# dpmerrell/PathMatFac.jl

Measured on AMD Instinct MI355X. Metric: fit_iters_per_sec, higher is better.
Workload: dtype f32; 1 GPU; fit! epoch on synthetic 200000x50000 matrix (D stored as f32), K=64, Gaussian loss, group-reg X (32 groups) + featureset-ARD Y, adam; rows sharded over 1 GPU(s); full_model=False, M=200000, N=50000, K=64, rows_per_gpu=200000, optimizer=adam, parallelism=single GPU, rccl_ranks=0, collectives_issued=0, column_chunks=1

## Files before the change

include/pmf_hip.h:

```cpp
#ifndef PMF_HIP_H
#define PMF_HIP_H

#include <stdint.h>

#ifdef __cplusplus
extern "C" {
#endif

typedef struct pmf_ctx pmf_ctx;

#define PMF_NOISE_NORMAL 0
#define PMF_NOISE_BERNOULLI 1
#define PMF_NOISE_POISSON 2
#define PMF_NOISE_SQ_HINGE 3

#define PMF_OPT_ADAGRAD 0
#define PMF_OPT_ADAM 1

#define PMF_STORE_F32 0
#define PMF_STORE_BF16 1

#define PMF_TERM_MAX_EPOCHS 0
#define PMF_TERM_LOSS_INCREASE 1
#define PMF_TERM_ABS_TOL 2
#define PMF_TERM_REL_TOL 3
#define PMF_TERM_NONFINITE 4

#define PMF_PARAM_X 0
#define PMF_PARAM_Y 1
#define PMF_PARAM_LOGSIGMA 2
#define PMF_PARAM_MU 3
#define PMF_PARAM_LOGDELTA 4
#define PMF_PARAM_THETA 5

typedef struct pmf_fit_opts {
  int32_t update_X;
  int32_t update_Y;
  int32_t update_col_layers;
  int32_t frozen_layers;
  int32_t frozen_regs;
  int32_t max_epochs;
  int32_t epoch;
  int32_t tol_max_iters;
  int32_t keep_trace;
  int32_t verbosity;
  int32_t print_iter;
  int32_t reserved;
  double abs_tol;
  double rel_tol;
  int64_t capacity;
} pmf_fit_opts;

typedef struct pmf_fit_result {
  int32_t term_code;
  int32_t epochs;
  int32_t n_trace;
  int32_t trace_cap;
  double final_loss;
  double *loss_trace;
  double seconds;
} pmf_fit_result;

const char *pmf_last_error(void);
int pmf_version(void);

int pmf_device_count(int *n);
int pmf_create(int device, pmf_ctx **out);
int pmf_destroy(pmf_ctx *ctx);
int pmf_set_stream(pmf_ctx *ctx, void *hip_stream);
int pmf_synchronize(pmf_ctx *ctx);

int pmf_set_data(pmf_ctx *ctx, const float *D_colmajor, int64_t M, int64_t N, int store);
int pmf_set_data_device(pmf_ctx *ctx, const void *D_device, int64_t M, int64_t N, int store);

int pmf_set_factors(pmf_ctx *ctx, const float *X, const float *Y, int K);
int pmf_set_X(pmf_ctx *ctx, const float *X, int K);
int pmf_set_Y(pmf_ctx *ctx, const float *Y, int K);
int pmf_get_factors(pmf_ctx *ctx, float *X, float *Y);

int pmf_set_col_params(pmf_ctx *ctx, const float *logsigma, const float *mu);
int pmf_get_col_params(pmf_ctx *ctx, float *logsigma, float *mu);

int pmf_set_n_batch_views(pmf_ctx *ctx, int n);
int pmf_set_batch_view(pmf_ctx *ctx, int v, int64_t col_start1, int64_t col_stop1, int nb,
                       const int32_t *batch_of_row, const float *logdelta, const float *theta);
int pmf_get_batch_view(pmf_ctx *ctx, int v, float *logdelta, float *theta);

int pmf_set_noise(pmf_ctx *ctx, int n_ranges, const int64_t *starts1, const int64_t *stops1, const int32_t *kinds,
                  const float *weights);

int pmf_set_noise_thresholds(pmf_ctx *ctx, int n_ranges, const int64_t *starts1, const int64_t *stops1, const float *thr);
int pmf_get_noise_thresholds(pmf_ctx *ctx, float *thr);

int pmf_clear_xreg(pmf_ctx *ctx);
int pmf_add_xreg_l2(pmf_ctx *ctx, const float *w, float p);
int pmf_add_xreg_group(pmf_ctx *ctx, int n_groups, const int64_t *starts1, const int64_t *stops1, const float *w,
                       float p);

int pmf_clear_yreg(pmf_ctx *ctx);
int pmf_add_yreg_l2(pmf_ctx *ctx, const float *w, float p);
int pmf_add_yreg_group(pmf_ctx *ctx, int n_groups, const int64_t *starts1, const int64_t *stops1, const float *w,
                       float p);
int pmf_add_yreg_ard(pmf_ctx *ctx, int n_ranges, const int64_t *starts1, const int64_t *stops1, const float *alpha,
                     const float *beta, float p);
int pmf_add_yreg_fsard(pmf_ctx *ctx, const float *alpha, const float *beta, float p);

typedef struct pmf_csr { int64_t n_rows, n_cols; const int64_t *rowptr; const int32_t *col; const float *val; } pmf_csr;
int pmf_add_xreg_network(pmf_ctx *ctx, int K, const pmf_csr *AA, const pmf_csr *AB, const pmf_csr *BB,
                         const float *const *u0, float p);
int pmf_add_yreg_network(pmf_ctx *ctx, int K, const pmf_csr *AA, const pmf_csr *AB, const pmf_csr *BB,
                         const float *const *u0, float p);
int pmf_get_reg_network_state(pmf_ctx *ctx, int which, int k, float *u, int *cg_iters);
int pmf_add_xreg_l1(pmf_ctx *ctx, const float *w, const uint8_t *mask, float p);
int pmf_add_yreg_l1(pmf_ctx *ctx, const float *w, const uint8_t *mask, float p);

int pmf_set_layer_regs(pmf_ctx *ctx, int n_ranges, const int64_t *starts1, const int64_t *stops1,
                       const float *w_logsigma, const float *c_logsigma, const float *w_mu, const float *c_mu,
                       const float *w_logdelta, const float *c_logdelta, const float *w_theta,
                       const float *c_theta);

int pmf_set_optimizer(pmf_ctx *ctx, int kind, float lr, float eps, float beta1, float beta2);
int pmf_set_lr(pmf_ctx *ctx, float lr);
int pmf_get_lr(pmf_ctx *ctx, float *lr);
int pmf_reset_optimizer_state(pmf_ctx *ctx);
int pmf_get_opt_state(pmf_ctx *ctx, int which, int view, float *acc, float *mom);

int pmf_fit(pmf_ctx *ctx, const pmf_fit_opts *opts, pmf_fit_result *result);

int pmf_loss(pmf_ctx *ctx, double *total, double *data, double *xreg, double *yreg);

typedef struct pmf_lbfgs_opts {
  int32_t m;
  int32_t max_iter;
  int32_t backtrack_max_iter;
  int32_t keep_trace;
  int32_t verbosity;
  int32_t print_iter;
  double rel_tol;
  double abs_tol;
  double backtrack_shrinkage;
  double c1;
  double sy_min;
} pmf_lbfgs_opts;
typedef struct pmf_lbfgs_result {
  int32_t term_code;
  int32_t iters;
  int32_t loss_evals;
  int32_t grad_evals;
  int32_t resets;
  int32_t n_trace;
  int32_t trace_cap;
  int32_t reserved;
  double final_loss;
  double seconds;
  double *loss_trace;
  int32_t *trial_trace;
  int32_t *flag_trace;
} pmf_lbfgs_result;
int pmf_fit_lbfgs(pmf_ctx *ctx, const pmf_lbfgs_opts *opts, pmf_lbfgs_result *result);
int pmf_debug_lbfgs_direction(pmf_ctx *ctx, int n_pairs, const float *sX, const float *sY, const float *yX,
                              const float *yY, const float *gX, const float *gY, float *pX, float *pY);

int pmf_epoch_begin(pmf_ctx *ctx, const pmf_fit_opts *opts);
int pmf_epoch_step_local(pmf_ctx *ctx, const pmf_fit_opts *opts);
int pmf_epoch_step_shared(pmf_ctx *ctx, const pmf_fit_opts *opts);
int pmf_epoch_loss(pmf_ctx *ctx, double *local_loss, double *shared_terms);

#define PMF_COMM_ID_BYTES 128
#define PMF_COMM_NONE 0
#define PMF_COMM_RCCL 1
#define PMF_COMM_HOST 2
typedef int (*pmf_host_allreduce_fn)(void *user, void *host_buf, int64_t count, int dtype);
int pmf_comm_get_unique_id(void *id_out);
int pmf_comm_init(pmf_ctx *ctx, int rank, int nranks, const void *unique_id);
int pmf_comm_init_host(pmf_ctx *ctx, int rank, int nranks, pmf_host_allreduce_fn fn, void *user);
int pmf_comm_destroy(pmf_ctx *ctx);
int pmf_comm_set_chunks(pmf_ctx *ctx, int n_chunks);
int pmf_comm_allreduce(pmf_ctx *ctx, void *host_buf, int64_t count, int dtype, int op);
int pmf_comm_info(pmf_ctx *ctx, int *rank, int *nranks, int *transport, int *n_chunks, int *reserved_cus,
                  int64_t *n_collectives);

int pmf_debug_last_path(pmf_ctx *ctx, int *bmode, int *layer_path, int *slots, int *xreg);
int pmf_debug_last_kernel(pmf_ctx *ctx, int *kernel);

#define PMF_PASS_EXTENTS_MAX 16
int pmf_debug_pass_extents(pmf_ctx *ctx, int update_X, int update_Y, const int64_t *cap_override, int n_max,
                           const char **names, int64_t *need, int64_t *capacity, int *n);

int pmf_debug_live_bytes(int64_t *device_bytes, int64_t *pinned_bytes);

int pmf_grad_device_ptr(pmf_ctx *ctx, int which, void **ptr, int64_t *n_elements);
int pmf_get_grad(pmf_ctx *ctx, int which, int view, float *out);

int pmf_forward(pmf_ctx *ctx, float *Z_host);

#define PMF_IMPUTE_BATCH 1
#define PMF_IMPUTE_LINK 2
#define PMF_IMPUTE_KEEP_OBSERVED 4
int pmf_impute(pmf_ctx *ctx, int flags, int64_t row_start1, int64_t row_stop1, float *out_host, int64_t ld);
int pmf_impute_device(pmf_ctx *ctx, int flags, int64_t row_start1, int64_t row_stop1, float *out_device, int64_t ld);
int pmf_impute_entries(pmf_ctx *ctx, int flags, int64_t n, const int64_t *rows1, const int64_t *cols1, float *out_host);
int pmf_debug_impute_offset(int64_t row, int64_t col, int64_t ld, int64_t *offset);

typedef struct pmf_sim_opts {
  uint64_t seed;
  int64_t row_offset;
  float noise;
  float frac_missing;
} pmf_sim_opts;
int pmf_simulate_data(pmf_ctx *ctx, const pmf_sim_opts *opts, int64_t row_start1, int64_t row_stop1, float *out_host, int64_t ld);
int pmf_simulate_data_device(pmf_ctx *ctx, const pmf_sim_opts *opts, int64_t row_start1, int64_t row_stop1, float *out_device,
                             int64_t ld);
int pmf_simulate_data_resident(pmf_ctx *ctx, const pmf_sim_opts *opts);

#define PMF_DEBATCH_LINK 1
#define PMF_DEBATCH_FILL_MISSING 2
int pmf_remove_batch_effect(pmf_ctx *ctx, int flags, int64_t row_start1, int64_t row_stop1, const float *Z_host, int64_t ldz,
                            float *out_host, int64_t ld);
int pmf_remove_batch_effect_device(pmf_ctx *ctx, int flags, int64_t row_start1, int64_t row_stop1, const float *Z_device,
                                   int64_t ldz, float *out_device, int64_t ld);
int pmf_remove_batch_effect_entries(pmf_ctx *ctx, int flags, int64_t n, const int64_t *rows1, const int64_t *cols1,
                                    const float *values, float *out_host);

int pmf_stats(pmf_ctx *ctx, int use_factors, float *col_n, float *col_sum, float *col_sumsq, float *col_sqerr,
              float *col_ssq_grad, float *batch_count, float *batch_sqerr);

typedef struct pmf_em_opts {
  int32_t update_priors;
  int32_t max_iter;
  int32_t verbosity;
  int32_t reserved;
  double rtol;
} pmf_em_opts;
typedef struct pmf_em_result {
  int32_t iters;
  int32_t n_diffs;
  int32_t diffs_cap;
  int32_t reserved;
  double *diffs;
  double seconds;
} pmf_em_result;
int pmf_stage_init_logsigma(pmf_ctx *ctx);
int pmf_stage_reweight_col_losses(pmf_ctx *ctx, int64_t M_total);
int pmf_get_noise_weights(pmf_ctx *ctx, float *w);
int pmf_stage_minimal_group_weights(pmf_ctx *ctx, int64_t M_total, float *w_out);
int pmf_stage_theta_delta_em(pmf_ctx *ctx, const pmf_em_opts *opts, const float *sigma2, double *delta2,
                             pmf_em_result *result);

int pmf_gram(pmf_ctx *ctx, int which, int n_groups, const int64_t *starts1, const int64_t *stops1, int diag_only, double *out);
int pmf_stage_lambda_max(pmf_ctx *ctx, int which, int n_groups, const int64_t *starts1, const int64_t *stops1, double *lam_out);
int pmf_stage_whiten(pmf_ctx *ctx, int64_t M_total, int n_views, const int64_t *starts1, const int64_t *stops1,
                     double *x_rms_out, double *y_rms_max_out);
int pmf_stage_rotate_by_svd(pmf_ctx *ctx, double *sing_out, double *U_out);
int pmf_stage_reorder_by_importance(pmf_ctx *ctx, int32_t *perm_out);
int pmf_debug_postprocess_times(pmf_ctx *ctx, double *gram_s, double *eig_s, double *apply_s);

int pmf_fsard_update_A(pmf_ctx *ctx, int64_t col_start1, int64_t col_stop1, int L, const float *S, const float *alpha,
                       const float *lambda, float alpha0, float v0, float lr, float *ssq_grad, float *A, int max_epochs,
                       int term_iter, double atol, double *best_loss, int *epochs_run, float *beta_out);
int pmf_fsard_update_A_csr(pmf_ctx *ctx, int64_t col_start1, int64_t col_stop1, int L, const int64_t *rowptr,
                           const int32_t *col, const float *val, const float *alpha, const float *lambda, float alpha0,
                           float v0, float lr, float *ssq_grad, float *A, int max_epochs, int term_iter, double atol,
                           double *best_loss, int *epochs_run, float *beta_out);

#define PMF_PREC_F32 0
#define PMF_PREC_BF16X3 1
int pmf_set_precision(pmf_ctx *ctx, int mode);
int pmf_get_precision(pmf_ctx *ctx, int *mode, int64_t *split_launches);

int pmf_kernel_time(pmf_ctx *ctx, double *mean_ms, int64_t *launches, int reset);
int pmf_synth_data(pmf_ctx *ctx, uint64_t seed, float noise, float frac_nan);

#ifdef __cplusplus
}
#endif
#endif
```

pathmatfac.jl_amd/_lib.py:

```python
import ctypes as C
import os
from pathlib import Path

import numpy as np

_HERE = Path(__file__).resolve().parent
LIB_PATH = _HERE / "libpmf_hip.so"

NOISE = {"normal": 0, "bernoulli": 1, "poisson": 2, "bernoulli_sq_hinge": 3, "ordinal_sq_hinge3": 3}
HINGE_THRESHOLDS = {"bernoulli_sq_hinge": (0.0, np.inf, np.inf), "ordinal_sq_hinge3": (-np.inf, -0.5, 0.5)}
OPT = {"adagrad": 0, "adam": 1}
STORE = {"f32": 0, "bf16": 1}
TERM = {0: "max_epochs", 1: "loss_increase", 2: "abs_tol", 3: "rel_tol", 4: "nonfinite"}
IMPUTE_BATCH, IMPUTE_LINK, IMPUTE_KEEP_OBSERVED = 1, 2, 4
DEBATCH_LINK, DEBATCH_FILL_MISSING = 1, 2
PARAM = {"X": 0, "Y": 1, "logsigma": 2, "mu": 3, "logdelta": 4, "theta": 5}


class PMFError(RuntimeError):
    pass


class FitOpts(C.Structure):
    _fields_ = [("update_X", C.c_int32), ("update_Y", C.c_int32), ("update_col_layers", C.c_int32),
                ("frozen_layers", C.c_int32), ("frozen_regs", C.c_int32), ("max_epochs", C.c_int32),
                ("epoch", C.c_int32), ("tol_max_iters", C.c_int32), ("keep_trace", C.c_int32),
                ("verbosity", C.c_int32), ("print_iter", C.c_int32), ("reserved", C.c_int32),
                ("abs_tol", C.c_double), ("rel_tol", C.c_double), ("capacity", C.c_int64)]


class FitResult(C.Structure):
    _fields_ = [("term_code", C.c_int32), ("epochs", C.c_int32), ("n_trace", C.c_int32),
                ("trace_cap", C.c_int32), ("final_loss", C.c_double), ("loss_trace", C.POINTER(C.c_double)),
                ("seconds", C.c_double)]


class LbfgsOpts(C.Structure):
    _fields_ = [("m", C.c_int32), ("max_iter", C.c_int32), ("backtrack_max_iter", C.c_int32), ("keep_trace", C.c_int32),
                ("verbosity", C.c_int32), ("print_iter", C.c_int32), ("rel_tol", C.c_double), ("abs_tol", C.c_double),
                ("backtrack_shrinkage", C.c_double), ("c1", C.c_double), ("sy_min", C.c_double)]


class LbfgsResult(C.Structure):
    _fields_ = [("term_code", C.c_int32), ("iters", C.c_int32), ("loss_evals", C.c_int32), ("grad_evals", C.c_int32),
                ("resets", C.c_int32), ("n_trace", C.c_int32), ("trace_cap", C.c_int32), ("reserved", C.c_int32),
                ("final_loss", C.c_double), ("seconds", C.c_double), ("loss_trace", C.POINTER(C.c_double)),
                ("trial_trace", C.POINTER(C.c_int32)), ("flag_trace", C.POINTER(C.c_int32))]


class EmOpts(C.Structure):
    _fields_ = [("update_priors", C.c_int32), ("max_iter", C.c_int32), ("verbosity", C.c_int32), ("reserved", C.c_int32),
                ("rtol", C.c_double)]


class EmResult(C.Structure):
    _fields_ = [("iters", C.c_int32), ("n_diffs", C.c_int32), ("diffs_cap", C.c_int32), ("reserved", C.c_int32),
                ("diffs", C.POINTER(C.c_double)), ("seconds", C.c_double)]


class SimOpts(C.Structure):
    _fields_ = [("seed", C.c_uint64), ("row_offset", C.c_int64), ("noise", C.c_float), ("frac_missing", C.c_float)]


class Csr(C.Structure):
    _fields_ = [("n_rows", C.c_int64), ("n_cols", C.c_int64), ("rowptr", C.POINTER(C.c_int64)),
                ("col", C.POINTER(C.c_int32)), ("val", C.POINTER(C.c_float))]


def csr_arrays(A):
    import scipy.sparse as sp
    A = sp.csr_matrix(A)
    A.sum_duplicates()
    A.sort_indices()
    return (A.shape, np.ascontiguousarray(A.indptr, dtype=np.int64), np.ascontiguousarray(A.indices, dtype=np.int32),
            np.ascontiguousarray(A.data, dtype=np.float32))


def dense_to_csr(S):
    S = np.ascontiguousarray(S, dtype=np.float32)
    if S.ndim != 2:
        raise ValueError("dense_to_csr: S must be a matrix")
    L, Nv = S.shape
    flat = np.flatnonzero(S.ravel())
    rowptr = np.zeros(L + 1, np.int64)
    if Nv:
        np.cumsum(np.bincount(flat // Nv, minlength=L), out=rowptr[1:])
        col = (flat % Nv).astype(np.int32)
    else:
        col = np.zeros(0, np.int32)
    return rowptr, col, S.ravel()[flat].astype(np.float32)


EXPORTS = [
    "pmf_last_error", "pmf_version", "pmf_device_count", "pmf_create", "pmf_destroy", "pmf_set_stream", "pmf_synchronize",
    "pmf_set_data", "pmf_set_data_device", "pmf_set_factors", "pmf_set_X", "pmf_set_Y", "pmf_get_factors",
    "pmf_set_col_params", "pmf_get_col_params", "pmf_set_n_batch_views", "pmf_set_batch_view",
    "pmf_get_batch_view", "pmf_set_noise", "pmf_clear_xreg", "pmf_add_xreg_l2", "pmf_add_xreg_group",
    "pmf_clear_yreg", "pmf_add_yreg_l2", "pmf_add_yreg_group", "pmf_add_yreg_ard", "pmf_add_yreg_fsard",
    "pmf_set_layer_regs", "pmf_set_optimizer", "pmf_set_lr", "pmf_get_lr", "pmf_reset_optimizer_state",
    "pmf_fit", "pmf_epoch_begin", "pmf_epoch_step_local", "pmf_epoch_step_shared", "pmf_epoch_loss",
    "pmf_grad_device_ptr", "pmf_get_grad", "pmf_forward", "pmf_stats", "pmf_kernel_time", "pmf_synth_data",
    "pmf_set_precision", "pmf_get_precision",
    "pmf_comm_get_unique_id", "pmf_comm_init", "pmf_comm_init_host", "pmf_comm_destroy", "pmf_comm_set_chunks",
    "pmf_comm_info", "pmf_comm_allreduce", "pmf_get_opt_state", "pmf_fsard_update_A", "pmf_debug_last_path", "pmf_debug_last_kernel",
    "pmf_debug_pass_extents", "pmf_debug_live_bytes",
    "pmf_add_xreg_network", "pmf_add_yreg_network", "pmf_get_reg_network_state", "pmf_add_xreg_l1", "pmf_add_yreg_l1",
    "pmf_impute", "pmf_impute_device", "pmf_impute_entries", "pmf_debug_impute_offset",
    "pmf_loss", "pmf_fit_lbfgs", "pmf_debug_lbfgs_direction",
    "pmf_stage_init_logsigma", "pmf_stage_reweight_col_losses", "pmf_get_noise_weights", "pmf_stage_minimal_group_weights",
    "pmf_stage_theta_delta_em",
    "pmf_gram", "pmf_stage_lambda_max", "pmf_stage_whiten", "pmf_stage_rotate_by_svd", "pmf_stage_reorder_by_importance",
    "pmf_debug_postprocess_times",
    "pmf_fsard_update_A_csr",
    "pmf_set_noise_thresholds", "pmf_get_noise_thresholds",
    "pmf_remove_batch_effect", "pmf_remove_batch_effect_device", "pmf_remove_batch_effect_entries",
    "pmf_simulate_data", "pmf_simulate_data_device", "pmf_simulate_data_resident",
]

COMM_ID_BYTES = 128
HOST_ALLREDUCE_FN = C.CFUNCTYPE(C.c_int, C.c_void_p, C.c_void_p, C.c_int64, C.c_int)


def comm_unique_id(lib_path=None):
    lib = load_library(lib_path)
    buf = C.create_string_buffer(COMM_ID_BYTES)
    if lib.pmf_comm_get_unique_id(buf) != 0:
        raise PMFError(lib.pmf_last_error().decode())
    return buf.raw



def live_bytes(lib_path=None):
    lib = load_library(lib_path)
    d, h = C.c_int64(0), C.c_int64(0)
    if lib.pmf_debug_live_bytes(C.byref(d), C.byref(h)) != 0:
        raise PMFError(lib.pmf_last_error().decode())
    return d.value, h.value


def device_count(lib_path=None):
    lib = load_library(lib_path)
    n = C.c_int(0)
    if lib.pmf_device_count(C.byref(n)) != 0:
        raise PMFError(lib.pmf_last_error().decode())
    return n.value


_lib = None


def load_library(path=None):
    global _lib
    if _lib is not None and path is None:
        return _lib
    p = Path(path) if path else LIB_PATH
    if not p.exists():
        raise PMFError(f"{p} not found: build it with pathmatfac.jl_amd/csrc/build.sh "
                       "(python -c 'import __graft_entry__ as g; g.build()'). There is no CPU fallback.")
    if os.environ.get("PMF_NO_TORCH", "0") != "1":
        try:
            import torch
        except ImportError:
            pass
    lib = C.CDLL(str(p))
    lib.pmf_last_error.restype = C.c_char_p
    for name in EXPORTS:
        getattr(lib, name)
    _lib = lib
    return lib


def _f32(a, order="F"):
    return np.require(np.asarray(a, dtype=np.float32), requirements=["F" if order == "F" else "C", "A"])


def _fp(a):
    return a.ctypes.data_as(C.POINTER(C.c_float)) if a is not None else C.POINTER(C.c_float)()


def _i64p(a):
    return a.ctypes.data_as(C.POINTER(C.c_int64))


def _flat(a):
    if a is None:
        return None
    if isinstance(a, (list, tuple)) and len(a) and np.ndim(a[0]) > 0:
        a = np.concatenate([np.asarray(x, dtype=np.float32).ravel() for x in a])
    return _f32(np.asarray(a, dtype=np.float32).ravel())


def _ranges(ranges):
    s = np.ascontiguousarray([r[0] for r in ranges], dtype=np.int64)
    e = np.ascontiguousarray([r[1] for r in ranges], dtype=np.int64)
    return s, e


class Context:

    def __init__(self, device=0, lib_path=None):
        self.lib = load_library(lib_path)
        self._h = C.c_void_p()
        self._chk(self.lib.pmf_create(int(device), C.byref(self._h)))
        self.M = self.N = self.K = 0
        self.view_shapes = []
        self.n_noise_ranges = 0

    def _chk(self, rc):
        if rc != 0:
            raise PMFError(self.lib.pmf_last_error().decode())

    def close(self):
        if getattr(self, "_h", None) is not None and self._h:
            self.lib.pmf_destroy(self._h)
            self._h = None

    def __del__(self):
        try:
            self.close()
        except Exception:
            pass

    def set_stream(self, stream_ptr):
        HIP_STREAM_LEGACY = 1
        self._chk(self.lib.pmf_set_stream(self._h, C.c_void_p(stream_ptr if stream_ptr else HIP_STREAM_LEGACY)))
        self._stream_adopted = True

    def use_own_stream(self):
        self._chk(self.lib.pmf_set_stream(self._h, C.c_void_p(0)))
        self._stream_adopted = False

    def synchronize(self):
        self._chk(self.lib.pmf_synchronize(self._h))

    def set_data(self, D, store="f32"):
        D = _f32(D)
        if D.shape != (self.M, self.N):
            self.n_noise_ranges = 0
        self.M, self.N = D.shape
        self._chk(self.lib.pmf_set_data(self._h, _fp(D), C.c_int64(self.M), C.c_int64(self.N), STORE[store]))

    def set_data_device(self, ptr, M, N, store="f32"):
        if (int(M), int(N)) != (self.M, self.N):
            self.n_noise_ranges = 0
        self.M, self.N = int(M), int(N)
        self._chk(self.lib.pmf_set_data_device(self._h, C.c_void_p(ptr), C.c_int64(M), C.c_int64(N), STORE[store]))

    def set_factors(self, X, Y):
        X, Y = _f32(X), _f32(Y)
        K = X.shape[0]
        if X.shape != (K, self.M) or Y.shape != (K, self.N):
            raise PMFError(f"factor shapes {X.shape}, {Y.shape} do not match data {self.M} x {self.N}")
        self.K = K
        self._chk(self.lib.pmf_set_factors(self._h, _fp(X), _fp(Y), K))

    def set_X(self, X):
        X = _f32(X)
        self._chk(self.lib.pmf_set_X(self._h, _fp(X), X.shape[0]))

    def set_Y(self, Y):
        Y = _f32(Y)
        self._chk(self.lib.pmf_set_Y(self._h, _fp(Y), Y.shape[0]))

    def get_factors(self):
        X = np.zeros((self.K, self.M), np.float32, order="F")
        Y = np.zeros((self.K, self.N), np.float32, order="F")
        self._chk(self.lib.pmf_get_factors(self._h, _fp(X), _fp(Y)))
        return X, Y

    def set_col_params(self, logsigma=None, mu=None):
        ls = None if logsigma is None else _f32(logsigma)
        m = None if mu is None else _f32(mu)
        self._chk(self.lib.pmf_set_col_params(self._h, _fp(ls), _fp(m)))

    def get_col_params(self):
        ls = np.zeros(self.N, np.float32)
        mu = np.zeros(self.N, np.float32)
        self._chk(self.lib.pmf_get_col_params(self._h, _fp(ls), _fp(mu)))
        return ls, mu

    def set_batch_views(self, views):
        self._chk(self.lib.pmf_set_n_batch_views(self._h, len(views)))
        self.view_shapes = []
        for v, b in enumerate(views):
            ld, th = _f32(b["logdelta"]), _f32(b["theta"])
            nb, Nv = ld.shape
            bor = np.ascontiguousarray(b["batch_of_row"], dtype=np.int32)
            if bor.shape != (self.M,):
                raise PMFError("batch_of_row must have one entry per row")
            self._chk(self.lib.pmf_set_batch_view(self._h, v, C.c_int64(b["start1"]), C.c_int64(b["stop1"]), nb,
                                                  bor.ctypes.data_as(C.POINTER(C.c_int32)), _fp(ld), _fp(th)))
            self.view_shapes.append((nb, Nv))

    def update_batch_values(self, v, start1, stop1, batch_of_row, logdelta, theta):
        ld, th = _f32(logdelta), _f32(theta)
        bor = np.ascontiguousarray(batch_of_row, dtype=np.int32)
        self._chk(self.lib.pmf_set_batch_view(self._h, v, C.c_int64(start1), C.c_int64(stop1), ld.shape[0],
                                              bor.ctypes.data_as(C.POINTER(C.c_int32)), _fp(ld), _fp(th)))

    def get_batch_view(self, v):
        nb, Nv = self.view_shapes[v]
        ld = np.zeros((nb, Nv), np.float32, order="F")
        th = np.zeros((nb, Nv), np.float32, order="F")
        self._chk(self.lib.pmf_get_batch_view(self._h, v, _fp(ld), _fp(th)))
        return ld, th

    def set_noise(self, ranges, kinds, weights=None):
        s, e = _ranges(ranges)
        k = np.ascontiguousarray([NOISE[x] if isinstance(x, str) else int(x) for x in kinds], dtype=np.int32)
        w = None if weights is None else _f32(weights)
        self._chk(self.lib.pmf_set_noise(self._h, len(k), _i64p(s), _i64p(e), k.ctypes.data_as(C.POINTER(C.c_int32)),
                                         _fp(w)))
        self.n_noise_ranges = len(k)
        named = [(r, HINGE_THRESHOLDS[x]) for r, x in zip(ranges, kinds) if x == "ordinal_sq_hinge3"]
        if named:
            self.set_noise_thresholds([r for r, _ in named], [t for _, t in named])

    def set_noise_thresholds(self, ranges, thresholds):
        s, e = _ranges(ranges)
        t = np.ascontiguousarray(np.asarray(thresholds, dtype=np.float32).reshape(len(s), 3))
        self._chk(self.lib.pmf_set_noise_thresholds(self._h, len(s), _i64p(s), _i64p(e), _fp(t)))

    def get_noise_thresholds(self):
        t = np.zeros((self.N, 3), np.float32)
        self._chk(self.lib.pmf_get_noise_thresholds(self._h, _fp(t)))
        return t

    def clear_xreg(self):
        self._chk(self.lib.pmf_clear_xreg(self._h))

    def clear_yreg(self):
        self._chk(self.lib.pmf_clear_yreg(self._h))

    def add_reg_l2(self, which, w, p=1.0):
        w = _f32(np.asarray(w).ravel())
        f = self.lib.pmf_add_xreg_l2 if which == "X" else self.lib.pmf_add_yreg_l2
        self._chk(f(self._h, _fp(w), C.c_float(p)))

    def add_reg_group(self, which, ranges, w, p=1.0):
        s, e = _ranges(ranges)
        w = np.ascontiguousarray(np.asarray(w, dtype=np.float32))
        if w.shape != (len(s), self.K):
            raise PMFError(f"group weights must be (n_groups, K) = ({len(s)}, {self.K}); got {w.shape}")
        f = self.lib.pmf_add_xreg_group if which == "X" else self.lib.pmf_add_yreg_group
        self._chk(f(self._h, len(s), _i64p(s), _i64p(e), _fp(w), C.c_float(p)))

    def add_yreg_ard(self, ranges, alpha, beta, p=1.0):
        s, e = _ranges(ranges)
        a, b = _f32(np.asarray(alpha).ravel()), _f32(np.asarray(beta).ravel())
        self._chk(self.lib.pmf_add_yreg_ard(self._h, len(s), _i64p(s), _i64p(e), _fp(a), _fp(b), C.c_float(p)))

    def add_yreg_fsard(self, alpha, beta, p=1.0):
        a, b = _f32(np.asarray(alpha).ravel()), _f32(beta)
        if a.shape != (self.N,) or b.shape != (self.K, self.N):
            raise PMFError("FeatureSetARD: alpha must be N, beta K x N")
        self._chk(self.lib.pmf_add_yreg_fsard(self._h, _fp(a), _fp(b), C.c_float(p)))

    def add_reg_network(self, which, AA, AB, BB, u0=None, p=1.0):
        K = len(AA)
        keep, blocks = [], []
        for mats in (AA, AB, BB):
            arr = (Csr * K)()
            for k, A in enumerate(mats):
                shape, rp, col, val = csr_arrays(A)
                keep.append((rp, col, val))
                arr[k] = Csr(shape[0], shape[1], rp.ctypes.data_as(C.POINTER(C.c_int64)),
                             col.ctypes.data_as(C.POINTER(C.c_int32)), _fp(val))
            blocks.append(arr)
        up = None
        if u0 is not None:
            us = [_f32(np.asarray(u).ravel()) for u in u0]
            for k, (u, B) in enumerate(zip(us, BB)):
                if u.shape != (B.shape[0],):
                    raise PMFError(f"network regularizer: u0[{k}] has {u.shape[0]} entries, BB[{k}] {B.shape[0]} rows")
            keep.append(us)
            up = (C.POINTER(C.c_float) * K)(*[_fp(u) for u in us])
        f = self.lib.pmf_add_xreg_network if which == "X" else self.lib.pmf_add_yreg_network
        self._chk(f(self._h, K, blocks[0], blocks[1], blocks[2], up, C.c_float(p)))
        if not hasattr(self, "_net_v"):
            self._net_v = {}
        self._net_v[which] = [int(B.shape[0]) for B in BB]

    def get_reg_network_state(self, which, k):
        v = getattr(self, "_net_v", {}).get(which)
        n = v[k] if v is not None and 0 <= k < len(v) else 0
        u = np.zeros(n, np.float32)
        it = C.c_int(0)
        self._chk(self.lib.pmf_get_reg_network_state(self._h, PARAM[which], int(k), _fp(u) if n else None, C.byref(it)))
        return u, it.value

    def add_reg_l1(self, which, w, mask=None, p=1.0):
        w = _f32(np.asarray(w).ravel())
        n = self.M if which == "X" else self.N
        if w.shape != (self.K,):
            raise PMFError(f"L1 weights must have K = {self.K} entries; got {w.shape}")
        mp = None
        if mask is not None:
            m = np.require(np.asarray(mask, dtype=np.uint8), requirements=["F", "A"])
            if m.shape != (self.K, n):
                raise PMFError(f"L1 mask must be K x n = ({self.K}, {n}); got {m.shape}")
            mp = m.ctypes.data_as(C.POINTER(C.c_uint8))
        f = self.lib.pmf_add_xreg_l1 if which == "X" else self.lib.pmf_add_yreg_l1
        self._chk(f(self._h, _fp(w), mp, C.c_float(p)))

    def set_layer_regs(self, ranges=None, w_logsigma=None, c_logsigma=None, w_mu=None, c_mu=None,
                       w_logdelta=None, c_logdelta=None, w_theta=None, c_theta=None):
        ranges = ranges or []
        s, e = _ranges(ranges) if ranges else (np.zeros(1, np.int64), np.zeros(1, np.int64))
        arrs = [_flat(a) for a in (w_logsigma, c_logsigma, w_mu, c_mu, w_logdelta, c_logdelta, w_theta, c_theta)]
        self._keep = arrs
        self._chk(self.lib.pmf_set_layer_regs(self._h, len(ranges), _i64p(s), _i64p(e), *[_fp(a) for a in arrs]))

    def set_optimizer(self, kind="adagrad", lr=1.0, eps=1e-8, beta1=0.9, beta2=0.999):
        self._chk(self.lib.pmf_set_optimizer(self._h, OPT[kind], C.c_float(lr), C.c_float(eps), C.c_float(beta1),
                                             C.c_float(beta2)))

    def set_lr(self, lr):
        self._chk(self.lib.pmf_set_lr(self._h, C.c_float(lr)))

    def get_lr(self):
        v = C.c_float(0)
        self._chk(self.lib.pmf_get_lr(self._h, C.byref(v)))
        return v.value

    def reset_optimizer_state(self):
        self._chk(self.lib.pmf_reset_optimizer_state(self._h))

    @staticmethod
    def make_opts(update_X=False, update_Y=False, update_col_layers=False, frozen_layers=0, frozen_regs=0,
                  max_epochs=1000, epoch=1, tol_max_iters=3, keep_trace=True, verbosity=0, print_iter=10,
                  abs_tol=1e-9, rel_tol=1e-6, capacity=10 ** 8):
        o = FitOpts()
        o.update_X, o.update_Y, o.update_col_layers = int(update_X), int(update_Y), int(update_col_layers)
        o.frozen_layers, o.frozen_regs = int(frozen_layers), int(frozen_regs)
        o.max_epochs, o.epoch, o.tol_max_iters = int(max_epochs), int(epoch), int(tol_max_iters)
        o.keep_trace, o.verbosity, o.print_iter = int(keep_trace), int(verbosity), int(print_iter)
        o.abs_tol, o.rel_tol, o.capacity = float(abs_tol), float(rel_tol), int(capacity)
        return o

    def fit(self, **kw):
        o = self.make_opts(**kw)
        cap = max(o.max_epochs - o.epoch + 1, 1)
        trace = np.zeros(cap, np.float64)
        r = FitResult()
        r.trace_cap = cap
        r.loss_trace = trace.ctypes.data_as(C.POINTER(C.c_double))
        self._chk(self.lib.pmf_fit(self._h, C.byref(o), C.byref(r)))
        return {"term_code": TERM[r.term_code], "epochs": r.epochs, "loss": trace[:r.n_trace].copy(),
                "final_loss": r.final_loss, "seconds": r.seconds}

    def loss(self):
        v = [C.c_double(0) for _ in range(4)]
        self._chk(self.lib.pmf_loss(self._h, *[C.byref(x) for x in v]))
        return dict(zip(("total", "data", "xreg", "yreg"), (x.value for x in v)))

    def fit_lbfgs(self, m=10, max_iter=1000, backtrack_max_iter=100, rel_tol=1e-9, abs_tol=1e-6, backtrack_shrinkage=0.8,
                  c1=1e-4, sy_min=1e-4, keep_trace=True, verbosity=0, print_iter=10):
        o = LbfgsOpts(int(m), int(max_iter), int(backtrack_max_iter), int(keep_trace), int(verbosity), int(print_iter),
                      float(rel_tol), float(abs_tol), float(backtrack_shrinkage), float(c1), float(sy_min))
        cap = max(int(max_iter), 1)
        loss, trials, flags = np.zeros(cap, np.float64), np.zeros(cap, np.int32), np.zeros(cap, np.int32)
        r = LbfgsResult()
        r.trace_cap = cap
        r.loss_trace = loss.ctypes.data_as(C.POINTER(C.c_double))
        r.trial_trace = trials.ctypes.data_as(C.POINTER(C.c_int32))
        r.flag_trace = flags.ctypes.data_as(C.POINTER(C.c_int32))
        self._chk(self.lib.pmf_fit_lbfgs(self._h, C.byref(o), C.byref(r)))
        n = r.n_trace
        return {"term_code": TERM[r.term_code], "iters": r.iters, "loss": loss[:n].copy(), "trials": trials[:n].copy(),
                "flags": flags[:n].copy(), "final_loss": r.final_loss, "loss_evals": r.loss_evals,
                "grad_evals": r.grad_evals, "resets": r.resets, "seconds": r.seconds}

    def debug_lbfgs_direction(self, s_pairs, y_pairs, g):
        n = len(s_pairs)
        def stack(pairs, i, cols):
            if not pairs:
                return None
            return np.ascontiguousarray(np.stack([np.asfortranarray(q[i], dtype=np.float32).ravel(order="F") for q in pairs]))
        sX, sY, yX, yY = stack(s_pairs, 0, self.M), stack(s_pairs, 1, self.N), stack(y_pairs, 0, self.M), stack(y_pairs, 1, self.N)
        gX, gY = _f32(g[0]), _f32(g[1])
        pX = np.zeros((self.K, self.M), np.float32, order="F")
        pY = np.zeros((self.K, self.N), np.float32, order="F")
        self._chk(self.lib.pmf_debug_lbfgs_direction(self._h, n, _fp(sX), _fp(sY), _fp(yX), _fp(yY), _fp(gX), _fp(gY),
                                                     _fp(pX), _fp(pY)))
        return pX, pY

    def epoch_begin(self, o):
        self._chk(self.lib.pmf_epoch_begin(self._h, C.byref(o)))

    def epoch_step_local(self, o):
        self._chk(self.lib.pmf_epoch_step_local(self._h, C.byref(o)))

    def epoch_step_shared(self, o):
        self._chk(self.lib.pmf_epoch_step_shared(self._h, C.byref(o)))

    def epoch_loss(self):
        a, b = C.c_double(0), C.c_double(0)
        self._chk(self.lib.pmf_epoch_loss(self._h, C.byref(a), C.byref(b)))
        return a.value, b.value

    def grad_device_ptr(self, which):
        p, n = C.c_void_p(), C.c_int64(0)
        self._chk(self.lib.pmf_grad_device_ptr(self._h, PARAM[which], C.byref(p), C.byref(n)))
        return p.value, n.value

    def get_grad(self, which, view=0):
        if which == "X":
            out = np.zeros((self.K, self.M), np.float32, order="F")
        elif which == "Y":
            out = np.zeros((self.K, self.N), np.float32, order="F")
        elif which in ("logsigma", "mu"):
            out = np.zeros(self.N, np.float32)
        else:
            out = np.zeros(self.view_shapes[view], np.float32, order="F")
        self._chk(self.lib.pmf_get_grad(self._h, PARAM[which], int(view), _fp(out)))
        return out

    def get_opt_state(self, which, view=0):
        if which == "X":
            shape = (self.K, self.M)
        elif which == "Y":
            shape = (self.K, self.N)
        elif which in ("logsigma", "mu"):
            shape = (self.N,)
        else:
            shape = self.view_shapes[view]
        acc, mom = np.zeros(shape, np.float32, order="F"), np.zeros(shape, np.float32, order="F")
        self._chk(self.lib.pmf_get_opt_state(self._h, PARAM[which], int(view), _fp(acc), _fp(mom)))
        return acc, mom

    def _fsard_call(self, entry, start1, stop1, L, Nv, s_args, alpha, lam, alpha0, v0, lr, ssq_grad, max_epochs, term_iter,
                    atol):
        al = np.ascontiguousarray(alpha, dtype=np.float32)
        lm = np.ascontiguousarray(lam, dtype=np.float32)
        if ssq_grad.dtype != np.float32 or not ssq_grad.flags.c_contiguous or ssq_grad.shape != (L, self.K):
            raise PMFError("ssq_grad must be a C-contiguous float32 L x K array")
        A = np.zeros((L, self.K), np.float32)
        beta = np.zeros((self.K, max(Nv, 0)), np.float32, order="F")
        best, ep = C.c_double(0), C.c_int(0)
        self._chk(entry(self._h, C.c_int64(start1), C.c_int64(stop1), int(L), *s_args, _fp(al), _fp(lm), C.c_float(alpha0),
                        C.c_float(v0), C.c_float(lr), _fp(ssq_grad), _fp(A), int(max_epochs), int(term_iter),
                        C.c_double(atol), C.byref(best), C.byref(ep), _fp(beta)))
        return A, beta, best.value, ep.value

    def fsard_update_A(self, start1, stop1, S, alpha, lam, alpha0, v0, lr, ssq_grad, max_epochs=1000, term_iter=20,
                       atol=1e-5):
        S = np.ascontiguousarray(S, dtype=np.float32)
        L, Nv = S.shape
        if Nv != stop1 - start1 + 1:
            raise PMFError("S must have one column per column of the view")
        return self._fsard_call(self.lib.pmf_fsard_update_A, start1, stop1, L, Nv, (_fp(S),), alpha, lam, alpha0, v0, lr,
                                ssq_grad, max_epochs, term_iter, atol)

    def fsard_update_A_csr(self, start1, stop1, S, alpha, lam, alpha0, v0, lr, ssq_grad, max_epochs=1000, term_iter=20,
                           atol=1e-5):
        Nv = stop1 - start1 + 1
        if isinstance(S, (tuple, list)):
            if len(S) != 3:
                raise PMFError("S must be a dense L x Nv array or a (rowptr, col, val) triple")
            rowptr, col, val = S
        else:
            S = np.asarray(S)
            if S.ndim != 2 or S.shape[1] != Nv:
                raise PMFError("S must have one column per column of the view")
            rowptr, col, val = dense_to_csr(S)
        rowptr = np.ascontiguousarray(rowptr, dtype=np.int64)
        col = np.ascontiguousarray(col, dtype=np.int32)
        val = np.ascontiguousarray(val, dtype=np.float32)
        L = rowptr.size - 1
        if L < 1 or col.shape != val.shape or col.ndim != 1 or rowptr[-1] != col.size:
            raise PMFError("S: rowptr must have L + 1 >= 2 entries and end at the length of col and val")
        if col.size == 0:
            col, val = np.zeros(1, np.int32), np.zeros(1, np.float32)
        al = np.ascontiguousarray(alpha, dtype=np.float32)
        lm = np.ascontiguousarray(lam, dtype=np.float32)
        if al.size != Nv or lm.size != self.K:
            raise PMFError("alpha must have one entry per column of the view and lambda one per factor")
        s_args = (_i64p(rowptr), col.ctypes.data_as(C.POINTER(C.c_int32)), _fp(val))
        return self._fsard_call(self.lib.pmf_fsard_update_A_csr, start1, stop1, L, Nv, s_args, al, lm, alpha0, v0, lr,
                                ssq_grad, max_epochs, term_iter, atol)

    def forward(self):
        Z = np.zeros((self.M, self.N), np.float32, order="F")
        self._chk(self.lib.pmf_forward(self._h, _fp(Z)))
        return Z

    @staticmethod
    def impute_flags(include_batch_effects=False, link=False, keep_observed=False):
        return ((IMPUTE_BATCH if include_batch_effects else 0) | (IMPUTE_LINK if link else 0)
                | (IMPUTE_KEEP_OBSERVED if keep_observed else 0))

    def impute(self, flags=0, row_start1=1, row_stop1=None, out=None, out_row=0):
        row_stop1 = self.M if row_stop1 is None else int(row_stop1)
        rows = max(row_stop1 - int(row_start1) + 1, 0)
        if out is None:
            out, out_row = np.zeros((rows, self.N), np.float32, order="F"), 0
        elif out.dtype != np.float32 or out.ndim != 2 or not out.flags.f_contiguous or out.shape[1] != self.N:
            raise PMFError("impute: out must be a Fortran-ordered float32 array with N columns")
        if out_row < 0 or out_row + rows > out.shape[0]:
            raise PMFError("impute: the block does not fit in out")
        ptr = C.c_void_p(out.ctypes.data + 4 * int(out_row)) if out.size else None
        self._chk(self.lib.pmf_impute(self._h, int(flags), C.c_int64(row_start1), C.c_int64(row_stop1), ptr,
                                      C.c_int64(out.shape[0])))
        return out[out_row:out_row + rows]

    def impute_device(self, ptr, flags=0, row_start1=1, row_stop1=None, ld=None):
        row_stop1 = self.M if row_stop1 is None else int(row_stop1)
        ld = row_stop1 - int(row_start1) + 1 if ld is None else int(ld)
        self._chk(self.lib.pmf_impute_device(self._h, int(flags), C.c_int64(row_start1), C.c_int64(row_stop1),
                                             C.c_void_p(ptr), C.c_int64(ld)))

    def impute_entries(self, rows1, cols1, flags=0):
        r = np.ascontiguousarray(rows1, dtype=np.int64).ravel()
        c = np.ascontiguousarray(cols1, dtype=np.int64).ravel()
        if r.shape != c.shape:
            raise PMFError("impute_entries: rows and columns must have the same length")
        out = np.zeros(max(r.size, 1), np.float32)
        self._chk(self.lib.pmf_impute_entries(self._h, int(flags), C.c_int64(r.size), _i64p(r), _i64p(c), _fp(out)))
        return out[:r.size]

    @staticmethod
    def sim_opts(seed=0, noise=0.1, frac_missing=0.0, row_offset=0):
        return SimOpts(int(seed) & 0xFFFFFFFFFFFFFFFF, int(row_offset), float(noise), float(frac_missing))

    def simulate_data(self, seed=0, noise=0.1, frac_missing=0.0, row_offset=0, row_start1=1, row_stop1=None, out=None,
                      out_row=0):
        row_stop1 = self.M if row_stop1 is None else int(row_stop1)
        rows = max(row_stop1 - int(row_start1) + 1, 0)
        if out is None:
            out, out_row = np.zeros((rows, self.N), np.float32, order="F"), 0
        elif out.dtype != np.float32 or out.ndim != 2 or not out.flags.f_contiguous or out.shape[1] != self.N:
            raise PMFError("simulate_data: out must be a Fortran-ordered float32 array with N columns")
        if out_row < 0 or out_row + rows > out.shape[0]:
            raise PMFError("simulate_data: the block does not fit in out")
        ptr = C.c_void_p(out.ctypes.data + 4 * int(out_row)) if out.size else None
        o = self.sim_opts(seed, noise, frac_missing, row_offset)
        self._chk(self.lib.pmf_simulate_data(self._h, C.byref(o), C.c_int64(row_start1), C.c_int64(row_stop1), ptr,
                                             C.c_int64(out.shape[0])))
        return out[out_row:out_row + rows]

    def simulate_data_device(self, ptr, seed=0, noise=0.1, frac_missing=0.0, row_offset=0, row_start1=1, row_stop1=None,
                             ld=None):
        row_stop1 = self.M if row_stop1 is None else int(row_stop1)
        ld = row_stop1 - int(row_start1) + 1 if ld is None else int(ld)
        o = self.sim_opts(seed, noise, frac_missing, row_offset)
        self._chk(self.lib.pmf_simulate_data_device(self._h, C.byref(o), C.c_int64(row_start1), C.c_int64(row_stop1),
                                                    C.c_void_p(ptr), C.c_int64(ld)))

    def simulate_data_resident(self, seed=0, noise=0.1, frac_missing=0.0, row_offset=0):
        o = self.sim_opts(seed, noise, frac_missing, row_offset)
        self._chk(self.lib.pmf_simulate_data_resident(self._h, C.byref(o)))

    @staticmethod
    def debatch_flags(link=False, fill_missing=False):
        return (DEBATCH_LINK if link else 0) | (DEBATCH_FILL_MISSING if fill_missing else 0)

    def remove_batch_effect(self, flags=0, row_start1=1, row_stop1=None, Z=None, out=None, out_row=0):
        row_stop1 = self.M if row_stop1 is None else int(row_stop1)
        rows = max(row_stop1 - int(row_start1) + 1, 0)
        zp, ldz = None, 0
        if Z is not None:
            Zf = _f32(Z)
            if Zf.shape != (rows, self.N):
                raise PMFError(f"remove_batch_effect: Z must be rows x N = {rows} x {self.N}")
            zp, ldz = C.c_void_p(Zf.ctypes.data), max(rows, 1)
        if out is None:
            out, out_row = np.zeros((rows, self.N), np.float32, order="F"), 0
        elif out.dtype != np.float32 or out.ndim != 2 or not out.flags.f_contiguous or out.shape[1] != self.N:
            raise PMFError("remove_batch_effect: out must be a Fortran-ordered float32 array with N columns")
        if out_row < 0 or out_row + rows > out.shape[0]:
            raise PMFError("remove_batch_effect: the block does not fit in out")
        ptr = C.c_void_p(out.ctypes.data + 4 * int(out_row)) if out.size else None
        self._chk(self.lib.pmf_remove_batch_effect(self._h, int(flags), C.c_int64(row_start1), C.c_int64(row_stop1), zp,
                                                   C.c_int64(ldz), ptr, C.c_int64(out.shape[0])))
        return out[out_row:out_row + rows]

    def remove_batch_effect_device(self, out_ptr, flags=0, row_start1=1, row_stop1=None, z_ptr=None, ldz=None, ld=None):
        row_stop1 = self.M if row_stop1 is None else int(row_stop1)
        rows = row_stop1 - int(row_start1) + 1
        ld = rows if ld is None else int(ld)
        ldz = rows if ldz is None else int(ldz)
        self._chk(self.lib.pmf_remove_batch_effect_device(self._h, int(flags), C.c_int64(row_start1), C.c_int64(row_stop1),
                                                          C.c_void_p(z_ptr) if z_ptr else None, C.c_int64(ldz),
                                                          C.c_void_p(out_ptr), C.c_int64(ld)))

    def remove_batch_effect_entries(self, rows1, cols1, values=None, flags=0):
        r = np.ascontiguousarray(rows1, dtype=np.int64).ravel()
        c = np.ascontiguousarray(cols1, dtype=np.int64).ravel()
        if r.shape != c.shape:
            raise PMFError("remove_batch_effect_entries: rows and columns must have the same length")
        v = None
        if values is not None:
            v = np.ascontiguousarray(values, dtype=np.float32).ravel()
            if v.shape != r.shape:
                raise PMFError("remove_batch_effect_entries: one value per entry")
            if v.size == 0:
                v = np.zeros(1, np.float32)
        out = np.zeros(max(r.size, 1), np.float32)
        self._chk(self.lib.pmf_remove_batch_effect_entries(self._h, int(flags), C.c_int64(r.size), _i64p(r), _i64p(c), _fp(v),
                                                           _fp(out)))
        return out[:r.size]

    def stats(self, use_factors=False):
        N = self.N
        out = {k: np.zeros(N, np.float32) for k in ("n", "sum", "sumsq", "sqerr", "ssq_grad")}
        nbt = sum(nb * nv for nb, nv in self.view_shapes)
        bc, bs = np.zeros(max(nbt, 1), np.float32), np.zeros(max(nbt, 1), np.float32)
        self._chk(self.lib.pmf_stats(self._h, int(use_factors), _fp(out["n"]), _fp(out["sum"]), _fp(out["sumsq"]),
                                     _fp(out["sqerr"]), _fp(out["ssq_grad"]), _fp(bc), _fp(bs)))
        off, cnt, sq = 0, [], []
        for nb, nv in self.view_shapes:
            cnt.append(bc[off:off + nb * nv].reshape((nb, nv), order="F").copy())
            sq.append(bs[off:off + nb * nv].reshape((nb, nv), order="F").copy())
            off += nb * nv
        out["batch_count"], out["batch_sqerr"] = cnt, sq
        return out

    def stage_init_logsigma(self):
        self._chk(self.lib.pmf_stage_init_logsigma(self._h))

    def stage_reweight_col_losses(self, M_total):
        self._chk(self.lib.pmf_stage_reweight_col_losses(self._h, C.c_int64(int(M_total))))

    def get_noise_weights(self):
        w = np.zeros(self.N, np.float32)
        self._chk(self.lib.pmf_get_noise_weights(self._h, _fp(w)))
        return w

    def stage_minimal_group_weights(self, M_total):
        w = np.zeros(max(self.n_noise_ranges, 1), np.float32)
        self._chk(self.lib.pmf_stage_minimal_group_weights(self._h, C.c_int64(int(M_total)), _fp(w)))
        return w[:self.n_noise_ranges]

    def stage_theta_delta_em(self, delta2, sigma2, update_priors=True, max_iter=100, rtol=1e-8, verbosity=0):
        if len(delta2) != len(self.view_shapes) or any(np.shape(d) != s for d, s in zip(delta2, self.view_shapes)):
            raise PMFError(f"delta2 must hold one array per batch view, shaped {self.view_shapes}")
        s2 = _f32(np.asarray(sigma2).ravel())
        if s2.shape != (self.N,):
            raise PMFError("sigma2 must have N entries")
        flat = np.ascontiguousarray(np.concatenate([np.asarray(d, np.float64).ravel(order="F") for d in delta2] or
                                                   [np.zeros(1)]))
        cap = max(int(max_iter), 1)
        diffs = np.zeros(cap, np.float64)
        o = EmOpts(int(bool(update_priors)), int(max_iter), int(verbosity), 0, float(rtol))
        r = EmResult()
        r.diffs_cap = cap
        r.diffs = diffs.ctypes.data_as(C.POINTER(C.c_double))
        self._chk(self.lib.pmf_stage_theta_delta_em(self._h, C.byref(o), _fp(s2), flat.ctypes.data_as(C.POINTER(C.c_double)),
                                                    C.byref(r)))
        out, off = [], 0
        for nb, nv in self.view_shapes:
            out.append(flat[off:off + nb * nv].reshape((nb, nv), order="F").copy())
            off += nb * nv
        theta = [self.get_batch_view(v)[1] for v in range(len(self.view_shapes))]
        return dict(theta=theta, delta2=out, diffs=diffs[:r.n_diffs].copy(), iters=r.iters, seconds=r.seconds)

    @staticmethod
    def _dp(a):
        return a.ctypes.data_as(C.POINTER(C.c_double))

    def gram(self, which, ranges, diag_only=False):
        s, e = _ranges(ranges)
        out = np.zeros((len(s), self.K) if diag_only else (len(s), self.K, self.K), np.float64)
        self._chk(self.lib.pmf_gram(self._h, int(which), len(s), _i64p(s), _i64p(e), int(bool(diag_only)), self._dp(out)))
        return out

    def stage_lambda_max(self, which, ranges):
        s, e = _ranges(ranges)
        lam = np.zeros(max(len(s), 1), np.float64)
        self._chk(self.lib.pmf_stage_lambda_max(self._h, int(which), len(s), _i64p(s), _i64p(e), self._dp(lam)))
        return lam[:len(s)]

    def stage_whiten(self, M_total, view_ranges):
        s, e = _ranges(view_ranges)
        xr, c = np.zeros(max(self.K, 1), np.float64), np.zeros(max(len(s), 1), np.float64)
        self._chk(self.lib.pmf_stage_whiten(self._h, C.c_int64(int(M_total)), len(s), _i64p(s), _i64p(e), self._dp(xr), self._dp(c)))
        return xr[:self.K], c[:len(s)]

    def stage_rotate_by_svd(self):
        sing, U = np.zeros(max(self.K, 1), np.float64), np.zeros((max(self.K, 1),) * 2, np.float64)
        self._chk(self.lib.pmf_stage_rotate_by_svd(self._h, self._dp(sing), self._dp(U)))
        return sing[:self.K], U[:self.K, :self.K]

    def stage_reorder_by_importance(self):
        p = np.zeros(max(self.K, 1), np.int32)
        self._chk(self.lib.pmf_stage_reorder_by_importance(self._h, p.ctypes.data_as(C.POINTER(C.c_int32))))
        return p[:self.K].astype(np.int64)

    def postprocess_times(self):
        g, e, a = C.c_double(0), C.c_double(0), C.c_double(0)
        self._chk(self.lib.pmf_debug_postprocess_times(self._h, C.byref(g), C.byref(e), C.byref(a)))
        return dict(gram=g.value, eig=e.value, apply=a.value)

    def comm_init(self, rank, nranks, unique_id):
        if len(unique_id) != COMM_ID_BYTES:
            raise PMFError("unique id must be 128 bytes (comm_unique_id())")
        self._chk(self.lib.pmf_comm_init(self._h, int(rank), int(nranks), C.c_char_p(bytes(unique_id))))

    def comm_init_host(self, rank, nranks, allreduce):
        def _cb(_user, buf, count, dtype):
            try:
                ct = C.c_double if dtype == 1 else C.c_float
                arr = np.ctypeslib.as_array(C.cast(buf, C.POINTER(ct)), shape=(int(count),))
                allreduce(arr)
                return 0
            except Exception:
                import traceback
                traceback.print_exc()
                return -1
        self._host_cb = HOST_ALLREDUCE_FN(_cb)
        self._chk(self.lib.pmf_comm_init_host(self._h, int(rank), int(nranks), self._host_cb, None))

    def comm_destroy(self):
        self._chk(self.lib.pmf_comm_destroy(self._h))
        self._host_cb = None

    def comm_set_chunks(self, n):
        self._chk(self.lib.pmf_comm_set_chunks(self._h, int(n)))

    def comm_allreduce(self, arr, op="sum"):
        if arr.dtype not in (np.float32, np.float64) or not arr.flags.c_contiguous:
            raise PMFError("comm_allreduce needs a contiguous float32 / float64 array")
        self._chk(self.lib.pmf_comm_allreduce(self._h, arr.ctypes.data_as(C.c_void_p), C.c_int64(arr.size),
                                              1 if arr.dtype == np.float64 else 0, {"sum": 0, "max": 1}[op]))
        return arr

    def comm_info(self):
        r, n, t, ch, cu = C.c_int(0), C.c_int(0), C.c_int(0), C.c_int(0), C.c_int(0)
        nc = C.c_int64(0)
        self._chk(self.lib.pmf_comm_info(self._h, C.byref(r), C.byref(n), C.byref(t), C.byref(ch), C.byref(cu), C.byref(nc)))
        return dict(rank=r.value, nranks=n.value, transport=("none", "rccl", "host")[t.value], n_chunks=ch.value,
                    reserved_cus=cu.value, n_collectives=nc.value)

    def last_path(self):
        b, l, s, x = C.c_int(0), C.c_int(0), C.c_int(0), C.c_int(0)
        self._chk(self.lib.pmf_debug_last_path(self._h, C.byref(b), C.byref(l), C.byref(s), C.byref(x)))
        return dict(bmode=b.value, layer_path=l.value, slots=s.value, xreg=x.value)

    def last_kernel(self):
        k = C.c_int(0)
        self._chk(self.lib.pmf_debug_last_kernel(self._h, C.byref(k)))
        return k.value

    def pass_extents(self, update_X=False, update_Y=False, capacity_override=None):
        n_max = 16
        names, n = (C.c_char_p * n_max)(), C.c_int(0)
        need, cap = (C.c_int64 * n_max)(), (C.c_int64 * n_max)()
        ov = None
        if capacity_override is not None:
            plain = self.pass_extents(update_X, update_Y)
            unknown = set(capacity_override) - set(plain)
            if unknown:
                raise PMFError(f"pass_extents: unknown buffers {sorted(unknown)}")
            ov = (C.c_int64 * n_max)(*([-1] * n_max))
            for i, k in enumerate(plain):
                ov[i] = int(capacity_override.get(k, -1))
        self._chk(self.lib.pmf_debug_pass_extents(self._h, int(update_X), int(update_Y), ov, n_max, names, need, cap,
                                                  C.byref(n)))
        return {names[i].decode(): dict(need=need[i], capacity=cap[i]) for i in range(n.value)}

    def set_precision(self, mode):
        self._chk(self.lib.pmf_set_precision(self._h, {"f32": 0, "bf16x3": 1}[mode]))

    def get_precision(self):
        mode, n = C.c_int(0), C.c_int64(0)
        self._chk(self.lib.pmf_get_precision(self._h, C.byref(mode), C.byref(n)))
        return ("f32", "bf16x3")[mode.value], n.value

    def kernel_time(self, reset=False):
        ms, n = C.c_double(0), C.c_int64(0)
        self._chk(self.lib.pmf_kernel_time(self._h, C.byref(ms), C.byref(n), int(reset)))
        return ms.value, n.value

    def synth_data(self, seed=20260104, noise=0.1, frac_nan=0.0):
        self._chk(self.lib.pmf_synth_data(self._h, C.c_uint64(seed), C.c_float(noise), C.c_float(frac_nan)))
```

pathmatfac.jl_amd/csrc/pmf_common.h:

```cpp
#ifndef PMF_COMMON_H
#define PMF_COMMON_H
#include <hip/hip_runtime.h>

#include <cstdint>
#include <type_traits>
#include <unordered_map>

#include "../../include/pmf_hip.h"

int pmf_fail(const char *fmt, ...);
#define HIPCHK(x)                                                                                    \
  do {                                                                                               \
    hipError_t e_ = (x);                                                                             \
    if (e_ != hipSuccess) return pmf_fail("%s failed: %s (%s:%d)", #x, hipGetErrorString(e_), __FILE__, __LINE__); \
  } while (0)
#define PMFCHK(x)          \
  do {                     \
    int r_ = (x);          \
    if (r_ < 0) return r_; \
  } while (0)

typedef std::unordered_map<const void *, size_t> PmfDynLds;
int pmf_ensure_dyn_lds(PmfDynLds *cache, const void *kern, size_t lds);

typedef float f32x16 __attribute__((ext_vector_type(16)));

#define PMF_MAXV 16
#define PMF_PM_BYTES 256
#define PMF_BN 32
#define PMF_DPAD 64

__host__ __device__ __forceinline__ int64_t pmf_d_off(int64_t i, int64_t j, int64_t nRB) {
  const int il = (int)(i & 31), jl = (int)(j & 31);
  const int h = (jl >> 2) & 1;
  const int r = (jl & 3) + 4 * (jl >> 3);
  return (((j >> 5) * nRB) + (i >> 5)) * 1024 + (r >> 2) * 256 + (h * 32 + il) * 4 + (r & 3);
}

struct ViewDesc {
  int64_t c0;
  int64_t c1;
  int64_t tab_off;
  int32_t nb;
  int32_t pad;
};

struct FusedArgs {
  const void *D;
  const uint32_t *tflags;
  int64_t nRB;
  const float *X;
  const float *Y;
  float *gX;
  float *gY;
  float *gy_slabs;
  int64_t slab_stride;
  int64_t n_rp;
  int64_t n_tiles;
  const int64_t *wg_begin;
  int32_t tps;
  int32_t n_ct;
  const float4 *colp;
  const int32_t *bor;
  const float2 *btab;
  const float2 *btd;
  const uint8_t *pm, *row_slot, *colview;
  int32_t nbs_shift;
  int32_t n_bv;
  double *loss_partial;
  int64_t M, N;
  int32_t n_cseg;
  int32_t want_gx, want_gy;
  unsigned long long *stamps;
  int32_t dbg;
  const ViewDesc *views;
  const char *Xsb, *Ysb;
  int32_t ct0;
  float *gx_part;
  const int32_t *piece_base;
  int64_t gx_slot_stride;
  const float *sb_scale_x, *sb_scale_y;
  const float *htab;
};

__device__ __forceinline__ int pmf_rowmap(int r, int h) { return (r & 3) + 8 * (r >> 2) + 4 * h; }
__device__ __forceinline__ bool pmf_finite(float y) { return fabsf(y) <= 3.402823466e38f; }

__host__ __device__ __forceinline__ int pmf_meta_kind(int meta) { return meta & 3; }
__host__ __device__ __forceinline__ int pmf_meta_view(int meta) { return (meta >> 2) - 1; }
__host__ __device__ __forceinline__ int64_t pmf_view_index(const ViewDesc &vd, int64_t j, int b) { return (j - vd.c0) * vd.nb + b; }
__host__ __device__ __forceinline__ int64_t pmf_btab_index(const ViewDesc &vd, int64_t j, int b) { return vd.tab_off + pmf_view_index(vd, j, b); }
__device__ __forceinline__ int pmf_row_batch(const int32_t *bor, int64_t M, int v, int64_t i) { return v >= 0 ? bor[(int64_t)v * M + i] : -1; }
__device__ __forceinline__ float2 pmf_batch_dt(const ViewDesc &vd, const float2 *btab, int64_t j, int b) {
  return b >= 0 ? btab[pmf_btab_index(vd, j, b)] : make_float2(1.f, 0.f);
}

#define PMF_HT 8
__device__ __forceinline__ void pmf_hinge_terms(float z, float y, const float *T, float &a, float &b) {
  const int c = (int)fminf(fmaxf(y + 0.5f, 0.f), 3.f);
  const float lo = T[c], hi = T[4 + c];
  a = fmaxf(0.f, 1.f - (z - lo));
  b = fmaxf(0.f, 1.f - (hi - z));
}
__device__ __forceinline__ float pmf_hinge_class(float z, const float4 t) { return (float)((t.x < z) + (t.y < z) + (t.z < z)); }

template <bool HINGE = true>
__device__ __forceinline__ void pmf_noise(int kind, float z, float y, float w, const float *tp, float &l, float &g) {
  if (HINGE && kind == PMF_NOISE_SQ_HINGE) {
    float a, b;
    pmf_hinge_terms(z, y, tp, a, b);
    l = 0.5f * w * fmaf(a, a, b * b);
    g = w * (b - a);
  } else if (kind == PMF_NOISE_NORMAL) {
    const float d = z - y;
    g = w * d;
    l = 0.5f * g * d;
  } else if (kind == PMF_NOISE_BERNOULLI) {
    const float e = __expf(-fabsf(z));
    const float sp = fmaxf(z, 0.f) + __logf(1.f + e);
    const float r = __frcp_rn(1.f + e);
    const float sg = z >= 0.f ? r : e * r;
    l = w * (sp - y * z);
    g = w * (sg - y);
  } else {
    const float e = __expf(z);
    l = w * (e - y * z);
    g = w * (e - y);
  }
}

#define PMF_SCHED_FENCE() asm volatile("" ::: "memory")

typedef float pmf_f32x4 __attribute__((ext_vector_type(4)));
__device__ __forceinline__ float4 pmf_load_stream(const float4 *p) {
  const pmf_f32x4 v = __builtin_nontemporal_load(reinterpret_cast<const pmf_f32x4 *>(p));
  return make_float4(v.x, v.y, v.z, v.w);
}
__device__ __forceinline__ void pmf_store_stream(float4 *p, const float4 &v) {
  const pmf_f32x4 vv = {v.x, v.y, v.z, v.w};
  __builtin_nontemporal_store(vv, reinterpret_cast<pmf_f32x4 *>(p));
}

#if defined(PMF_STAMPS) && defined(PMF_STAMP_FROM)
#define PMF_STAMP(slot)                                                                      \
  do {                                                                                       \
    if ((slot) == PMF_STAMP_FROM || (slot) == PMF_STAMP_TO) {                                \
      unsigned long long t_;                                                                 \
      __builtin_amdgcn_sched_barrier(0);                                                     \
      asm volatile("s_memtime %0\n\ts_waitcnt lgkmcnt(0)" : "=s"(t_)::"memory");             \
      __builtin_amdgcn_sched_barrier(0);                                                     \
      if ((slot) == PMF_STAMP_TO) st_acc[1] += t_ - st_prev;                                 \
      if ((slot) == PMF_STAMP_FROM) st_prev = t_;                                            \
    }                                                                                        \
  } while (0)
#elif defined(PMF_STAMPS)
#define PMF_STAMP(slot)                                                                      \
  do {                                                                                       \
    unsigned long long t_;                                                                   \
    __builtin_amdgcn_sched_barrier(0);                                                       \
    asm volatile("s_memtime %0\n\ts_waitcnt lgkmcnt(0)" : "=s"(t_)::"memory");               \
    __builtin_amdgcn_sched_barrier(0);                                                       \
    st_acc[slot] += t_ - st_prev;                                                            \
    st_prev = t_;                                                                            \
  } while (0)
#else
#define PMF_STAMP(slot) do { } while (0)
#endif


typedef __bf16 bf16x8 __attribute__((ext_vector_type(8)));
typedef __bf16 bf16x4 __attribute__((ext_vector_type(4)));
typedef short s16x4 __attribute__((ext_vector_type(4)));

template <int KB>
__host__ __device__ __forceinline__ int pmf_sb_f(int row) {
  if (KB == 1) return (row >> 2) & 3;
  const int x = (row >> 1) & 7;
  return x ^ ((x & 1) << 2);
}
template <int KB>
__host__ __device__ __forceinline__ int pmf_sb_off(int row, int ch) { return 64 * KB * row + 16 * (ch ^ pmf_sb_f<KB>(row)); }

template <int KB>
struct SbCfg {
  static constexpr int NW = 8, Kp = 32 * KB, SLAB = 32 * Kp;
  static constexpr int IMG = 2048 * KB;
  static constexpr int BLK = 3 * IMG;
  static constexpr int LDSP = 2 * IMG;
  static constexpr size_t lds_bytes = 2 * LDSP + IMG + NW * LDSP + NW * SLAB * 4 + 8 * PMF_BN * 4 + 16 + 8 * NW;
  static constexpr size_t lds_batch(int n_bv) { return PMF_BN * 16 * sizeof(float2) + PMF_PM_BYTES + (size_t)NW * n_bv * 32; }
  static constexpr int max_bv = KB == 1 ? PMF_MAXV : (int)((160 * 1024 - lds_bytes - PMF_BN * 16 * sizeof(float2) - PMF_PM_BYTES) / (NW * 32));
};

struct SbSplitArgs {
  const float *src;
  const float4 *colp;
  int64_t n, nblk;
  char *out;
};

struct Sb2Cfg {
  static constexpr size_t lds_bytes = (2 * 2 * 4096 + 4096 + 8 * 2 * 4096 + 4 * 8192 + 4 * 4096 + 8 * PMF_BN * 4 + 16 + 8 * 4 + 15) / 16 * 16;
  static constexpr size_t lds_batch(int n_bv) { return PMF_BN * 16 * sizeof(float2) + PMF_PM_BYTES + (size_t)4 * 2 * n_bv * 32; }
  static constexpr int max_bv = PMF_MAXV;
};

__device__ __forceinline__ bf16x8 pmf_sb_tr8(const char *p0, const char *p1) {
  typedef s16x4 __attribute__((address_space(3))) * lds_p;
  const s16x4 t0 = __builtin_amdgcn_ds_read_tr16_b64_v4i16((lds_p)(p0));
  const s16x4 t1 = __builtin_amdgcn_ds_read_tr16_b64_v4i16((lds_p)(p1));
  typedef short s16x8 __attribute__((ext_vector_type(8)));
  const s16x8 t = __builtin_shufflevector(t0, t1, 0, 1, 2, 3, 4, 5, 6, 7);
  return __builtin_bit_cast(bf16x8, t);
}


__host__ __device__ __forceinline__ int pmf_sb4_off(int row, int ch) { return 256 * row + 16 * (ch ^ (((row & 3) << 2) | ((row >> 2) & 3))); }
template <int KB>
struct Sb4Cfg {
  static constexpr int NW = 4, Kp = 32 * KB, SLAB = 32 * Kp;
  static constexpr int IMG = 32 * 256;
  static constexpr int XBLK = 5 * IMG;
  static constexpr int YBLK = 3 * IMG;
  static constexpr size_t lds_bytes = (2 * 2 * IMG + IMG + NW * SLAB * 4 + 8 * PMF_BN * 4 + 16 + 8 * NW + 15) / 16 * 16;
  static constexpr size_t lds_batch(int n_bv) { return PMF_BN * 16 * sizeof(float2) + PMF_PM_BYTES + (size_t)NW * n_bv * 32; }
  static constexpr int max_bv = PMF_MAXV;
};
struct Sb4SplitArgs {
  const float *src;
  const float4 *colp;
  int64_t n, nblk;
  int32_t Ksrc, transposed;
  char *out;
};
typedef _Float16 f16x8 __attribute__((ext_vector_type(8)));
template <int KB>
__host__ __device__ __forceinline__ int pmf_sb8_f_off(int row, int ch) { return 1024 * (ch % (2 * KB)) + 512 * (ch / (2 * KB)) + 16 * row; }
__host__ __device__ __forceinline__ int pmf_sb8_xt_off(int k, int c) { return 64 * k + 16 * (c ^ ((k >> 2) & 3)); }
template <int KB>
struct Sb8Cfg {
  static_assert(KB == 4 || KB == 2, "pmf_fused_sb8_kernel: KB = 4 or 2");
  static constexpr int NW = 4, RB = 8 / KB, Kp = 32 * KB, BM = 32 * NW * RB, NBLK = NW * RB;
  static constexpr int IMG = 64 * Kp;
  static constexpr int XBLK = 4 * IMG, YBLK = 4 * IMG;
  static constexpr size_t lds_bytes = (2 * 2 * IMG + 2 * IMG + NBLK * 4096 + NBLK * IMG + 8 * PMF_BN * 4 + 16 + 8 * NW + 15) / 16 * 16;
  static constexpr size_t lds_batch(int n_bv) { return PMF_BN * 16 * sizeof(float2) + PMF_PM_BYTES + (size_t)NW * RB * n_bv * 32; }
  static constexpr int max_bv = (int)((160 * 1024 - lds_bytes - PMF_BN * 16 * sizeof(float2) - PMF_PM_BYTES) / (NW * RB * 32)) < PMF_MAXV
                                    ? (int)((160 * 1024 - lds_bytes - PMF_BN * 16 * sizeof(float2) - PMF_PM_BYTES) / (NW * RB * 32)) : PMF_MAXV;
};
template <int KB>
__host__ __device__ __forceinline__ int pmf_sb8_y_off(int row, int ch) { return KB == 4 ? pmf_sb4_off(row, ch) : pmf_sb_off<2>(row, ch); }
struct Sb8SplitArgs {
  const float *src;
  const float4 *colp;
  const float *scale;
  int64_t n, nblk;
  int32_t transposed;
  char *out;
};
struct Sb8ScaleArgs {
  const float *src;
  const float4 *colp;
  int64_t n;
  int32_t Kp;
  uint32_t *max_bits;
  float *scale_out;
};

__device__ __forceinline__ uint32_t pmf_bt_index(const FusedArgs &a, const unsigned char *Pm, int64_t j, int s, int vw) {
  const int ident = (1 << a.nbs_shift) - 1;
  int b = ident;
  if (vw != 255) { const int q = Pm[vw * 16 + s]; if (q != 255) b = q; }
  return ((uint32_t)j << a.nbs_shift) + (uint32_t)b;
}

__device__ __forceinline__ int pmf_bt_view(const FusedArgs &a, int64_t j, int e) { return a.colview[j + (e >> 4)]; }
__device__ __forceinline__ float2 pmf_bt_entry(const FusedArgs &a, const unsigned char *Pm, int64_t j, int e, int vw) {
  return a.btd[pmf_bt_index(a, Pm, j + (e >> 4), e & 15, vw)];
}

__device__ __forceinline__ int pmf_xcd_wg(unsigned b, unsigned g) {
  const unsigned x = b & 7, q = g >> 3, r = g & 7;
  return (int)(x * q + (x < r ? x : r) + (b >> 3));
}

__host__ __device__ __forceinline__ int64_t pmf_d_off16(int64_t i, int64_t j, int64_t nRB) {
  const int il = (int)(i & 31), jl = (int)(j & 31);
  const int h = (jl >> 2) & 1;
  const int r = (jl & 3) + 4 * (jl >> 3);
  return (((j >> 5) * nRB) + (i >> 5)) * 1024 + ((r >> 3) * 256 + (h * 32 + il) * 4 + ((r & 7) >> 1)) * 2 + (r & 1);
}
template <bool DB>
struct PmfDTile;
template <>
struct PmfDTile<false> {
  f32x16 v;
  static constexpr int NCH = 4;
  __device__ __forceinline__ float get(int r) const { return v[r]; }
  __device__ __forceinline__ void load(const void *D, int64_t tile, int lane, int q) {
    const float4 x = pmf_load_stream(reinterpret_cast<const float4 *>(reinterpret_cast<const float *>(D) + tile * 1024) + lane + 64 * q);
    v[4 * q + 0] = x.x; v[4 * q + 1] = x.y; v[4 * q + 2] = x.z; v[4 * q + 3] = x.w;
  }
  __device__ __forceinline__ void touch() const { const f32x16 k = v; asm volatile("" ::"v"(k)); }
};
template <>
struct PmfDTile<true> {
  uint32_t w[8];
  static constexpr int NCH = 2;
  __device__ __forceinline__ float get(int r) const {
    const uint32_t x = w[r >> 1];
    return __uint_as_float((r & 1) ? (x & 0xffff0000u) : (x << 16));
  }
  __device__ __forceinline__ void load(const void *D, int64_t tile, int lane, int q) {
    typedef uint32_t u32x4 __attribute__((ext_vector_type(4)));
    const u32x4 x = __builtin_nontemporal_load(reinterpret_cast<const u32x4 *>(reinterpret_cast<const uint16_t *>(D) + tile * 1024) + lane + 64 * q);
    w[4 * q + 0] = x.x; w[4 * q + 1] = x.y; w[4 * q + 2] = x.z; w[4 * q + 3] = x.w;
  }
  __device__ __forceinline__ void touch() const {
    const uint32_t a0 = w[0], a1 = w[1], a2 = w[2], a3 = w[3], a4 = w[4], a5 = w[5], a6 = w[6], a7 = w[7];
    asm volatile("" ::"v"(a0), "v"(a1), "v"(a2), "v"(a3), "v"(a4), "v"(a5), "v"(a6), "v"(a7));
  }
};


#define PMF_LS 2

struct LayerPassArgs {
  const void *D;
  int32_t d_bf16;
  int64_t nRB;
  const float *X, *Y;
  const float4 *colp;
  const int32_t *bor;
  const float2 *btd;
  float2 *LG;
  int64_t lg_stride;
  int32_t nbs_shift;
  double *loss_partial;
  int64_t M, N;
  int32_t n_bv, n_ct, n_rp, n_seg, R;
  const float *htab;
};

struct LayerMapArgs {
  const float2 *LG;
  int64_t lg_stride;
  int32_t n_parts;
  const float2 *btd;
  const float4 *colp;
  float *g_logsigma, *g_mu, *g_logdelta, *g_theta;
  int64_t N;
  int32_t n_bv, nbs_shift;
  ViewDesc views[PMF_MAXV];
  int64_t val_off[PMF_MAXV];
};

__host__ __device__ __forceinline__ int64_t pmf_impute_off(int64_t r, int64_t j, int64_t ld) { return j * ld + r; }

__device__ __forceinline__ float pmf_impute_invlink(int kind, float z, const float4 *tp) {
  if (kind == PMF_NOISE_SQ_HINGE) return pmf_hinge_class(z, *tp);
  if (kind == PMF_NOISE_BERNOULLI) {
    const float e = __expf(-fabsf(z));
    const float r = __frcp_rn(1.f + e);
    return z >= 0.f ? r : e * r;
  }
  if (kind == PMF_NOISE_POISSON) return __expf(z);
  return z;
}

struct ImputeArgs {
  const float *X, *Y;
  const float4 *colp;
  const int32_t *bor;
  const float2 *btab;
  const ViewDesc *views;
  const void *D;
  int64_t nRB;
  float *out;
  int64_t ld;
  int64_t M, N;
  int64_t row0, row1;
  int64_t rp0, n_rp;
  int32_t n_bv, n_ct, n_seg, R, flags;
  const float4 *thr;
};

__host__ __device__ __forceinline__ void pmf_philox4x32(const uint32_t c[4], uint32_t k0, uint32_t k1, uint32_t r[4]) {
  uint32_t c0 = c[0], c1 = c[1], c2 = c[2], c3 = c[3];
#pragma unroll
  for (int i = 0; i < 10; ++i) {
    const uint64_t p0 = (uint64_t)0xD2511F53u * c0, p1 = (uint64_t)0xCD9E8D57u * c2;
    const uint32_t n0 = (uint32_t)(p1 >> 32) ^ c1 ^ k0, n2 = (uint32_t)(p0 >> 32) ^ c3 ^ k1;
    c1 = (uint32_t)p1; c3 = (uint32_t)p0; c0 = n0; c2 = n2;
    k0 += 0x9E3779B9u; k1 += 0xBB67AE85u;
  }
  r[0] = c0; r[1] = c1; r[2] = c2; r[3] = c3;
}
struct PmfSimDraws { float n, u3, u4; };
__host__ __device__ __forceinline__ PmfSimDraws pmf_sim_draws(uint64_t seed, uint64_t i, uint64_t j, bool want_n) {
  const uint32_t c[4] = {(uint32_t)i, (uint32_t)(i >> 32), (uint32_t)j, (uint32_t)(j >> 32)};
  uint32_t r[4];
  pmf_philox4x32(c, (uint32_t)seed, (uint32_t)(seed >> 32), r);
  PmfSimDraws d;
  d.n = 0.f;
  if (want_n) {
    const float u1 = (float)((r[0] >> 8) + 1u) * 5.9604644775390625e-8f, u2 = (float)(r[1] >> 8) * 5.9604644775390625e-8f;
    d.n = sqrtf(-2.f * logf(u1)) * cosf(6.28318530718f * u2);
  }
  d.u3 = (float)(r[2] >> 8) * 5.9604644775390625e-8f;
  d.u4 = (float)(r[3] >> 8) * 5.9604644775390625e-8f;
  return d;
}

struct SimArgs {
  uint64_t seed;
  int64_t row_offset;
  float noise, frac_missing;
};
#define PMF_SIM_COLMAJOR 0
#define PMF_SIM_TILE_F32 1
#define PMF_SIM_TILE_BF16 2

struct ImputeEntriesArgs {
  const float *X, *Y;
  const float4 *colp;
  const int32_t *bor;
  const float2 *btab;
  const ViewDesc *views;
  const int64_t *rows1, *cols1;
  float *out;
  int64_t n, M;
  int32_t Kp, K, flags;
  const float4 *thr;
};

struct DebatchArgs {
  const void *Z;
  int64_t ldz, nRB;
  const float4 *colp;
  const int32_t *bor;
  const float2 *btab;
  const ViewDesc *views;
  float *out;
  int64_t ld;
  int64_t M, N;
  int64_t row0, row1;
  int64_t rb0, n_rb;
  int64_t n_ct;
  int32_t n_bv, flags;
};

struct DebatchEntriesArgs {
  const float *values;
  const void *D;
  int64_t nRB;
  int32_t d_bf16, n_bv;
  const float4 *colp;
  const int32_t *bor;
  const float2 *btab;
  const ViewDesc *views;
  const int64_t *rows1, *cols1;
  float *out;
  int64_t n, M;
  int32_t flags;
};

typedef int PmfFusedLaunch(PmfDynLds *cache, hipStream_t stream, const FusedArgs &a, int grid, bool batch, bool mixed);
PmfFusedLaunch pmf_launch_fused_exact_11, pmf_launch_fused_exact_12, pmf_launch_fused_exact_21, pmf_launch_fused_exact_31,
    pmf_launch_fused_exact_41, pmf_launch_fused_exact_11_bf16, pmf_launch_fused_exact_12_bf16, pmf_launch_fused_exact_21_bf16,
    pmf_launch_fused_exact_31_bf16, pmf_launch_fused_exact_41_bf16;
extern thread_local int pmf_last_xreg;
PmfFusedLaunch pmf_launch_fused_sb_1, pmf_launch_fused_sb_2, pmf_launch_fused_sb_1_bf16, pmf_launch_fused_sb_2_bf16;
PmfFusedLaunch pmf_launch_fused_sb2, pmf_launch_fused_sb2_bf16;
PmfFusedLaunch pmf_launch_fused_sb4_3, pmf_launch_fused_sb4_4, pmf_launch_fused_sb4_3_bf16, pmf_launch_fused_sb4_4_bf16;
PmfFusedLaunch pmf_launch_fused_sb8_2, pmf_launch_fused_sb8_4, pmf_launch_fused_sb8_2_bf16, pmf_launch_fused_sb8_4_bf16;
int pmf_launch_sb4_split(hipStream_t stream, const Sb4SplitArgs &a);
int pmf_launch_sb8_split(hipStream_t stream, const Sb8SplitArgs &a, int KB);
int pmf_launch_sb8_scale(hipStream_t stream, const Sb8ScaleArgs &a);
int pmf_launch_sb_split_1(hipStream_t stream, const SbSplitArgs &a);
int pmf_launch_sb_split_2(hipStream_t stream, const SbSplitArgs &a);
size_t pmf_layer_pass_lds(int KB, int lnw, int nbs);
int pmf_launch_layer_pass(PmfDynLds *cache, hipStream_t stream, int KB, int lnw, bool mixed, int grid, const LayerPassArgs &a);
int pmf_launch_layer_map(hipStream_t stream, const LayerMapArgs &m);
int pmf_impute_waves(int KB);
int pmf_launch_impute(PmfDynLds *cache, hipStream_t stream, int KB, bool d_bf16, int grid, const ImputeArgs &a);
int pmf_launch_impute_entries(hipStream_t stream, const ImputeEntriesArgs &a);
int pmf_launch_simulate(PmfDynLds *cache, hipStream_t stream, int KB, int form, int grid, const ImputeArgs &a, const SimArgs &s);
int pmf_launch_debatch(hipStream_t stream, int src, int n_cu, const DebatchArgs &a);
int pmf_launch_debatch_entries(hipStream_t stream, const DebatchEntriesArgs &a);
#endif
```

pathmatfac.jl_amd/csrc/pmf_ctx.h:

```cpp
#ifndef PMF_CTX_H
#define PMF_CTX_H
#include <hip/hip_runtime.h>

#include <algorithm>
#include <atomic>
#include <chrono>
#include <cmath>
#include <cstdarg>
#include <cstdio>
#include <cstdlib>
#include <cstring>
#include <memory>
#include <string>
#include <unordered_map>
#include <vector>

#include "pmf_common.h"

int memset_now(void *p, int v, size_t bytes);
inline std::atomic<int64_t> pmf_live_bytes[2];
template <typename T, bool PINNED = false>
struct DevBuf {
  T *p = nullptr;
  size_t n = 0;
  DevBuf() = default;
  DevBuf(const DevBuf &) = delete;
  DevBuf &operator=(const DevBuf &) = delete;
  DevBuf(DevBuf &&o) noexcept : p(o.p), n(o.n) { o.p = nullptr; o.n = 0; }
  DevBuf &operator=(DevBuf &&o) noexcept {
    if (this != &o) { free(); p = o.p; n = o.n; o.p = nullptr; o.n = 0; }
    return *this;
  }
  ~DevBuf() { free(); }
  operator T *() const { return p; }
  size_t size() const { return n; }
  size_t bytes() const { return n * sizeof(T); }
  void free() {
    if (p) {
      (void)(PINNED ? hipHostFree(p) : hipFree(p));
      pmf_live_bytes[PINNED] -= (int64_t)bytes();
    }
    p = nullptr; n = 0;
  }
  int alloc(size_t count, bool zero, const char *what = nullptr) {
    free();
    count = std::max<size_t>(count, 1);
    const hipError_t e = PINNED ? hipHostMalloc((void **)&p, count * sizeof(T)) : hipMalloc((void **)&p, count * sizeof(T));
    if (e != hipSuccess) {
      p = nullptr;
      (void)hipGetLastError();
      return pmf_fail("cannot allocate %zu bytes of %s memory for %s: %s", count * sizeof(T), PINNED ? "pinned host" : "device",
                      what ? what : "a library buffer", hipGetErrorString(e));
    }
    n = count;
    pmf_live_bytes[PINNED] += (int64_t)bytes();
    if (zero) {
      if (PINNED) memset(p, 0, bytes());
      else PMFCHK(memset_now(p, 0, bytes()));
    }
    return 0;
  }
  int ensure(size_t count, bool zero, const char *what = nullptr) { return count <= n ? 0 : alloc(count, zero, what); }
  int upload(const T *src, size_t count) {
    if (count) HIPCHK(hipMemcpy(p, src, count * sizeof(T), hipMemcpyHostToDevice));
    return 0;
  }
};
template <typename T>
using PinnedBuf = DevBuf<T, true>;

struct ParamBuf {
  DevBuf<float> p, g, acc, mom;
  DevBuf<float> wq, cq;
  DevBuf<float> wl1;
  int64_t n = 0;
  float bp1 = 0.f, bp2 = 0.f;
};

struct PanelSlots {
  int64_t serial = -1;
  int BM = 0;
  bool ok = false;
  DevBuf<uint8_t> pm, row_slot;
};

struct WorkSplit {
  int64_t key[11] = {-1, -1, -1, -1, -1, -1, -1, -1, -1, -1, -1};
  int grid = 0;
  int64_t serial = 0;
  DevBuf<int64_t> wg_begin;
  DevBuf<int32_t> c_off, c_idx;
  DevBuf<int32_t> piece_base;
  std::vector<int32_t> h_piece_base;
  std::vector<int32_t> piece_rp;
  int32_t slot_base = 0;
  DevBuf<int32_t> d_piece_base_abs;
};

struct Comm {
  int rank = 0, nranks = 1;
  void *nccl = nullptr;
  pmf_host_allreduce_fn host_fn = nullptr;
  void *host_user = nullptr;
  hipStream_t stream = nullptr;
  PinnedBuf<char> stage;
  int reserve_cus = 0;
  int cta_cap = 0;
  DevBuf<char> dstage;
  bool broken = false;
  int64_t m_mean = 0;
  std::vector<hipEvent_t> ev_ready, ev_done;
  hipEvent_t ev_loss_ready = nullptr, ev_loss_done = nullptr, ev_layer_ready = nullptr, ev_layer_done = nullptr;
  int64_t n_allreduce = 0;
};

struct NetReg {
  int K = 0;
  int64_t n = 0, V = 0;
  float p = 1.f;
  std::vector<int64_t> h_voff;
  DevBuf<int64_t> voff;
  DevBuf<int64_t> aa_rp, ab_rp, abt_rp, bb_rp;
  DevBuf<int32_t> aa_col, ab_col, abt_col, bb_col;
  DevBuf<float> aa_val, ab_val, abt_val, bb_val;
  DevBuf<float> u;
  DevBuf<float> work;
  DevBuf<float> PT;
  DevBuf<float> grad;
  DevBuf<int32_t> iters;
  DevBuf<double> uloss;
  int rb = 1;
  int64_t vmax = 0;
};

struct pmf_ctx {
  int device = 0;
  hipStream_t stream = nullptr;
  bool own_stream = true;
  int n_cu = 256;
  int64_t M = 0, N = 0;
  int K = 0, Kp = 0, KB = 0;
  DevBuf<char> D;
  bool own_D = false;
  int64_t D_M = 0, D_Npad = 0, nRB = 0;
  DevBuf<uint32_t> tflags;
  bool tflags_valid = false;
  int store = PMF_STORE_F32;
  ParamBuf P[6];
  int n_bv = 0;
  std::vector<ViewDesc> views;
  std::vector<int64_t> val_off;
  std::vector<int64_t> bvb_off;
  DevBuf<int32_t> bor;
  DevBuf<float2> btab;
  bool views_dirty = true;
  DevBuf<ViewDesc> d_views;
  DevBuf<float2> LG;
  DevBuf<float> lgrad_part;
  DevBuf<float2> btd;
  bool btd_ok = false;
  int nbs = 16;
  DevBuf<uint8_t> colview;
  std::vector<std::vector<int32_t>> h_bor;
  PanelSlots pslots[3];
  int64_t views_serial = 0;
  int last_kernel = 0;
  int last_bmode = 0, last_layer_path = 0, last_xreg = 0;
  DevBuf<int32_t> d_val_view;
  DevBuf<int32_t> colmeta;
  DevBuf<float> colw;
  DevBuf<float4> colp;
  DevBuf<float4> thr;
  DevBuf<float> htab;
  std::vector<float> h_thr;
  bool mixed = false;
  bool prepared = false;
  DevBuf<float> ard_alpha, ard_beta;
  float ard_scale = 0.f;
  bool has_ard = false;
  bool ard_is_fsard = false;
  int opt_kind = PMF_OPT_ADAGRAD;
  float lr = 1.f, eps = 1e-8f, b1 = 0.9f, b2 = 0.999f;
  bool state_init = false;
  DevBuf<double> loss_partial;
  std::vector<uint8_t> h_kind;
  std::vector<int64_t> noise_s1, noise_e1;
  std::vector<WorkSplit> splits;
  int n_chunks_req = 0;
  DevBuf<float> gx_part;
  DevBuf<int32_t> gx_off, gx_idx;
  int64_t gx_serial = -1;
  int64_t split_serial = 0;
  Comm comm;
  int last_chunks = 1;
  hipEvent_t ev_host = nullptr;
  int64_t kind_version = 0;
  DevBuf<float> gy_slabs;
  int precision = PMF_PREC_F32;
  DevBuf<char> xsb, ysb;
  DevBuf<float> sb8_scale;
  DevBuf<uint32_t> sb8_max;
  int64_t sb_launches = 0;
  int64_t n_macro = 0;
  DevBuf<double> reg_partial;
  DevBuf<double> d_loss;
  PinnedBuf<double> h_loss;
  std::vector<std::pair<hipEvent_t, hipEvent_t>> ev_pool;
  size_t ev_used = 0;
  double kernel_ms_sum = 0.0;
  int64_t kernel_launches = 0;
  NetReg *net[2] = {nullptr, nullptr};
  int reg_counts[4] = {0, 0, 0, 0};
  DevBuf<char> scratch;
  DevBuf<char> impute_stage;
  PmfDynLds dyn_lds;
  double pp_seconds[3] = {0.0, 0.0, 0.0};
  struct LbfgsState *lbfgs = nullptr;
};

#define REG_SLOTS 1024
#define PMF_MAX_CHUNKS 16

struct FusedFamily;
struct FusedGeom {
  const FusedFamily *fam = nullptr;
  int grid_max = 256, S = 1;
  int bmode = 0;
  PanelSlots *ps = nullptr;
  int64_t n_rp = 0, n_ct_all = 0;
  int64_t ct0[PMF_MAX_CHUNKS], nct[PMF_MAX_CHUNKS];
};

struct RegCounts { int c[4]; };

__device__ __forceinline__ double block_reduce_sum(double v, double *sh) {
#pragma unroll
  for (int off = 32; off > 0; off >>= 1) v += __shfl_xor(v, off, 64);
  const int w = threadIdx.x >> 6;
  if ((threadIdx.x & 63) == 0) sh[w] = v;
  __syncthreads();
  double s = 0.0;
  if (threadIdx.x == 0)
    for (int q = 0; q < (int)(blockDim.x >> 6); ++q) s += sh[q];
  return s;
}
__device__ __forceinline__ double block_all_sum_256(double v, double *sh) {
#pragma unroll
  for (int off = 32; off > 0; off >>= 1) v += __shfl_xor(v, off, 64);
  if ((threadIdx.x & 63) == 0) sh[threadIdx.x >> 6] = v;
  __syncthreads();
  const double s = ((sh[0] + sh[1]) + sh[2]) + sh[3];
  __syncthreads();
  return s;
}

struct StepArgs {
  float *p, *g, *acc, *mom;
  const float *wq, *cq;
  const float *ard_alpha, *ard_beta;
  float ard_scale;
  int64_t n;
  int Kp, K;
  int opt_kind;
  float lr, eps, b1, b2, c1, c2;
  int do_step;
  int use_reg;
  double *reg_partial;
};
__device__ __forceinline__ void pmf_reg_quad(float p, float w, float cq, float &g, double &lacc) {
  const float d = p - cq;
  const float gr = w * d;
  lacc += 0.5 * (double)(gr * d);
  g += gr;
}
__device__ __forceinline__ void pmf_reg_ard(float p, float be, float al, float scale, float &g, double &lacc) {
  const float b = 1.f + (0.5f / be) * (p * p);
  lacc += (double)(scale * (0.5f + al) * logf(b));
  g += scale * ((al + 0.5f) * p / (b * be));
}

inline int nblocks(int64_t n, int bs) { return (int)((n + bs - 1) / bs); }
inline void fill_views(const pmf_ctx *c, ViewDesc *views, int64_t *val_off = nullptr) {
  for (int v = 0; v < c->n_bv; ++v) {
    views[v] = c->views[v];
    if (val_off) val_off[v] = c->val_off[v];
  }
}
inline int ensure_loss_partials(pmf_ctx *c, int64_t n) {
  PMFCHK(c->loss_partial.ensure((size_t)n, true));
  c->n_macro = n;
  return 0;
}
template <typename T>
int upload_new(DevBuf<T> &b, const T *src, size_t n) {
  PMFCHK(b.alloc(n, false));
  return b.upload(src, n);
}
template <typename T>
int upload_vec(pmf_ctx *c, std::common_type_t<T> *dst, const T *src, size_t n) {
  if (n == 0) return 0;
  HIPCHK(hipMemcpyAsync(dst, src, sizeof(T) * n, hipMemcpyHostToDevice, c->stream));
  HIPCHK(hipStreamSynchronize(c->stream));
  return 0;
}

int ctx_bind(pmf_ctx *c);
int ensure_dyn_lds(pmf_ctx *c, const void *kern, size_t lds);
int check_ready(pmf_ctx *c);
int prepare(pmf_ctx *c);
int upload_padded(pmf_ctx *c, float *dst, const float *src, int64_t n, float padval);
int download_padded(pmf_ctx *c, float *dst_host, const float *src_dev, int64_t n);
int epoch_open(pmf_ctx *c, const pmf_fit_opts *o);
int epoch_layer_pass(pmf_ctx *c, const pmf_fit_opts *o, bool with_loss);
int step_param_range(pmf_ctx *c, int which, int64_t e0, int64_t n, bool do_step, bool use_reg, int reg_slot, int *reg_count,
                     int max_blocks, bool advance);
int step_param(pmf_ctx *c, int which, bool do_step, bool use_reg, int reg_slot, int *reg_count);
int step_layers(pmf_ctx *c, const pmf_fit_opts *o, int *reg_count);
int launch_loss_reduce(pmf_ctx *c, const RegCounts &rc, int mask);
void step_args_xy(pmf_ctx *c, int which, StepArgs *s);
int eval_full_loss(pmf_ctx *c, double out[4]);
int eval_data_grads(pmf_ctx *c);
int stats_pass_check(pmf_ctx *c);
int stats_pass(pmf_ctx *c, int use_factors, bool want_cols, bool want_batch, const float **cols, const float **batch);
int harvest_events(pmf_ctx *c);
int launch_fused(pmf_ctx *c, bool want_gx, bool want_gy);
FusedGeom fused_geometry(pmf_ctx *c, bool want_gx, bool want_gy, bool allow_chunks);
int prepare_fused_pass(pmf_ctx *c, const FusedGeom &g, bool want_gx, bool want_gy);
int launch_fused_chunk(pmf_ctx *c, const FusedGeom &g, int s, bool want_gx, bool want_gy);
struct PassExtent { const char *name; int64_t need, cap; };
constexpr int PMF_PASS_EXTENTS = 10;
int fused_pass_extents(pmf_ctx *c, const FusedGeom &g, bool want_gx, bool want_gy, PassExtent *out);
int check_pass_extents(const PassExtent *e, int n);
int guard_fused_pass(pmf_ctx *c, const FusedGeom &g, bool want_gx, bool want_gy);
void lbfgs_free(pmf_ctx *c);
void netreg_free(pmf_ctx *c, int which);
int netreg_eval(pmf_ctx *c, int which, int *reg_count);
int comm_release(pmf_ctx *c);
bool comm_active(const pmf_ctx *c);
int comm_allreduce(pmf_ctx *c, void *p, int64_t count, bool f64);
int comm_error_exit(pmf_ctx *c, int rc);
#endif
```

pathmatfac.jl_amd/csrc/pmf_fused.hip.inc:

```

template <int KB, int NW, int RBW = 1>
struct FusedCfg {
  static constexpr int Kp = 32 * KB;
  static constexpr int KpS = Kp + 4;
  static constexpr int SLAB = 32 * Kp;
  static constexpr int YT = PMF_BN * KpS;
  static constexpr int XP = 32 * KpS;
  static constexpr int TT = (RBW - 1) * 1024;
  static constexpr int FIXED = NW * SLAB + NW * RBW * XP + NW * TT + 8 * PMF_BN + 4;
  static constexpr int LDS_BUDGET = 160 * 1024;
  static constexpr int NYB = (2 * YT + FIXED) * 4 + 8 * NW <= LDS_BUDGET ? 2 : 1;
  static constexpr size_t lds_bytes = (sizeof(float) * (NYB * YT + FIXED) + sizeof(double) * NW + 15) / 16 * 16;
  static constexpr size_t lds_batch_extra = PMF_BN * 16 * sizeof(float2) + PMF_PM_BYTES + NW * RBW * 16 * 32;
};

#ifndef PMF_NW4_WAVES
#define PMF_NW4_WAVES 1
#endif
template <int KB, int NW, int RBW, int BMODE, bool MIXED, int GM, bool DB, bool XW = false, bool XR = false>
__global__ __launch_bounds__(64 * NW, (NW == 8 ? 2 : PMF_NW4_WAVES)) void pmf_fused_kernel(const FusedArgs a) {
  using Cfg = FusedCfg<KB, NW, RBW>;
  constexpr bool FULL = GM != 3;
  constexpr bool TIGHT = XW && DB && MIXED && BMODE != 0;
  constexpr bool BATCH = BMODE != 0;
  constexpr bool bt_lds = BMODE == 1;
  constexpr int Kp = Cfg::Kp;
  constexpr int KS = Kp / 2;
  constexpr int KpS = Cfg::KpS;
  constexpr int BM = 32 * NW * RBW;
  constexpr int BN = PMF_BN;
  constexpr int NT = 64 * NW;
  constexpr int SLAB = Cfg::SLAB;
  constexpr int NYB = Cfg::NYB;
  constexpr int YV = (BN * Kp / 4 + NT - 1) / NT;
  constexpr int RV4 = (BN * Kp / 4 + NT - 1) / NT;
  constexpr int NBT = (BN * 16 + NT - 1) / NT;
  static_assert(!XW || (KB == 2 && NW == 8 && RBW == 1 && GM == 0 && NYB == 2 && RV4 == 1 && 2 * NW * 1024 <= NW * SLAB),
                "cross-wave GEMM3: 8 waves x one row block, Kp = 64, both gradients");
  static_assert(!XR || XW, "register-resident X fragments: the cross-wave GEMM3 instances only");

  extern __shared__ __attribute__((aligned(16))) char smem[];
  float *Ys = reinterpret_cast<float *>(smem);
  float *Xs = Ys + NYB * Cfg::YT;
  float *Sl = Xs + NW * RBW * Cfg::XP;
  float *Tt = Sl + NW * SLAB;
  float *Cmu = Tt + NW * Cfg::TT;
  float *Cw = Cmu + 2 * BN;
  float *Csg = Cw + 2 * BN;
  int *Cmt = reinterpret_cast<int *>(Csg + 2 * BN);
  int *Ck = Cmt + 2 * BN;
  double *red = reinterpret_cast<double *>(Ck + 4);
  float *Btd = reinterpret_cast<float *>(smem + Cfg::lds_bytes), *Btt = Btd + BN * 16;
  unsigned char *Pm = reinterpret_cast<unsigned char *>(Btd + 2 * BN * 16);
  unsigned char *Bw0 = Pm + PMF_PM_BYTES + (threadIdx.x >> 6) * RBW * 16 * 32;

  const int tid = threadIdx.x;
  const int lane = tid & 63;
  const int w = tid >> 6;
  const int l31 = lane & 31;
  const int h = lane >> 5;
  const int64_t M = a.M, N = a.N;
  const bool want_gx = GM == 3 ? a.want_gx != 0 : GM != 2, want_gy = GM == 3 ? a.want_gy != 0 : GM != 1;
  const int dbg = FULL ? 0 : a.dbg;
  float *Sw = Sl + w * SLAB;
  float *Xw[RBW], *T[RBW];
#pragma unroll
  for (int rb = 0; rb < RBW; ++rb) {
    Xw[rb] = Xs + (w * RBW + rb) * Cfg::XP;
    T[rb] = rb == 0 ? Sw + (KB - 1) * 1024 : Tt + (w * (RBW - 1) + rb - 1) * 1024;
  }
  const int xw_j = 16 * (w & 1) + (lane & 15), xw_k = 16 * (w >> 1) + 4 * (lane >> 4);
  const int xw_e = xw_j * Kp + xw_k;
  const int xw_x = 4 * (lane >> 4) * KpS + 16 * (w >> 1) + (lane & 15);
  int xw_g[4];
  typedef const __attribute__((address_space(3))) float *lds_cptr;
  unsigned xw_xa[4];
#pragma unroll
  for (int u = 0; u < 4; ++u) {
    const int i = 4 * (lane >> 4) + u;
    xw_g[u] = i * 32 + 4 * ((xw_j >> 2) ^ (i & 7)) + (xw_j & 3);
    xw_xa[u] = (unsigned)(uintptr_t)(lds_cptr)(Xs + xw_x + u * KpS);
    if (XW && !TIGHT) asm volatile("" : "+v"(xw_xa[u]));
  }

  constexpr bool HOIST = KB == 2 && NW == 8 && RBW == 1 && GM != 3 && !TIGHT && (XW || GM != 0 || BMODE == 0);
  unsigned ho_y[2][YV], ho_s[2][YV], ho_c[2], ho_g[2][RV4];
  if (HOIST) {
#pragma unroll
    for (int z = 0; z < 2; ++z) {
      const int ncol = z == 0 || N % BN == 0 ? BN : (int)(N % BN);
#pragma unroll
      for (int q = 0; q < YV; ++q) {
        int e4 = tid + NT * q;
        if (e4 > BN * Kp / 4 - 1) e4 = BN * Kp / 4 - 1;
        int jl = (e4 * 4) / Kp;
        if (jl >= ncol) { jl = ncol - 1; e4 = jl * (Kp / 4); }
        ho_y[z][q] = 16u * e4;
        ho_s[z][q] = 16u * jl;
        asm volatile("" : "+v"(ho_y[z][q]), "+v"(ho_s[z][q]));
      }
      ho_c[z] = 16u * (tid < ncol ? tid : ncol - 1);
      asm volatile("" : "+v"(ho_c[z]));
#pragma unroll
      for (int q = 0; q < RV4; ++q) {
        int e = xw_e;
        if (!XW) {
          const int f = tid + NT * q, ff = f < BN * Kp / 4 ? f : 0;
          e = ((ff % (BN * 8)) / 8) * Kp + 32 * (ff / (BN * 8)) + 4 * (ff % 8);
        }
        ho_g[z][q] = 4u * (e < ncol * Kp ? e : e % Kp);
        asm volatile("" : "+v"(ho_g[z][q]));
      }
    }
  }
  auto ho_at = [](const void *base, unsigned off) { return reinterpret_cast<const char *>(base) + off; };
#ifdef PMF_STAMPS
  unsigned long long st_acc[16] = {0, 0, 0, 0, 0, 0, 0, 0, 0, 0, 0, 0, 0, 0, 0, 0};
  unsigned long long st_prev = __builtin_amdgcn_s_memtime();
  const unsigned long long st_t0 = st_prev, st_r0 = __builtin_amdgcn_s_memrealtime();
#endif
  const int wg = pmf_xcd_wg(blockIdx.x, gridDim.x);
  const int64_t w_begin = a.wg_begin[wg];
  const int64_t w_end = a.wg_begin[wg + 1];
  float *myslab = a.gy_slabs + (int64_t)wg * a.slab_stride;
  const int64_t seg_block = a.n_rp * a.tps;
  double lossacc = 0.0;
  int seg_cur = -1, pidx = 0, t0_first = 0;
  int gx_slot = (GM == 2) ? 0 : a.piece_base[wg];
  for (int64_t widx = w_begin; widx < w_end;) {
    int cs = (int)(widx / seg_block);
    if (cs > a.n_cseg - 1) cs = a.n_cseg - 1;
    const int tps_cs = cs == a.n_cseg - 1 ? a.n_ct - (a.n_cseg - 1) * a.tps : a.tps;
    const int64_t rem = widx - (int64_t)cs * seg_block;
    const int64_t rp = rem / tps_cs;
    const int ti0 = (int)(rem - rp * tps_cs);
    const int ntiles = (int)(tps_cs - ti0 < w_end - widx ? tps_cs - ti0 : w_end - widx);
    widx += ntiles;
    if (cs != seg_cur) { seg_cur = cs; pidx = 0; t0_first = ti0; } else { ++pidx; }
    bool slab_first = true;
    const int64_t col_begin = ((int64_t)a.ct0 + (int64_t)cs * a.tps + ti0) * BN;
    int64_t row0[RBW], irow_c[RBW];
    bool row_ok[RBW];
#pragma unroll
    for (int rb = 0; rb < RBW; ++rb) {
      row0[rb] = rp * BM + (int64_t)(w * RBW + rb) * 32;
      const int64_t irow = row0[rb] + l31;
      row_ok[rb] = irow < M;
      irow_c[rb] = row_ok[rb] ? irow : (M - 1);
    }

    constexpr int XV = (32 * Kp / 4) / 64;
    float4 xv0[RBW][XV];
#pragma unroll
    for (int rb = 0; rb < RBW; ++rb) {
#pragma unroll
      for (int q = 0; q < XV; ++q) {
        const int e4 = lane + 64 * q;
        const int il = (e4 * 4) / Kp;
        const int64_t ir = row0[rb] + il < M ? row0[rb] + il : M - 1;
        xv0[rb][q] = *reinterpret_cast<const float4 *>(a.X + ir * Kp + (e4 * 4) % Kp);
      }
    }
    f32x16 gx[RBW][KB];
#pragma unroll
    for (int rb = 0; rb < RBW; ++rb)
#pragma unroll
      for (int kb = 0; kb < KB; ++kb)
#pragma unroll
        for (int r = 0; r < 16; ++r) gx[rb][kb][r] = 0.f;
    float4 xf[XR ? KS / 4 : 1];
    float xg[XR ? 8 * NW : 1];

    auto stage_load_y = [&](int64_t jt, int q, float4 (&yv)[YV], float (&sgv)[YV]) {
      const float *yb = a.Y + jt * Kp;
      const float4 *cb = a.colp + jt;
      const int64_t rem = N - jt;
      if (HOIST) {
        const bool rag = rem < BN;
        yv[q] = *reinterpret_cast<const float4 *>(ho_at(yb, rag ? ho_y[1][q] : ho_y[0][q]));
        sgv[q] = *reinterpret_cast<const float *>(ho_at(cb, rag ? ho_s[1][q] : ho_s[0][q]));
        return;
      }
      const int ncol = rem > BN ? BN : (int)rem;
      int e4 = tid + NT * q;
      if (e4 > BN * Kp / 4 - 1) e4 = BN * Kp / 4 - 1;
      int jl = (e4 * 4) / Kp;
      if (jl >= ncol) { jl = ncol - 1; e4 = jl * (Kp / 4); }
      yv[q] = *reinterpret_cast<const float4 *>(yb + e4 * 4);
      sgv[q] = cb[jl].x;
    };
    auto stage_load_c = [&](int64_t jt, float4 &cv) {
      const float4 *cb = a.colp + jt;
      const int64_t rem = N - jt;
      if (HOIST) {
        cv = *reinterpret_cast<const float4 *>(ho_at(cb, rem < BN ? ho_c[1] : ho_c[0]));
        return;
      }
      const int ncol = rem > BN ? BN : (int)rem;
      cv = cb[tid < ncol ? tid : ncol - 1];
    };
    auto stage_load = [&](int64_t jt, float4 (&yv)[YV], float (&sgv)[YV], float4 &cv) {
#pragma unroll
      for (int q = 0; q < YV; ++q) stage_load_y(jt, q, yv, sgv);
      stage_load_c(jt, cv);
    };
    auto stage_store = [&](int ybuf, int cbuf, int64_t jt, const float4 (&yv)[YV], const float (&sgv)[YV], const float4 &cv) {
      float *Yn = Ys + ybuf * Cfg::YT;
      const int64_t rem = N - jt;
      const int ncol = rem > BN ? BN : (int)rem;
#pragma unroll
      for (int q = 0; q < YV; ++q) {
        const int e4 = tid + NT * q;
        if (e4 < BN * Kp / 4) {
          const int jl = (e4 * 4) / Kp, kf = (e4 * 4) % Kp;
          const float sg = jl < ncol ? sgv[q] : 0.f;
          *reinterpret_cast<float4 *>(Yn + jl * KpS + kf) = make_float4(yv[q].x * sg, yv[q].y * sg, yv[q].z * sg, yv[q].w * sg);
        }
      }
      asm volatile("" ::"v"(cv.x), "v"(cv.y), "v"(cv.z), "v"(cv.w));
      if (tid < BN) {
        const bool livec = tid < ncol;
        Csg[cbuf * BN + tid] = livec ? cv.x : 0.f;
        Cmu[cbuf * BN + tid] = livec ? cv.y : 0.f;
        Cw[cbuf * BN + tid] = livec ? cv.z : 0.f;
        Cmt[cbuf * BN + tid] = livec ? __float_as_int(cv.w) : 3;
        if (MIXED) {
          const int kd = __float_as_int(cv.w) & 3;
          const unsigned m0 = (unsigned)__ballot(!livec || kd == 0), m1 = (unsigned)__ballot(!livec || kd == 1),
                         m2 = (unsigned)__ballot(!livec || kd == 2);
          if (tid == 0) Ck[cbuf] = m0 == 0xffffffffu ? 0 : (m1 == 0xffffffffu ? 1 : (m2 == 0xffffffffu ? 2 : 3));
        }
        if (bt_lds) {
          const int vw = (__float_as_int(cv.w) >> 2) - 1;
          const int vw0 = __builtin_amdgcn_readfirstlane(vw);
          const unsigned mv = (unsigned)__ballot(!livec || vw == vw0);
          if (tid == 0) Ck[2 + cbuf] = mv == 0xffffffffu ? vw0 : -2;
        }
      }
    };
    auto bt_e = [&](int q) { return (tid & 31) * 16 + (tid >> 5) + (NT / 32) * q; };
    auto bt_mu = [&](int64_t jt, int e) -> float { const int64_t j = jt + (e >> 4); return j < N ? a.colp[j].y : 0.f; };
    auto bt_store = [&](int e, const float2 &dt, float mu) __attribute__((always_inline)) {
      const int o = (e & 15) * 32 + (e >> 4);
      Btd[o] = dt.x;
      Btt[o] = dt.y + mu;
    };
    float4 gold[RV4];
    PmfDTile<DB> dcur[RBW];
    constexpr int DCH = PmfDTile<DB>::NCH;
    auto slab_map = [&](int q, int &so, int &e) -> bool {
      const int f = tid + NT * q;
      const bool in = f < BN * Kp / 4;
      const int ff = in ? f : 0;
      so = 4 * ff;
      e = ((ff % (BN * 8)) / 8) * Kp + 32 * (ff / (BN * 8)) + 4 * (ff % 8);
      return in;
    };
    auto slab_prefetch_one = [&](int64_t jt, int q) {
      const float *sb = myslab + jt * Kp;
      const int64_t rem = N - jt;
      if (HOIST) {
        gold[q] = pmf_load_stream(reinterpret_cast<const float4 *>(ho_at(sb, rem < BN ? ho_g[1][q] : ho_g[0][q])));
        return;
      }
      const int nel = (rem > BN ? BN : (int)rem) * Kp;
      int so, e;
      if (XW) e = xw_e;
      else slab_map(q, so, e);
      gold[q] = pmf_load_stream(reinterpret_cast<const float4 *>(sb + (e < nel ? e : (e % Kp))));
    };
    auto forward_reduce = [&](f32x16 (&acc)[RBW], int ybuf, int cbuf, bool do_red, int64_t jt_red) {
      const int cb0 = cbuf * BN + 4 * h;
#pragma unroll
      for (int r = 0; r < 16; ++r) {
        const float m0 = BATCH ? 0.f : Cmu[cb0 + (r & 3) + 8 * (r >> 2)];
#pragma unroll
        for (int rb = 0; rb < RBW; ++rb) acc[rb][r] = m0;
      }
      const float4 *yr = reinterpret_cast<const float4 *>(Ys + ybuf * Cfg::YT + l31 * KpS + h * (Kp / 2));
      const float4 *xr[RBW];
      float4 yv = yr[0], xv[RBW];
#pragma unroll
      for (int rb = 0; rb < RBW; ++rb) {
        xr[rb] = reinterpret_cast<const float4 *>(Xw[rb] + l31 * KpS + h * (Kp / 2));
        xv[rb] = XR ? xf[0] : xr[rb][0];
      }
      constexpr int NIT = KS / 4, RTOT = NW * RV4, RPI = (RTOT + NIT - 1) / NIT;
      float4 racc[RV4];
      int so[RV4], eo[RV4];
      bool in[RV4];
#pragma unroll
      for (int q = 0; q < RV4; ++q) {
        racc[q] = make_float4(0.f, 0.f, 0.f, 0.f);
        in[q] = slab_map(q, so[q], eo[q]);
      }
#pragma unroll
      for (int q = 0; q < NIT; ++q) {
        float4 yn = yv, xn[RBW];
#pragma unroll
        for (int rb = 0; rb < RBW; ++rb) xn[rb] = xv[rb];
        if (q + 1 < NIT) {
          yn = yr[q + 1];
#pragma unroll
          for (int rb = 0; rb < RBW; ++rb) xn[rb] = XR ? xf[XR ? q + 1 : 0] : xr[rb][q + 1];
        }
        if (do_red) {
#pragma unroll
          for (int z = 0; z < RPI; ++z) {
            const int idx = q * RPI + z;
            if (idx < RTOT) {
              const float4 v = *reinterpret_cast<const float4 *>(Sl + (idx / RV4) * SLAB + so[idx % RV4]);
              float4 &ra = racc[idx % RV4];
              ra.x += v.x; ra.y += v.y; ra.z += v.z; ra.w += v.w;
            }
          }
        }
#pragma unroll
        for (int rb = 0; rb < RBW; ++rb) acc[rb] = __builtin_amdgcn_mfma_f32_32x32x2f32(yv.x, xv[rb].x, acc[rb], 0, 0, 0);
#pragma unroll
        for (int rb = 0; rb < RBW; ++rb) acc[rb] = __builtin_amdgcn_mfma_f32_32x32x2f32(yv.y, xv[rb].y, acc[rb], 0, 0, 0);
#pragma unroll
        for (int rb = 0; rb < RBW; ++rb) acc[rb] = __builtin_amdgcn_mfma_f32_32x32x2f32(yv.z, xv[rb].z, acc[rb], 0, 0, 0);
#pragma unroll
        for (int rb = 0; rb < RBW; ++rb) acc[rb] = __builtin_amdgcn_mfma_f32_32x32x2f32(yv.w, xv[rb].w, acc[rb], 0, 0, 0);
        yv = yn;
#pragma unroll
        for (int rb = 0; rb < RBW; ++rb) xv[rb] = xn[rb];
        __builtin_amdgcn_sched_barrier(0);
      }
      if (do_red && (FULL || !(dbg & 8))) {
#pragma unroll
        for (int rb = 0; rb < RBW; ++rb) {
          dcur[rb].touch();
        }
        const int64_t rem = N - jt_red;
        const int nel = (rem > BN ? BN : (int)rem) * Kp;
        float *sb = myslab + jt_red * Kp;
#pragma unroll
        for (int q = 0; q < RV4; ++q) {
          float4 v = racc[q];
          const float sgj = Csg[(cbuf ^ 1) * BN + eo[q] / Kp];
          v.x *= sgj; v.y *= sgj; v.z *= sgj; v.w *= sgj;
          if (!slab_first) { v.x += gold[q].x; v.y += gold[q].y; v.z += gold[q].z; v.w += gold[q].w; }
          if (in[q] && eo[q] < nel) pmf_store_stream(reinterpret_cast<float4 *>(sb + eo[q]), v);
        }
      }
    };

    bool rows_in[RBW];
    int rb_u[RBW];
    uint32_t tflag[RBW];
#pragma unroll
    for (int rb = 0; rb < RBW; ++rb) {
      const int rb_raw = __builtin_amdgcn_readfirstlane((int)(row0[rb] >> 5));
      rows_in[rb] = rb_raw < a.nRB;
      rb_u[rb] = rows_in[rb] ? rb_raw : (int)a.nRB - 1;
      tflag[rb] = a.tflags[(col_begin >> 5) * a.nRB + rb_u[rb]];
#pragma unroll
      for (int q = 0; q < DCH; ++q) dcur[rb].load(a.D, (col_begin >> 5) * a.nRB + rb_u[rb], lane, q);
    }
    {
      float4 yv[YV], cv;
      float sgv[YV];
      stage_load(col_begin, yv, sgv, cv);
#pragma unroll
      for (int rb = 0; rb < RBW; ++rb)
#pragma unroll
        for (int q = 0; q < XV; ++q) {
          const int e4 = lane + 64 * q;
          const int il = (e4 * 4) / Kp, kf = (e4 * 4) % Kp;
          *reinterpret_cast<float4 *>(Xw[rb] + il * KpS + kf) = row0[rb] + il < M ? xv0[rb][q] : make_float4(0.f, 0.f, 0.f, 0.f);
        }
      stage_store(0, 0, col_begin, yv, sgv, cv);
      if (bt_lds) {
#pragma unroll
        for (int q = 0; q < NBT; ++q) {
          const int e = bt_e(q);
          bt_store(e, pmf_bt_entry(a, a.pm + rp * a.n_bv * 16, col_begin, e, pmf_bt_view(a, col_begin, e)), bt_mu(col_begin, e));
        }
        if (tid < a.n_bv * 16) Pm[tid] = a.pm[rp * a.n_bv * 16 + tid];
        if (h == 0)
#pragma unroll
          for (int rb = 0; rb < RBW; ++rb)
            for (int v = 0; v < a.n_bv; ++v) Bw0[rb * 512 + v * 32 + l31] = a.row_slot[(int64_t)v * M + irow_c[rb]];
      }
    }
    __syncthreads();
    if (XR) {
      const float4 *xr0 = reinterpret_cast<const float4 *>(Xw[0] + l31 * KpS + h * (Kp / 2));
#pragma unroll
      for (int q = 0; q < KS / 4; ++q) xf[XR ? q : 0] = xr0[q];
#pragma unroll
      for (int q = 0; q < 8 * NW; ++q) {
        const int p = q >> 3, u = (q >> 1) & 3, hi = q & 1;
        xg[XR ? q : 0] = *(lds_cptr)(uintptr_t)(xw_xa[u] + 4 * (p * Cfg::XP + 16 * hi * KpS));
      }
    }

    f32x16 acc[RBW];
    forward_reduce(acc, 0, 0, false, 0);

    for (int t = 0; t < ntiles; ++t) {
      const int par = t & 1;
      const int cur = NYB == 2 ? par : 0, nxt = NYB == 2 ? (par ^ 1) : 0;
      const int64_t j0 = col_begin + (int64_t)t * BN;
      const float *Yc = Ys + cur * Cfg::YT;
      const bool have_next = (t + 1 < ntiles);
      const int cb0 = par * BN + 4 * h;
      float4 ynext[YV], cnext;
      float2 btn[NBT];
      float btm[NBT];
      int btv[NBT];
      float sgnext[YV];
      PMF_STAMP(0);
      const float xw_sg = XW ? Csg[par * BN + xw_j] : 0.f;

      float lsum = 0.f;
      const int tkind = MIXED ? __builtin_amdgcn_readfirstlane(Ck[par]) : 0;
      const int tview = bt_lds ? __builtin_amdgcn_readfirstlane(Ck[2 + par]) : -1;
      float lnorm = 0.f;
      auto epi_reg = [&](int rb, int r, float dl, float th, float wj, int kmode, bool fast) __attribute__((always_inline)) {
        if (dbg & 4) return;
        float z = acc[rb][r];
        if (BATCH) z = fmaf(z, dl, th);
        float y = dcur[rb].get(r);
        if (kmode == PMF_NOISE_NORMAL) {
          if (!fast) y = (pmf_finite(y) && row_ok[rb]) ? y : z;
          const float d = z - y, g = wj * d;
          lnorm = fmaf(g, d, lnorm);
          acc[rb][r] = BATCH ? g * dl : g;
        } else {
          const bool ok = pmf_finite(y) && row_ok[rb];
          float l, g;
          if (kmode == 3) pmf_noise<MIXED>(Cmt[cb0 + (r & 3) + 8 * (r >> 2)] & 3, z, y, wj, a.htab + (j0 + 4 * h) * PMF_HT + PMF_HT * ((r & 3) + 8 * (r >> 2)), l, g);
          else pmf_noise(kmode, z, y, wj, nullptr, l, g);
          lsum += ok ? l : 0.f;
          acc[rb][r] = ok ? (BATCH ? g * dl : g) : 0.f;
        }
      };
      auto grp_load = [&](int rb, int c4, bool uni, const float *bdl, const float *btl, float4 &dl4, float4 &th4) __attribute__((always_inline)) {
        if (!BATCH) {
          th4 = make_float4(0.f, 0.f, 0.f, 0.f);
        } else if (bt_lds && uni) {
          dl4 = *reinterpret_cast<const float4 *>(bdl + 8 * c4);
          th4 = *reinterpret_cast<const float4 *>(btl + 8 * c4);
        } else {
          float dv[4], tv[4];
#pragma unroll
          for (int u = 0; u < 4; ++u) {
            const int cl = 8 * c4 + 4 * h + u;
            const int v = (Cmt[par * BN + cl] >> 2) - 1;
            dv[u] = 1.f;
            if (bt_lds) {
              const int bsr = v < 0 ? 15 : Bw0[rb * 512 + v * 32 + l31];
              dv[u] = Btd[bsr * 32 + cl];
              tv[u] = Btt[bsr * 32 + cl];
            } else {
              tv[u] = Cmu[par * BN + cl];
              if (v >= 0) {
                const int64_t vc0 = a.views[v].c0, vto = a.views[v].tab_off;
                const int vnb = a.views[v].nb;
                const int b = a.bor[(int64_t)v * M + irow_c[rb]];
                if (b >= 0) {
                  const float2 dt = a.btab[vto + (j0 + cl - vc0) * vnb + b];
                  dv[u] = dt.x;
                  tv[u] += dt.y;
                }
              }
            }
          }
          dl4 = make_float4(dv[0], dv[1], dv[2], dv[3]);
          th4 = make_float4(tv[0], tv[1], tv[2], tv[3]);
        }
      };
      const float4 *cw4 = reinterpret_cast<const float4 *>(Cw + cb0);
      auto f4get = [](const float4 &v, int u) { return u == 0 ? v.x : (u == 1 ? v.y : (u == 2 ? v.z : v.w)); };

      const int64_t jn = have_next ? j0 + BN : j0;
      constexpr int NOTH = YV + 1 + RV4 + (BATCH ? NBT : 0);
      constexpr int NVM = NOTH + (DCH + 1) * RBW;
      bool tile_fast[RBW];
#pragma unroll
      for (int rb = 0; rb < RBW; ++rb) tile_fast[rb] = rows_in[rb] && tflag[rb] != 0;
      auto vmem_op = [&](int i) {
        if (i == 0 && bt_lds) {
#pragma unroll
          for (int q = 0; q < NBT; ++q) btv[q] = pmf_bt_view(a, jn, bt_e(q));
        }
        if (i < YV) stage_load_y(jn, i, ynext, sgnext);
        else if (i == YV) stage_load_c(jn, cnext);
        else if (i < YV + 1 + RV4) { if (want_gy) slab_prefetch_one(j0, i - YV - 1); }
        else if (i < NOTH) {
          const int q = i - YV - 1 - RV4;
          if (bt_lds) { btn[q] = pmf_bt_entry(a, Pm, jn, bt_e(q), btv[q]); btm[q] = bt_mu(jn, bt_e(q)); }
        }
        else if (i < NVM) {
          const int rb = (i - NOTH) / (DCH + 1), q = (i - NOTH) % (DCH + 1);
          if (q < DCH) {
            if (FULL || !(dbg & 2)) dcur[rb].load(a.D, (jn >> 5) * a.nRB + rb_u[rb], lane, q);
          } else {
            tflag[rb] = a.tflags[(jn >> 5) * a.nRB + rb_u[rb]];
          }
        }
      };
      typedef float f32x2 __attribute__((ext_vector_type(2)));
#pragma unroll
      for (int rb = 0; rb < RBW; ++rb) {
        if (!BATCH && tile_fast[rb] && (!MIXED || tkind == 0)) {
          f32x2 ls2 = {0.f, 0.f};
          if (!(dbg & 4)) {
#pragma unroll
            for (int c4 = 0; c4 < 4; ++c4) {
              const float4 w4 = cw4[2 * c4];
#pragma unroll
              for (int p2 = 0; p2 < 2; ++p2) {
                const int r = 4 * c4 + 2 * p2;
                const f32x2 zz = {acc[rb][r], acc[rb][r + 1]}, yy = {dcur[rb].get(r), dcur[rb].get(r + 1)};
                const f32x2 ww = p2 == 0 ? f32x2{w4.x, w4.y} : f32x2{w4.z, w4.w};
                f32x2 dd;
                asm("v_pk_add_f32 %0, %1, %2 neg_lo:[0,1] neg_hi:[0,1]" : "=v"(dd) : "v"(zz), "v"(yy));
                const f32x2 gg = ww * dd;
                ls2 = gg * dd + ls2;
                acc[rb][r] = gg.x; acc[rb][r + 1] = gg.y;
              }
            }
          }
          lsum += 0.5f * (ls2.x + ls2.y);
        } else {
          int bs = 15;
          if (bt_lds && tview >= 0) bs = Bw0[rb * 512 + tview * 32 + l31];
          const float *bdl = Btd + bs * 32 + 4 * h, *btl = Btt + bs * 32 + 4 * h;
          auto epi_all = [&](int kmode, bool uni, bool fast) __attribute__((always_inline)) {
#pragma unroll
            for (int c4 = 0; c4 < 4; ++c4) {
              const float4 w4 = cw4[2 * c4];
              float4 dl4 = make_float4(1.f, 1.f, 1.f, 1.f), th4;
              grp_load(rb, c4, uni, bdl, btl, dl4, th4);
#pragma unroll
              for (int u = 0; u < 4; ++u) epi_reg(rb, 4 * c4 + u, f4get(dl4, u), f4get(th4, u), f4get(w4, u), kmode, fast);
            }
          };
          const bool uni = !bt_lds || tview != -2;
          if (!uni) epi_all(3, false, false);
          else if (!MIXED || tkind == 0) { if (BATCH && tile_fast[rb]) epi_all(PMF_NOISE_NORMAL, true, true); else epi_all(PMF_NOISE_NORMAL, true, false); }
          else if (tkind == 1) epi_all(PMF_NOISE_BERNOULLI, true, false);
          else if (tkind == 2) epi_all(PMF_NOISE_POISSON, true, false);
          else epi_all(3, true, false);
        }
        if (want_gy) {
#pragma unroll
          for (int c4 = 0; c4 < 4; ++c4)
            *reinterpret_cast<float4 *>((XW ? Sl + (par * NW + w) * 1024 : T[rb]) + l31 * 32 + 4 * ((2 * c4 + h) ^ (l31 & 7))) =
                make_float4(acc[rb][4 * c4], acc[rb][4 * c4 + 1], acc[rb][4 * c4 + 2], acc[rb][4 * c4 + 3]);
        }
      }
      PMF_STAMP(1);
      if (want_gx) {
        float bq[3][KB];
#pragma unroll
        for (int s0 = 0; s0 < 2; ++s0) {
          const float *yp = Yc + pmf_rowmap(s0, h) * KpS + l31;
#pragma unroll
          for (int kb = 0; kb < KB; ++kb) bq[s0][kb] = yp[32 * kb];
        }
        __builtin_amdgcn_sched_barrier(0);
#pragma unroll
        for (int s = 0; s < 16; ++s) {
          if (s + 2 < 16) {
            const float *yp = Yc + pmf_rowmap(s + 2, h) * KpS + l31;
#pragma unroll
            for (int kb = 0; kb < KB; ++kb) bq[(s + 2) % 3][kb] = yp[32 * kb];
          }
          if (s < NVM) vmem_op(s);
#pragma unroll
          for (int rb = 0; rb < RBW; ++rb)
#pragma unroll
            for (int kb = 0; kb < KB; ++kb)
              gx[rb][kb] = __builtin_amdgcn_mfma_f32_32x32x2f32(acc[rb][s], bq[s % 3][kb], gx[rb][kb], 0, 0, 0);
          __builtin_amdgcn_sched_barrier(0);
        }
#pragma unroll
        for (int i = 16; i < NVM; ++i) vmem_op(i);
      } else if (GM != 2) {
#pragma unroll
        for (int i = 0; i < NVM; ++i) vmem_op(i);
      }
      lossacc += (double)fmaf(0.5f, lnorm, lsum);

      PMF_STAMP(3);
      if (want_gy && !XW) {
        __builtin_amdgcn_wave_barrier();
        f32x16 gy[KB];
#pragma unroll
        for (int kb = 0; kb < KB; ++kb)
#pragma unroll
          for (int r = 0; r < 16; ++r) gy[kb][r] = 0.f;
#pragma unroll
        for (int s = 0; s < 16; ++s) {
          const int i = 2 * s + h;
          if (GM == 2 && s < NVM) vmem_op(s);
#pragma unroll
          for (int rb = 0; rb < RBW; ++rb) {
            const float av = T[rb][i * 32 + 4 * ((l31 >> 2) ^ (i & 7)) + (l31 & 3)];
#pragma unroll
            for (int kb = 0; kb < KB; ++kb)
              gy[kb] = __builtin_amdgcn_mfma_f32_32x32x2f32(av, Xw[rb][i * KpS + 32 * kb + l31], gy[kb], 0, 0, 0);
          }
        }
        if (GM == 2) {
#pragma unroll
          for (int i = 16; i < NVM; ++i) vmem_op(i);
        }
        if (!(dbg & 32)) {
#pragma unroll
          for (int kb = 0; kb < KB; ++kb)
#pragma unroll
            for (int r = 0; r < 16; ++r) Sw[kb * 1024 + pmf_rowmap(r, h) * 32 + l31] = gy[kb][r];
        } else {
          f32x16 keep = gy[0];
#pragma unroll
          for (int kb = 1; kb < KB; ++kb) keep += gy[kb];
          asm volatile("" ::"v"(keep));
        }
      }

      PMF_STAMP(4);
      if (NYB == 1) __syncthreads();
      stage_store(nxt, par ^ 1, jn, ynext, sgnext, cnext);
      PMF_STAMP(5);
      __syncthreads();
      PMF_STAMP(6);

      if (bt_lds) {
#pragma unroll
        for (int q = 0; q < NBT; ++q) bt_store(bt_e(q), btn[q], btm[q]);
      }
      slab_first = pidx == 0 || (pidx == 1 && ti0 + t < t0_first);
      if (XW) {
        typedef float f32x4 __attribute__((ext_vector_type(4)));
        constexpr int XW_RING = 8, XW_AHEAD = 6;
        const float *Gp = Sl + par * (NW * 1024);
        int xt_g[4];
        unsigned xt_xa[4];
        if (TIGHT) {
          int lo = lane;
          asm volatile("" : "+v"(lo));
#pragma unroll
          for (int u = 0; u < 4; ++u) {
            const int i = 4 * (lo >> 4) + u, j = 16 * (w & 1) + (lo & 15);
            xt_g[u] = i * 32 + 4 * ((j >> 2) ^ (i & 7)) + (j & 3);
            xt_xa[u] = (unsigned)(uintptr_t)(lds_cptr)(Xs + 4 * (lo >> 4) * KpS + 16 * (w >> 1) + (lo & 15) + u * KpS);
          }
        }
        float xa[XW_RING], xb[XW_RING];
        auto xw_read = [&](int q) __attribute__((always_inline)) {
          const int p = q >> 3, u = (q >> 1) & 3;
#pragma unroll
          for (int hi = 0; hi < 2; ++hi) {
            if (!XR) xa[(q + hi) % XW_RING] = *(lds_cptr)(uintptr_t)((TIGHT ? xt_xa[u] : xw_xa[u]) + 4 * (p * Cfg::XP + 16 * hi * KpS));
            xb[(q + hi) % XW_RING] = Gp[p * 1024 + (TIGHT ? xt_g[u] : xw_g[u]) + 512 * hi];
          }
        };
#pragma unroll
        for (int q = 0; q < XW_AHEAD; q += 2) xw_read(q);
        f32x4 gy0 = {0.f, 0.f, 0.f, 0.f}, gy1 = {0.f, 0.f, 0.f, 0.f};
        __builtin_amdgcn_sched_barrier(0);
#pragma unroll
        for (int q = 0; q < 8 * NW; q += 2) {
          if (q + XW_AHEAD < 8 * NW) xw_read(q + XW_AHEAD);
          gy0 = __builtin_amdgcn_mfma_f32_16x16x4f32(XR ? xg[XR ? q : 0] : xa[q % XW_RING], xb[q % XW_RING], gy0, 0, 0, 0);
          gy1 = __builtin_amdgcn_mfma_f32_16x16x4f32(XR ? xg[XR ? q + 1 : 0] : xa[(q + 1) % XW_RING], xb[(q + 1) % XW_RING], gy1, 0, 0, 0);
          __builtin_amdgcn_sched_barrier(0);
        }
        dcur[0].touch();
        const int64_t rem = N - j0;
        const int nel = (rem > BN ? BN : (int)rem) * Kp;
        float4 v = make_float4((gy0[0] + gy1[0]) * xw_sg, (gy0[1] + gy1[1]) * xw_sg, (gy0[2] + gy1[2]) * xw_sg, (gy0[3] + gy1[3]) * xw_sg);
        if (!slab_first) { v.x += gold[0].x; v.y += gold[0].y; v.z += gold[0].z; v.w += gold[0].w; }
        if (xw_e < nel) pmf_store_stream(reinterpret_cast<float4 *>(myslab + j0 * Kp + xw_e), v);
        PMF_STAMP(4);
        forward_reduce(acc, nxt, par ^ 1, false, 0);
        PMF_STAMP(8);
        if (bt_lds) __syncthreads();
        PMF_STAMP(9);
      } else {
        if (FULL || have_next) forward_reduce(acc, nxt, par ^ 1, want_gy && !(dbg & 1), j0);
        else if (want_gy && !(dbg & 1)) { f32x16 dummy[RBW]; forward_reduce(dummy, nxt, par ^ 1, true, j0); }
        PMF_STAMP(8);
        if ((GM != 1 || bt_lds) && !(dbg & 16)) __syncthreads();
        PMF_STAMP(9);
      }
    }
    if (XW && !bt_lds) __syncthreads();

    PMF_STAMP(10);
    if (want_gx) {
      float *gp = a.gx_part + (int64_t)gx_slot * a.gx_slot_stride + (int64_t)(w * RBW) * 32 * Kp + l31;
#pragma unroll
      for (int rb = 0; rb < RBW; ++rb)
#pragma unroll
        for (int kb = 0; kb < KB; ++kb)
#pragma unroll
          for (int r = 0; r < 16; ++r) gp[(rb * 32 + pmf_rowmap(r, h)) * Kp + 32 * kb] = gx[rb][kb][r];
    }
    ++gx_slot;
    PMF_STAMP(11);
  }
#pragma unroll
  for (int off = 32; off > 0; off >>= 1) lossacc += __shfl_xor(lossacc, off, 64);
  if (lane == 0) red[w] = lossacc;
  __syncthreads();
  if (tid == 0) {
    double s = 0.0;
    for (int q = 0; q < NW; ++q) s += red[q];
    a.loss_partial[wg] = s;
  }
#ifdef PMF_STAMPS
  st_acc[14] = __builtin_amdgcn_s_memtime() - st_t0;
  st_acc[15] = __builtin_amdgcn_s_memrealtime() - st_r0;
  if (a.stamps && (threadIdx.x & 63) == 0) {
    for (int q = 0; q < 16; ++q) a.stamps[((int64_t)blockIdx.x * NW + (threadIdx.x >> 6)) * 16 + q] = st_acc[q];
  }
#endif
}
```

pathmatfac.jl_amd/csrc/pmf_pass.hip:

```cpp
#include "pmf_ctx.h"

__global__ void k_tile_flags(const void *__restrict__ D, int64_t ntiles, uint32_t *__restrict__ flags, int bf16) {
  const int64_t t = blockIdx.x;
  if (t >= ntiles) return;
  bool ok;
  if (bf16) {
    const uint2 v = reinterpret_cast<const uint2 *>(reinterpret_cast<const uint16_t *>(D) + t * 1024)[threadIdx.x];
    ok = (v.x & 0x7f80u) != 0x7f80u && (v.x & 0x7f800000u) != 0x7f800000u && (v.y & 0x7f80u) != 0x7f80u && (v.y & 0x7f800000u) != 0x7f800000u;
  } else {
    const float4 v = reinterpret_cast<const float4 *>(reinterpret_cast<const float *>(D) + t * 1024)[threadIdx.x];
    ok = fabsf(v.x) <= 3.402823466e38f && fabsf(v.y) <= 3.402823466e38f && fabsf(v.z) <= 3.402823466e38f && fabsf(v.w) <= 3.402823466e38f;
  }
  const int all_ok = __syncthreads_and(ok ? 1 : 0);
  if (threadIdx.x == 0) flags[t] = all_ok ? 1u : 0u;
}

static int ensure_tile_flags(pmf_ctx *c) {
  if (c->tflags_valid) return 0;
  const int64_t ntiles = c->nRB * (c->D_Npad / 32);
  PMFCHK(c->tflags.ensure((size_t)ntiles, false));
  if (ntiles > 0x7fffffff) return pmf_fail("too many tiles");
  k_tile_flags<<<(unsigned)ntiles, 256, 0, c->stream>>>(c->D, ntiles, c->tflags, c->store == PMF_STORE_BF16);
  HIPCHK(hipGetLastError());
  c->tflags_valid = true;
  return 0;
}

__global__ __launch_bounds__(64) void k_gy_reduce(const float *__restrict__ slabs, int64_t stride,
                                                  const int32_t *__restrict__ c_off, const int32_t *__restrict__ c_idx,
                                                  int Kp, int64_t N, float *__restrict__ gY, int ct0,
                                                  const float4 *__restrict__ colscale) {
  const int ct = blockIdx.x;
  const int64_t e0 = (int64_t)(ct0 + ct) * 32 * Kp;
  const int64_t rem = (int64_t)Kp * N - e0;
  const int nel = rem > 32 * Kp ? 32 * Kp : (int)rem;
  const int q = (blockIdx.y * 64 + threadIdx.x) * 4;
  if (q >= nel) return;
  const float *base = slabs + e0 + q;
  const int c0 = c_off[ct], n = c_off[ct + 1] - c0;
  const int32_t *ci = c_idx + c0;
  float4 a0 = make_float4(0.f, 0.f, 0.f, 0.f), a1 = a0, a2 = a0, a3 = a0;
  int c = 0;
  for (; c + 4 <= n; c += 4) {
    const float4 v0 = *reinterpret_cast<const float4 *>(base + (int64_t)ci[c] * stride);
    const float4 v1 = *reinterpret_cast<const float4 *>(base + (int64_t)ci[c + 1] * stride);
    const float4 v2 = *reinterpret_cast<const float4 *>(base + (int64_t)ci[c + 2] * stride);
    const float4 v3 = *reinterpret_cast<const float4 *>(base + (int64_t)ci[c + 3] * stride);
    a0.x += v0.x; a0.y += v0.y; a0.z += v0.z; a0.w += v0.w;
    a1.x += v1.x; a1.y += v1.y; a1.z += v1.z; a1.w += v1.w;
    a2.x += v2.x; a2.y += v2.y; a2.z += v2.z; a2.w += v2.w;
    a3.x += v3.x; a3.y += v3.y; a3.z += v3.z; a3.w += v3.w;
  }
  for (; c < n; ++c) {
    const float4 v = *reinterpret_cast<const float4 *>(base + (int64_t)ci[c] * stride);
    a0.x += v.x; a0.y += v.y; a0.z += v.z; a0.w += v.w;
  }
  const float sg = colscale ? colscale[(e0 + q) / Kp].x : 1.f;
  *reinterpret_cast<float4 *>(gY + e0 + q) =
      make_float4(((a0.x + a1.x) + (a2.x + a3.x)) * sg, ((a0.y + a1.y) + (a2.y + a3.y)) * sg, ((a0.z + a1.z) + (a2.z + a3.z)) * sg,
                  ((a0.w + a1.w) + (a2.w + a3.w)) * sg);
}

__global__ __launch_bounds__(256) void k_gx_reduce(const float *__restrict__ part, int64_t slot_stride,
                                                   const int32_t *__restrict__ gx_off, const int32_t *__restrict__ gx_idx,
                                                   int64_t panel_floats, int64_t total_floats, float *__restrict__ gX) {
  const int rp = blockIdx.x;
  const int64_t q = ((int64_t)blockIdx.y * 256 + threadIdx.x) * 4;
  if (q >= panel_floats) return;
  const int64_t e = (int64_t)rp * panel_floats + q;
  if (e >= total_floats) return;
  const int c0 = gx_off[rp], n = gx_off[rp + 1] - c0;
  const int32_t *ci = gx_idx + c0;
  const float *base = part + q;
  float4 a0 = make_float4(0.f, 0.f, 0.f, 0.f), a1 = a0;
  int c = 0;
  for (; c + 2 <= n; c += 2) {
    const float4 v0 = *reinterpret_cast<const float4 *>(base + (int64_t)ci[c] * slot_stride);
    const float4 v1 = *reinterpret_cast<const float4 *>(base + (int64_t)ci[c + 1] * slot_stride);
    a0.x += v0.x; a0.y += v0.y; a0.z += v0.z; a0.w += v0.w;
    a1.x += v1.x; a1.y += v1.y; a1.z += v1.z; a1.w += v1.w;
  }
  if (c < n) {
    const float4 v = *reinterpret_cast<const float4 *>(base + (int64_t)ci[c] * slot_stride);
    a0.x += v.x; a0.y += v.y; a0.z += v.z; a0.w += v.w;
  }
  *reinterpret_cast<float4 *>(gX + e) = make_float4(a0.x + a1.x, a0.y + a1.y, a0.z + a1.z, a0.w + a1.w);
}

static void noise_tile_weights(int KB, bool split, bool batch, int64_t &w_gauss, int64_t &w_bern, int64_t &w_pois, int64_t &w_hinge) {
  static const int64_t wb_exact[4] = {26, 22, 20, 20}, wb_split[4] = {31, 30, 24, 24};
  static const int64_t we_exact[4] = {6, 6, 5, 4}, we_split[4] = {12, 8, 6, 6};
  w_bern = (split ? wb_split : wb_exact)[KB - 1];
  if (getenv("PMF_W_BERN")) w_bern = std::max(16, atoi(getenv("PMF_W_BERN")));
  w_pois = 16 + ((w_bern - 16) * 5 + 3) / 6;
  if (getenv("PMF_W_POIS")) w_pois = std::max(16, atoi(getenv("PMF_W_POIS")));
  w_hinge = w_pois;
  if (getenv("PMF_W_HINGE")) w_hinge = std::max(16, atoi(getenv("PMF_W_HINGE")));
  int64_t w_batch = batch ? (split ? we_split : we_exact)[KB - 1] : 0;
  if (batch && getenv("PMF_W_BATCH")) w_batch = std::max(0, atoi(getenv("PMF_W_BATCH")));
  w_gauss = 16 + w_batch;
  w_bern += w_batch;
  w_pois += w_batch;
  w_hinge += w_batch;
}

static int compute_work_split(pmf_ctx *c, WorkSplit &ws, int grid, int64_t n_rp, int64_t ct0, int64_t n_ct, int64_t tps, int64_t n_cseg, bool split) {
  int64_t w_gauss, w_bern, w_pois, w_hinge;
  noise_tile_weights(c->KB, split, c->n_bv > 0, w_gauss, w_bern, w_pois, w_hinge);
  const int64_t key[11] = {c->M, c->N, c->Kp, grid, n_rp, tps, n_cseg, c->kind_version, ct0, n_ct,
                           c->mixed ? ((w_gauss * 64 + w_bern) * 64 + w_pois) * 64 + w_hinge : 0};
  if (ws.wg_begin && memcmp(key, ws.key, sizeof(key)) == 0) return 0;
  std::vector<int64_t> tw((size_t)n_ct, w_gauss);
  if (c->mixed && (int64_t)c->h_kind.size() == c->N) {
    for (int64_t ct = 0; ct < n_ct; ++ct) {
      int64_t wmax = w_gauss;
      for (int64_t j = (ct0 + ct) * 32; j < std::min<int64_t>(c->N, (ct0 + ct) * 32 + 32); ++j) {
        const int k = c->h_kind[(size_t)j];
        wmax = std::max<int64_t>(wmax, k == PMF_NOISE_BERNOULLI ? w_bern : (k == PMF_NOISE_POISSON ? w_pois : (k == PMF_NOISE_SQ_HINGE ? w_hinge : w_gauss)));
      }
      tw[(size_t)ct] = wmax;
    }
  }
  std::vector<int64_t> seg_t0((size_t)n_cseg), seg_nt((size_t)n_cseg), seg_w((size_t)n_cseg), seg_pref((size_t)n_cseg + 1, 0);
  for (int64_t cs = 0; cs < n_cseg; ++cs) {
    seg_t0[(size_t)cs] = cs * tps;
    seg_nt[(size_t)cs] = cs == n_cseg - 1 ? n_ct - cs * tps : tps;
    int64_t w = 0;
    for (int64_t t = 0; t < seg_nt[(size_t)cs]; ++t) w += tw[(size_t)(seg_t0[(size_t)cs] + t)];
    seg_w[(size_t)cs] = w;
    seg_pref[(size_t)cs + 1] = seg_pref[(size_t)cs] + w * n_rp;
  }
  const int64_t W = seg_pref[(size_t)n_cseg], T = n_rp * n_ct;
  std::vector<int64_t> wb((size_t)grid + 1, 0);
  for (int g = 1; g < grid; ++g) {
    const int64_t target = (int64_t)((__int128)W * g / grid);
    int64_t cs = 0;
    while (cs + 1 < n_cseg && seg_pref[(size_t)cs + 1] <= target) ++cs;
    int64_t rem = target - seg_pref[(size_t)cs];
    const int64_t rp = std::min<int64_t>(n_rp - 1, rem / seg_w[(size_t)cs]);
    rem -= rp * seg_w[(size_t)cs];
    int64_t ti = 0;
    while (ti + 1 < seg_nt[(size_t)cs] && rem >= tw[(size_t)(seg_t0[(size_t)cs] + ti)]) { rem -= tw[(size_t)(seg_t0[(size_t)cs] + ti)]; ++ti; }
    int64_t idx = cs * n_rp * tps + rp * seg_nt[(size_t)cs] + ti;
    idx = std::max(idx, wb[(size_t)g - 1]);
    wb[(size_t)g] = std::min(idx, T);
  }
  wb[(size_t)grid] = T;
  std::vector<int32_t> h_off((size_t)n_ct + 1, 0), h_idx;
  for (int64_t ct = 0; ct < n_ct; ++ct) {
    const int64_t cs = std::min<int64_t>(ct / tps, n_cseg - 1);
    const int64_t tps_cs = seg_nt[(size_t)cs], ti = ct - cs * tps;
    const int64_t s0 = cs * n_rp * tps, s1 = s0 + n_rp * tps_cs;
    int g_lo = (int)(std::upper_bound(wb.begin(), wb.begin() + grid, s0) - wb.begin()) - 1;
    if (g_lo < 0) g_lo = 0;
    for (int g = g_lo; g < grid && wb[(size_t)g] < s1; ++g) {
      const int64_t lo = std::max(wb[(size_t)g], s0), hi = std::min(wb[(size_t)g + 1], s1);
      if (hi <= lo) continue;
      const int64_t first = (lo - s0) % tps_cs;
      const int64_t d = (ti - first + tps_cs) % tps_cs;
      if (d < hi - lo) h_idx.push_back(g);
    }
    h_off[(size_t)ct + 1] = (int32_t)h_idx.size();
  }
  if (h_idx.empty()) h_idx.push_back(0);
  ws.h_piece_base.assign((size_t)grid, 0);
  ws.piece_rp.clear();
  const int64_t seg_block = n_rp * tps;
  for (int g = 0; g < grid; ++g) {
    ws.h_piece_base[(size_t)g] = (int32_t)ws.piece_rp.size();
    for (int64_t widx = wb[(size_t)g]; widx < wb[(size_t)g + 1];) {
      const int64_t cs = std::min<int64_t>(widx / seg_block, n_cseg - 1);
      const int64_t tps_cs = seg_nt[(size_t)cs];
      const int64_t rem = widx - cs * seg_block;
      const int64_t rp = rem / tps_cs, ti0 = rem - rp * tps_cs;
      widx += std::min<int64_t>(tps_cs - ti0, wb[(size_t)g + 1] - widx);
      ws.piece_rp.push_back((int32_t)rp);
    }
  }
  PMFCHK(ws.wg_begin.alloc((size_t)grid + 1, false));
  PMFCHK(ws.c_off.alloc((size_t)n_ct + 1, false));
  PMFCHK(ws.c_idx.alloc(h_idx.size(), false));
  PMFCHK(ws.piece_base.alloc((size_t)grid, false));
  PMFCHK(ws.d_piece_base_abs.alloc((size_t)grid, false));
  HIPCHK(hipMemcpyAsync(ws.wg_begin, wb.data(), sizeof(int64_t) * ((size_t)grid + 1), hipMemcpyHostToDevice, c->stream));
  HIPCHK(hipMemcpyAsync(ws.c_off, h_off.data(), sizeof(int32_t) * h_off.size(), hipMemcpyHostToDevice, c->stream));
  HIPCHK(hipMemcpyAsync(ws.c_idx, h_idx.data(), sizeof(int32_t) * h_idx.size(), hipMemcpyHostToDevice, c->stream));
  HIPCHK(hipStreamSynchronize(c->stream));
  memcpy(ws.key, key, sizeof(key));
  ws.grid = grid;
  ws.serial = ++c->split_serial;
  return 0;
}

#ifdef PMF_STAMPS
static unsigned long long *g_stamps = nullptr;
extern "C" int pmf_debug_stamps(unsigned long long *out, int n) {
  if (!g_stamps) return -1;
  return hipMemcpy(out, g_stamps, sizeof(unsigned long long) * (size_t)n, hipMemcpyDeviceToHost) == hipSuccess ? 0 : -1;
}
#endif

int harvest_events(pmf_ctx *c) {
  for (size_t e = 0; e < c->ev_used; ++e) {
    float ms = 0.f;
    if (hipEventElapsedTime(&ms, c->ev_pool[e].first, c->ev_pool[e].second) == hipSuccess) {
      c->kernel_ms_sum += ms;
      c->kernel_launches += 1;
    }
  }
  c->ev_used = 0;
  return 0;
}

static int ensure_panel_slots(pmf_ctx *c, int BM, PanelSlots **out) {
  PanelSlots &ps = c->pslots[BM == 128 ? 0 : (BM == 256 ? 1 : 2)];
  *out = &ps;
  if (ps.serial == c->views_serial && ps.BM == BM) return 0;
  const int64_t n_rp = (c->M + BM - 1) / BM;
  std::vector<uint8_t> pm((size_t)(n_rp * c->n_bv * 16), 255), rs((size_t)((int64_t)c->n_bv * c->M), 15);
  bool ok = true;
  std::vector<int> slot_of;
  for (int v = 0; v < c->n_bv && ok; ++v) {
    if ((int64_t)c->h_bor[(size_t)v].size() != c->M) { ok = false; break; }
    const int32_t *bor = c->h_bor[(size_t)v].data();
    slot_of.assign((size_t)std::max<int>(c->views[v].nb, 1), -1);
    for (int64_t rp = 0; rp < n_rp && ok; ++rp) {
      uint8_t *pmv = pm.data() + (rp * c->n_bv + v) * 16;
      int used = 0;
      const int64_t i1 = std::min<int64_t>(c->M, (rp + 1) * BM);
      for (int64_t i = rp * BM; i < i1; ++i) {
        const int b = bor[i];
        if (b < 0) continue;
        if (b > 254) { ok = false; break; }
        int sl = slot_of[(size_t)b];
        if (sl < 0) {
          if (used == 15) { ok = false; break; }
          sl = used++;
          slot_of[(size_t)b] = sl;
          pmv[sl] = (uint8_t)b;
        }
        rs[(size_t)((int64_t)v * c->M + i)] = (uint8_t)sl;
      }
      for (int q = 0; q < used; ++q) slot_of[pmv[q]] = -1;
    }
  }
  ps.ok = ok;
  ps.BM = BM;
  ps.serial = c->views_serial;
  if (ok) {
    PMFCHK(upload_new(ps.pm, pm.data(), pm.size()));
    PMFCHK(upload_new(ps.row_slot, rs.data(), rs.size()));
  }
  return 0;
}

enum FusedImages { IMG_NONE, IMG_SB, IMG_SB4, IMG_SB8 };
struct FusedFamily {
  int kernel;
  int KB, NW, RBW;
  int max_bv;
  FusedImages img;
  int img_kb;
  int xblk, yblk;
  int nblk;
  PmfFusedLaunch *launch[2];
  constexpr int BM() const { return 32 * NW * RBW; }
};
static constexpr FusedFamily fused_families[] = {
    {0, 1, 8,             2,             PMF_MAXV,          IMG_NONE, 0, 0,               0,               1,               {pmf_launch_fused_exact_12, pmf_launch_fused_exact_12_bf16}},
    {0, 1, 8,             1,             PMF_MAXV,          IMG_NONE, 0, 0,               0,               1,               {pmf_launch_fused_exact_11, pmf_launch_fused_exact_11_bf16}},
    {0, 2, 8,             1,             PMF_MAXV,          IMG_NONE, 0, 0,               0,               1,               {pmf_launch_fused_exact_21, pmf_launch_fused_exact_21_bf16}},
    {0, 3, 4,             1,             PMF_MAXV,          IMG_NONE, 0, 0,               0,               1,               {pmf_launch_fused_exact_31, pmf_launch_fused_exact_31_bf16}},
    {0, 4, 4,             1,             PMF_MAXV,          IMG_NONE, 0, 0,               0,               1,               {pmf_launch_fused_exact_41, pmf_launch_fused_exact_41_bf16}},
    {1, 1, SbCfg<1>::NW,  1,             SbCfg<1>::max_bv,  IMG_SB,   1, SbCfg<1>::BLK,   SbCfg<1>::BLK,   1,               {pmf_launch_fused_sb_1, pmf_launch_fused_sb_1_bf16}},
    {1, 2, SbCfg<2>::NW,  1,             SbCfg<2>::max_bv,  IMG_SB,   2, SbCfg<2>::BLK,   SbCfg<2>::BLK,   1,               {pmf_launch_fused_sb_2, pmf_launch_fused_sb_2_bf16}},
    {2, 2, 4,             2,             Sb2Cfg::max_bv,    IMG_SB,   2, SbCfg<2>::BLK,   SbCfg<2>::BLK,   1,               {pmf_launch_fused_sb2, pmf_launch_fused_sb2_bf16}},
    {4, 3, Sb4Cfg<3>::NW, 1,             Sb4Cfg<3>::max_bv, IMG_SB4,  4, Sb4Cfg<3>::XBLK, Sb4Cfg<3>::YBLK, 1,               {pmf_launch_fused_sb4_3, pmf_launch_fused_sb4_3_bf16}},
    {4, 4, Sb4Cfg<4>::NW, 1,             Sb4Cfg<4>::max_bv, IMG_SB4,  4, Sb4Cfg<4>::XBLK, Sb4Cfg<4>::YBLK, 1,               {pmf_launch_fused_sb4_4, pmf_launch_fused_sb4_4_bf16}},
    {8, 2, Sb8Cfg<2>::NW, Sb8Cfg<2>::RB, Sb8Cfg<2>::max_bv, IMG_SB8,  2, Sb8Cfg<2>::XBLK, Sb8Cfg<2>::YBLK, Sb8Cfg<2>::NBLK, {pmf_launch_fused_sb8_2, pmf_launch_fused_sb8_2_bf16}},
    {8, 4, Sb8Cfg<4>::NW, Sb8Cfg<4>::RB, Sb8Cfg<4>::max_bv, IMG_SB8,  4, Sb8Cfg<4>::XBLK, Sb8Cfg<4>::YBLK, Sb8Cfg<4>::NBLK, {pmf_launch_fused_sb8_4, pmf_launch_fused_sb8_4_bf16}},
};
constexpr int PMF_XSB_PAD = 16;
static_assert([] { for (const FusedFamily &f : fused_families) if (f.nblk - 1 > PMF_XSB_PAD) return false; return true; }(), "PMF_XSB_PAD");

static const FusedFamily *find_family(int kernel, int KB, int RBW = 0) {
  for (const FusedFamily &f : fused_families)
    if (f.kernel == kernel && f.KB == KB && (RBW == 0 || f.RBW == RBW)) return &f;
  return nullptr;
}

FusedGeom fused_geometry(pmf_ctx *c, bool want_gx, bool want_gy, bool allow_chunks) {
  FusedGeom g;
  auto batch_fits = [&](const FusedFamily *f) {
    if (c->n_bv == 0) return true;
    PanelSlots *ps = nullptr;
    if (!c->btd_ok || c->n_bv > f->max_bv || ensure_panel_slots(c, f->BM(), &ps) != 0 || !ps || !ps->ok) return false;
    g.ps = ps;
    return true;
  };
  if (c->precision == PMF_PREC_BF16X3 && (want_gx || want_gy) && !getenv("PMF_DEBUG_FLAGS")) {
    static const bool sb2_off = getenv("PMF_SB2") && atoi(getenv("PMF_SB2")) == 0;
    const char *e8 = getenv("PMF_SB8");
    const int m8 = e8 ? atoi(e8) : 1;
    const bool both = want_gx && want_gy;
    int base = 0;
    bool sb8 = false;
    switch (c->KB) {
      case 1: base = 1; break;
      case 2: base = sb2_off ? 1 : 2; sb8 = both && m8 != 0 && m8 != 4; break;
      case 3: base = 4; break;
      case 4: base = 4; sb8 = both && m8 != 0; break;
    }
    const FusedFamily *f8 = sb8 ? find_family(8, c->KB) : nullptr, *fb = find_family(base, c->KB);
    g.fam = f8 && batch_fits(f8) ? f8 : (fb && batch_fits(fb) ? fb : nullptr);
    g.bmode = g.fam && c->n_bv > 0 ? 1 : 0;
  }
  if (!g.fam) {
    const char *rbwenv = getenv("PMF_RBW");
    g.fam = find_family(0, c->KB, c->KB == 1 && c->n_bv == 0 && !(rbwenv && atoi(rbwenv) == 1) ? 2 : 1);
    if (!g.fam) return g;
    if (c->n_bv > 0) g.bmode = batch_fits(g.fam) ? 1 : 2;
  }
  g.n_rp = (c->M + g.fam->BM() - 1) / g.fam->BM();
  g.n_ct_all = (c->N + PMF_BN - 1) / PMF_BN;
  int reserve = c->comm.nranks > 1 ? c->comm.reserve_cus : 0;
  if (const char *e = getenv("PMF_RESERVE_CUS")) reserve = std::max(0, std::min(atoi(e), c->n_cu / 2));
  g.grid_max = std::max(1, c->n_cu - reserve);
  int S = 1;
  if (allow_chunks && want_gy) {
    S = c->n_chunks_req > 0 ? c->n_chunks_req : 1;
    if (c->n_chunks_req <= 0 && c->comm.nranks > 1) {
      const char *bw = getenv("PMF_COMM_ALGBW_GBPS");
      const double algbw = (bw && atof(bw) > 0 ? atof(bw) : 60.0) * 1e9;
      const int64_t Mref = c->comm.m_mean > 0 ? c->comm.m_mean : c->M;
      const double bytes = 4.0 * (double)c->Kp * (double)c->N;
      const double t_pass = 6.0 * (double)Mref * (double)c->N * (double)c->Kp / (c->precision == PMF_PREC_BF16X3 ? 200e12 : 115e12);
      S = 2;
      while (S < 4 && 30e-6 + bytes / S / algbw > t_pass * (S - 1) / S) ++S;
      constexpr int64_t REF_PANEL = 256;
      const int64_t n_rp_ref = (Mref + REF_PANEL - 1) / REF_PANEL;
      const int64_t min_tiles = 32ll * std::max(1, c->n_cu - c->comm.reserve_cus);
      while (S > 1 && (n_rp_ref * g.n_ct_all) / S < min_tiles) --S;
    }
    S = (int)std::max<int64_t>(1, std::min<int64_t>(std::min<int64_t>(S, PMF_MAX_CHUNKS), g.n_ct_all));
  }
  g.S = S;
  for (int s = 0; s < S; ++s) {
    g.ct0[s] = g.n_ct_all * s / S;
    g.nct[s] = g.n_ct_all * (s + 1) / S - g.ct0[s];
  }
  return g;
}

static void chunk_segments(pmf_ctx *c, const FusedGeom &g, int s, int &grid, int64_t &tps, int64_t &n_cseg) {
  const int64_t n_ct = g.nct[s], n_rp = g.n_rp;
  grid = (int)std::min<int64_t>(n_rp * n_ct, (int64_t)g.grid_max);
  const double tiles_per_wg = (double)(n_rp * n_ct) / grid;
  const double a_cost = tiles_per_wg * 8e-6;
  const double b_cost = (double)grid * (double)c->Kp * (double)n_ct * 32.0 * 4.0 / ((double)n_ct * 4e12);
  tps = (int64_t)std::llround(std::sqrt(a_cost / std::max(b_cost, 1e-12)));
  {
    const char *ts = getenv("PMF_TPS_SCALE");
    if (ts) tps = (int64_t)std::llround((double)tps * atof(ts));
  }
  tps = std::max<int64_t>(std::min<int64_t>(8, n_ct), std::min<int64_t>(tps, n_ct));
  n_cseg = std::max<int64_t>(1, n_ct / tps);
}

int prepare_fused_pass(pmf_ctx *c, const FusedGeom &g, bool want_gx, bool want_gy) {
  if (!g.fam) return pmf_fail("unsupported KB=%d", c->KB);
  const FusedFamily &f = *g.fam;
  if ((int)c->splits.size() < g.S) c->splits.resize((size_t)g.S);
  int64_t grid_sum = 0, serial_sum = 0;
  for (int s = 0; s < g.S; ++s) {
    int grid; int64_t tps, n_cseg;
    chunk_segments(c, g, s, grid, tps, n_cseg);
    PMFCHK(compute_work_split(c, c->splits[(size_t)s], grid, g.n_rp, g.ct0[s], g.nct[s], tps, n_cseg, f.kernel != 0));
    grid_sum += grid;
  }
  serial_sum = c->split_serial * PMF_MAX_CHUNKS + g.S;
  PMFCHK(ensure_loss_partials(c, grid_sum));
  const int64_t slab_stride = (int64_t)c->Kp * c->N;
  const size_t gy_need = (size_t)g.grid_max * (size_t)slab_stride + (size_t)PMF_BN * (size_t)c->Kp;
  if (want_gy) PMFCHK(c->gy_slabs.ensure(gy_need, false));
  if (want_gx && serial_sum != c->gx_serial) {
    std::vector<std::vector<int32_t>> lists((size_t)g.n_rp);
    int32_t base = 0;
    for (int s = 0; s < g.S; ++s) {
      WorkSplit &ws = c->splits[(size_t)s];
      ws.slot_base = base;
      for (size_t p = 0; p < ws.piece_rp.size(); ++p) lists[(size_t)ws.piece_rp[p]].push_back(base + (int32_t)p);
      std::vector<int32_t> abs(ws.h_piece_base);
      for (auto &v : abs) v += base;
      PMFCHK(ws.d_piece_base_abs.upload(abs.data(), abs.size()));
      base += (int32_t)ws.piece_rp.size();
    }
    std::vector<int32_t> off((size_t)g.n_rp + 1, 0), idx;
    for (int64_t rp = 0; rp < g.n_rp; ++rp) {
      idx.insert(idx.end(), lists[(size_t)rp].begin(), lists[(size_t)rp].end());
      off[(size_t)rp + 1] = (int32_t)idx.size();
    }
    if (idx.empty()) idx.push_back(0);
    PMFCHK(upload_new(c->gx_off, off.data(), off.size()));
    PMFCHK(upload_new(c->gx_idx, idx.data(), idx.size()));
    c->gx_serial = serial_sum;
  }
  if (want_gx) {
    size_t pieces = 0;
    for (int s = 0; s < g.S; ++s) pieces += c->splits[(size_t)s].piece_rp.size();
    PMFCHK(c->gx_part.ensure(pieces * (size_t)f.BM() * (size_t)c->Kp, false));
  }
  PMFCHK(ensure_tile_flags(c));
  if (f.img != IMG_NONE) {
    size_t xblk = 0, yblk = 0;
    for (const FusedFamily &o : fused_families)
      if (o.img_kb == f.img_kb) { xblk = std::max<size_t>(xblk, o.xblk); yblk = std::max<size_t>(yblk, o.yblk); }
    const size_t xb = ((size_t)c->nRB + PMF_XSB_PAD) * xblk, yb = (size_t)g.n_ct_all * yblk;
    PMFCHK(c->xsb.ensure(xb, true));
    PMFCHK(c->ysb.ensure(yb, false));
    if (f.img == IMG_SB8) {
      PMFCHK(c->sb8_scale.ensure((size_t)(1 + PMF_MAX_CHUNKS), false));
      PMFCHK(c->sb8_max.ensure((size_t)(1 + PMF_MAX_CHUNKS), true));
    }
  }
  return 0;
}

int fused_pass_extents(pmf_ctx *c, const FusedGeom &g, bool want_gx, bool want_gy, PassExtent *out) {
  const FusedFamily &f = *g.fam;
  const int64_t Kp = c->Kp, Npad = g.n_ct_all * PMF_BN;
  int64_t pieces = 0, grid_sum = 0, grid_top = 0;
  for (int s = 0; s < g.S; ++s) {
    const WorkSplit &ws = c->splits[(size_t)s];
    pieces += (int64_t)ws.piece_rp.size();
    grid_sum += ws.grid;
    grid_top = std::max<int64_t>(grid_top, ws.grid);
  }
  const bool bt = g.bmode == 1;
  int nbs_shift = 0;
  while ((1 << nbs_shift) < c->nbs) ++nbs_shift;
  const int64_t gx_slot_stride = (int64_t)f.BM() * Kp, slab_stride = Kp * c->N;
  int n = 0;
  out[n++] = {"gx_part", want_gx ? pieces * gx_slot_stride * 4 : 0, (int64_t)c->gx_part.bytes()};
  out[n++] = {"gy_slabs", want_gy ? ((grid_top - 1) * slab_stride + (f.img == IMG_SB8 ? Npad * Kp : slab_stride)) * 4 : 0,
              (int64_t)c->gy_slabs.bytes()};
  out[n++] = {"xsb", f.img != IMG_NONE ? (c->nRB + f.nblk - 1) / f.nblk * f.nblk * f.xblk : 0, (int64_t)c->xsb.bytes()};
  out[n++] = {"ysb", f.img != IMG_NONE ? g.n_ct_all * f.yblk : 0, (int64_t)c->ysb.bytes()};
  out[n++] = {"btd", bt ? (Npad << nbs_shift) * (int64_t)sizeof(float2) : 0, (int64_t)c->btd.bytes()};
  out[n++] = {"colview", bt ? Npad : 0, (int64_t)c->colview.bytes()};
  out[n++] = {"tflags", g.n_ct_all * c->nRB * 4, (int64_t)c->tflags.bytes()};
  out[n++] = {"loss_partial", grid_sum * 8, (int64_t)c->loss_partial.bytes()};
  out[n++] = {"pm", bt ? g.n_rp * c->n_bv * 16 : 0, bt ? (int64_t)g.ps->pm.bytes() : 0};
  out[n++] = {"row_slot", bt ? (int64_t)c->n_bv * c->M : 0, bt ? (int64_t)g.ps->row_slot.bytes() : 0};
  static_assert(PMF_PASS_EXTENTS == 10, "fused_pass_extents");
  return n;
}
int check_pass_extents(const PassExtent *e, int n) {
  for (int i = 0; i < n; ++i)
    if (e[i].need > e[i].cap)
      return pmf_fail("data pass refused: it addresses %lld bytes of %s, %lld are allocated", (long long)e[i].need, e[i].name,
                      (long long)e[i].cap);
  return 0;
}
int guard_fused_pass(pmf_ctx *c, const FusedGeom &g, bool want_gx, bool want_gy) {
  PassExtent e[PMF_PASS_EXTENTS];
  return check_pass_extents(e, fused_pass_extents(c, g, want_gx, want_gy, e));
}

static int sb8_split(pmf_ctx *c, const FusedFamily &f, const float *src, const float4 *colp, int64_t n, int64_t nblk, int slot,
                     int transposed, char *out) {
  Sb8ScaleArgs sa = {src, colp, n, c->Kp, c->sb8_max + slot, c->sb8_scale + slot};
  PMFCHK(pmf_launch_sb8_scale(c->stream, sa));
  Sb8SplitArgs sp = {src, colp, c->sb8_scale + slot, n, nblk, transposed, out};
  return pmf_launch_sb8_split(c->stream, sp, f.KB);
}
static int sb_split_x(pmf_ctx *c, const FusedFamily &f) {
  if (f.img == IMG_SB8) {
    return sb8_split(c, f, c->P[0].p, nullptr, c->M, (c->nRB + f.nblk - 1) / f.nblk * f.nblk, 0, 1, c->xsb);
  }
  if (f.img == IMG_SB4) {
    Sb4SplitArgs s4 = {c->P[0].p, nullptr, c->M, c->nRB, c->Kp, 1, c->xsb};
    return pmf_launch_sb4_split(c->stream, s4);
  }
  SbSplitArgs sx = {c->P[0].p, nullptr, c->M, c->nRB, c->xsb};
  return f.KB == 1 ? pmf_launch_sb_split_1(c->stream, sx) : pmf_launch_sb_split_2(c->stream, sx);
}
static int sb_split_y(pmf_ctx *c, const FusedFamily &f, int64_t ct0, int64_t nct, int chunk) {
  const int64_t c0 = ct0 * 32;
  const float *src = c->P[1].p + c0 * c->Kp;
  char *out = c->ysb + (size_t)ct0 * (size_t)f.yblk;
  if (f.img == IMG_SB8) return sb8_split(c, f, src, c->colp + c0, std::min<int64_t>(c->N - c0, nct * 32), nct, 1 + chunk, 0, out);
  if (f.img == IMG_SB4) {
    Sb4SplitArgs s4 = {src, c->colp + c0, c->N - c0, nct, c->Kp, 0, out};
    return pmf_launch_sb4_split(c->stream, s4);
  }
  SbSplitArgs sy = {src, c->colp + c0, c->N - c0, nct, out};
  return f.KB == 1 ? pmf_launch_sb_split_1(c->stream, sy) : pmf_launch_sb_split_2(c->stream, sy);
}

int launch_fused_chunk(pmf_ctx *c, const FusedGeom &g, int s, bool want_gx, bool want_gy) {
  const FusedFamily &f = *g.fam;
  WorkSplit &ws = c->splits[(size_t)s];
  const int grid = ws.grid;
  int grid_dummy; int64_t tiles_per_seg, n_cseg;
  chunk_segments(c, g, s, grid_dummy, tiles_per_seg, n_cseg);
  const int64_t n_ct = g.nct[s], n_rp = g.n_rp;
  const int64_t slab_stride = (int64_t)c->Kp * c->N;
  int64_t loss_off = 0;
  for (int q = 0; q < s; ++q) loss_off += c->splits[(size_t)q].grid;
  FusedArgs a;
  memset(&a, 0, sizeof(a));
  a.tflags = c->tflags;
  a.wg_begin = ws.wg_begin;
  a.D = c->D; a.X = c->P[0].p; a.Y = c->P[1].p; a.gX = c->P[0].g; a.gY = c->P[1].g;
  a.colp = c->colp; a.htab = c->htab; a.bor = c->bor; a.btab = c->btab; a.loss_partial = c->loss_partial + loss_off;
  a.btd = g.bmode == 1 ? c->btd : nullptr; a.n_bv = c->n_bv;
  if (g.bmode == 1) {
    a.pm = g.ps->pm; a.row_slot = g.ps->row_slot; a.colview = c->colview;
    a.nbs_shift = 0;
    while ((1 << a.nbs_shift) < c->nbs) ++a.nbs_shift;
  }
  c->last_bmode = g.bmode;
  a.nRB = c->nRB; a.gy_slabs = c->gy_slabs; a.slab_stride = slab_stride; a.n_rp = n_rp;
  a.M = c->M; a.N = c->N; a.n_tiles = n_rp * n_ct; a.tps = (int)tiles_per_seg; a.n_ct = (int)n_ct; a.n_cseg = (int)n_cseg;
  a.want_gx = want_gx; a.want_gy = want_gy;
  a.ct0 = (int32_t)g.ct0[s];
  a.gx_part = c->gx_part; a.piece_base = ws.d_piece_base_abs; a.gx_slot_stride = (int64_t)f.BM() * c->Kp;
  {
    const char *dbg = getenv("PMF_DEBUG_FLAGS");
    a.dbg = dbg ? atoi(dbg) : 0;
  }
#ifdef PMF_STAMPS
  {
    static DevBuf<unsigned long long> d_stamps;
    PMFCHK(d_stamps.ensure((size_t)16 * 8 * 1024, false));
    HIPCHK(hipMemsetAsync(d_stamps, 0, sizeof(unsigned long long) * 16 * 8 * 1024, c->stream));
    a.stamps = d_stamps;
    g_stamps = d_stamps;
  }
#endif
  a.views = c->d_views;
  const bool batch = c->n_bv > 0;
  if (f.img != IMG_NONE) {
    if (s == 0) PMFCHK(sb_split_x(c, f));
    PMFCHK(sb_split_y(c, f, g.ct0[s], n_ct, s));
    a.Xsb = c->xsb; a.Ysb = c->ysb;
    if (f.img == IMG_SB8) { a.sb_scale_x = c->sb8_scale; a.sb_scale_y = c->sb8_scale + 1 + s; }
  }
  if (c->ev_used == c->ev_pool.size()) {
    if (c->ev_pool.size() >= 4096) {
      HIPCHK(hipStreamSynchronize(c->stream));
      harvest_events(c);
    } else {
      hipEvent_t e0, e1;
      HIPCHK(hipEventCreate(&e0));
      HIPCHK(hipEventCreate(&e1));
      c->ev_pool.emplace_back(e0, e1);
    }
  }
  auto &ev = c->ev_pool[c->ev_used++];
  HIPCHK(hipEventRecord(ev.first, c->stream));
  c->last_kernel = f.kernel;
  pmf_last_xreg = 0;
  const int rc = f.launch[c->store == PMF_STORE_BF16](&c->dyn_lds, c->stream, a, grid, batch, c->mixed);
  c->last_xreg = pmf_last_xreg;
  if (f.kernel != 0) c->sb_launches += 1;
  PMFCHK(rc);
  HIPCHK(hipEventRecord(ev.second, c->stream));
  if (want_gy && !(a.dbg & 8)) {
    k_gy_reduce<<<dim3((unsigned)n_ct, (unsigned)(32 * c->Kp / 256)), 64, 0, c->stream>>>(c->gy_slabs, slab_stride, ws.c_off, ws.c_idx,
                                                                                      c->Kp, c->N, c->P[1].g, (int)g.ct0[s],
                                                                                      f.img == IMG_SB8 ? c->colp : nullptr);
    HIPCHK(hipGetLastError());
  }
  if (want_gx && s == g.S - 1) {
    const int64_t panel = (int64_t)f.BM() * c->Kp;
    k_gx_reduce<<<dim3((unsigned)g.n_rp, (unsigned)((panel / 4 + 255) / 256)), 256, 0, c->stream>>>(
        c->gx_part, panel, c->gx_off, c->gx_idx, panel, (int64_t)c->Kp * c->M, c->P[0].g);
    HIPCHK(hipGetLastError());
  }
  return 0;
}

int launch_fused(pmf_ctx *c, bool want_gx, bool want_gy) {
  const FusedGeom g = fused_geometry(c, want_gx, want_gy, c->n_chunks_req > 0);
  PMFCHK(prepare_fused_pass(c, g, want_gx, want_gy));
  PMFCHK(guard_fused_pass(c, g, want_gx, want_gy));
  for (int s = 0; s < g.S; ++s) PMFCHK(launch_fused_chunk(c, g, s, want_gx, want_gy));
  return 0;
}

thread_local int pmf_last_xreg = 0;
extern "C" int pmf_debug_last_kernel(pmf_ctx *c, int *kernel) {
  if (!c) return pmf_fail("null context");
  if (kernel) *kernel = c->last_kernel;
  return 0;
}

extern "C" int pmf_debug_last_path(pmf_ctx *c, int *bmode, int *layer_path, int *slots, int *xreg) {
  if (!c) return pmf_fail("null context");
  if (xreg) *xreg = c->last_xreg;
  if (bmode) *bmode = c->last_bmode;
  if (layer_path) *layer_path = c->last_layer_path;
  if (slots) *slots = c->nbs;
  return 0;
}

extern "C" int pmf_debug_pass_extents(pmf_ctx *c, int update_X, int update_Y, const int64_t *cap_override, int n_max,
                                      const char **names, int64_t *need, int64_t *capacity, int *n_out) {
  PMFCHK(ctx_bind(c));
  PMFCHK(check_ready(c));
  if (!c->prepared) PMFCHK(prepare(c));
  const bool want_gx = update_X != 0, want_gy = update_Y != 0;
  const FusedGeom g = fused_geometry(c, want_gx, want_gy, c->n_chunks_req > 0);
  PMFCHK(prepare_fused_pass(c, g, want_gx, want_gy));
  PassExtent e[PMF_PASS_EXTENTS];
  const int n = fused_pass_extents(c, g, want_gx, want_gy, e);
  if (n_max < n) return pmf_fail("pmf_debug_pass_extents: room for %d entries, %d needed", n_max, n);
  for (int i = 0; i < n; ++i) {
    if (cap_override && cap_override[i] >= 0) e[i].cap = cap_override[i];
    if (names) names[i] = e[i].name;
    if (need) need[i] = e[i].need;
    if (capacity) capacity[i] = e[i].cap;
  }
  if (n_out) *n_out = n;
  return cap_override ? check_pass_extents(e, n) : 0;
}
```

Measured before the change: 32.51 iters/s.

## Add specialized plain-tile loop skipping per-tile flag checks and ragged handling

Precomputes a per-row-panel prefix-sum table of tiles whose data blocks are all fully observed. In the fused kernel, runs of interior tiles found clean through that table go through a compile-time PLAIN variant of the tile loop. That variant drops the tile-flag loads, the ragged-column masking and the slab-first logic, and uses a single hoisted address set. It also pins LDS addresses for the Y reads in the gx path to a lane base register. The aim is fewer VMEM ops and less branching and register pressure, at the cost of code size from three loop instantiations, an extra table kernel and memory, and new debug APIs.

New measurement: 32.86 iters/s (median of 6 runs). 1.01x the previous value.

```diff
diff --git a/include/pmf_hip.h b/include/pmf_hip.h
--- a/include/pmf_hip.h
+++ b/include/pmf_hip.h
@@ -180,7 +180,8 @@
 int pmf_comm_info(pmf_ctx *ctx, int *rank, int *nranks, int *transport, int *n_chunks, int *reserved_cus,
                   int64_t *n_collectives);
 
-int pmf_debug_last_path(pmf_ctx *ctx, int *bmode, int *layer_path, int *slots, int *xreg);
+int pmf_debug_last_path(pmf_ctx *ctx, int *bmode, int *layer_path, int *slots, int *xreg, int64_t *plain_tiles);
+int pmf_debug_plain_table(pmf_ctx *ctx, int32_t *out, int64_t cap, int64_t *n_rp, int64_t *n_ct);
 int pmf_debug_last_kernel(pmf_ctx *ctx, int *kernel);
 
 #define PMF_PASS_EXTENTS_MAX 16
diff --git a/pathmatfac.jl_amd/_lib.py b/pathmatfac.jl_amd/_lib.py
--- a/pathmatfac.jl_amd/_lib.py
+++ b/pathmatfac.jl_amd/_lib.py
@@ -103,7 +103,7 @@
     "pmf_set_precision", "pmf_get_precision",
     "pmf_comm_get_unique_id", "pmf_comm_init", "pmf_comm_init_host", "pmf_comm_destroy", "pmf_comm_set_chunks",
     "pmf_comm_info", "pmf_comm_allreduce", "pmf_get_opt_state", "pmf_fsard_update_A", "pmf_debug_last_path", "pmf_debug_last_kernel",
-    "pmf_debug_pass_extents", "pmf_debug_live_bytes",
+    "pmf_debug_pass_extents", "pmf_debug_live_bytes", "pmf_debug_plain_table",
     "pmf_add_xreg_network", "pmf_add_yreg_network", "pmf_get_reg_network_state", "pmf_add_xreg_l1", "pmf_add_yreg_l1",
     "pmf_impute", "pmf_impute_device", "pmf_impute_entries", "pmf_debug_impute_offset",
     "pmf_loss", "pmf_fit_lbfgs", "pmf_debug_lbfgs_direction",
@@ -834,8 +834,16 @@
 
     def last_path(self):
         b, l, s, x = C.c_int(0), C.c_int(0), C.c_int(0), C.c_int(0)
-        self._chk(self.lib.pmf_debug_last_path(self._h, C.byref(b), C.byref(l), C.byref(s), C.byref(x)))
-        return dict(bmode=b.value, layer_path=l.value, slots=s.value, xreg=x.value)
+        pt = C.c_int64(0)
+        self._chk(self.lib.pmf_debug_last_path(self._h, C.byref(b), C.byref(l), C.byref(s), C.byref(x), C.byref(pt)))
+        return dict(bmode=b.value, layer_path=l.value, slots=s.value, xreg=x.value, plain_tiles=pt.value)
+
+    def plain_table(self):
+        n_rp, n_ct = C.c_int64(0), C.c_int64(0)
+        self._chk(self.lib.pmf_debug_plain_table(self._h, None, C.c_int64(0), C.byref(n_rp), C.byref(n_ct)))
+        out = np.zeros((n_rp.value, n_ct.value + 1), np.int32)
+        self._chk(self.lib.pmf_debug_plain_table(self._h, out.ctypes.data_as(C.c_void_p), C.c_int64(out.size), None, None))
+        return out
 
     def last_kernel(self):
         k = C.c_int(0)
diff --git a/pathmatfac.jl_amd/csrc/pmf_common.h b/pathmatfac.jl_amd/csrc/pmf_common.h
--- a/pathmatfac.jl_amd/csrc/pmf_common.h
+++ b/pathmatfac.jl_amd/csrc/pmf_common.h
@@ -81,6 +81,10 @@
   int64_t gx_slot_stride;
   const float *sb_scale_x, *sb_scale_y;
   const float *htab;
+  const int32_t *ptab;
+  int32_t ptab_stride;
+  int32_t plain;
+  int32_t *plain_count;
 };
 
 __device__ __forceinline__ int pmf_rowmap(int r, int h) { return (r & 3) + 8 * (r >> 2) + 4 * h; }
diff --git a/pathmatfac.jl_amd/csrc/pmf_ctx.h b/pathmatfac.jl_amd/csrc/pmf_ctx.h
--- a/pathmatfac.jl_amd/csrc/pmf_ctx.h
+++ b/pathmatfac.jl_amd/csrc/pmf_ctx.h
@@ -145,6 +145,10 @@
   int64_t D_M = 0, D_Npad = 0, nRB = 0;
   DevBuf<uint32_t> tflags;
   bool tflags_valid = false;
+  DevBuf<int32_t> ptab;
+  int64_t ptab_bm = 0, ptab_n_rp = 0, ptab_n_ct = 0;
+  DevBuf<int32_t> plain_count;
+  int64_t last_plain_n = -1;
   int store = PMF_STORE_F32;
   ParamBuf P[6];
   int n_bv = 0;
@@ -328,7 +332,7 @@
 int prepare_fused_pass(pmf_ctx *c, const FusedGeom &g, bool want_gx, bool want_gy);
 int launch_fused_chunk(pmf_ctx *c, const FusedGeom &g, int s, bool want_gx, bool want_gy);
 struct PassExtent { const char *name; int64_t need, cap; };
-constexpr int PMF_PASS_EXTENTS = 10;
+constexpr int PMF_PASS_EXTENTS = 12;
 int fused_pass_extents(pmf_ctx *c, const FusedGeom &g, bool want_gx, bool want_gy, PassExtent *out);
 int check_pass_extents(const PassExtent *e, int n);
 int guard_fused_pass(pmf_ctx *c, const FusedGeom &g, bool want_gx, bool want_gy);
diff --git a/pathmatfac.jl_amd/csrc/pmf_fused.hip.inc b/pathmatfac.jl_amd/csrc/pmf_fused.hip.inc
--- a/pathmatfac.jl_amd/csrc/pmf_fused.hip.inc
+++ b/pathmatfac.jl_amd/csrc/pmf_fused.hip.inc
@@ -17,6 +17,10 @@
 #ifndef PMF_NW4_WAVES
 #define PMF_NW4_WAVES 1
 #endif
+#ifndef PMF_Y1BASE
+#define PMF_Y1BASE 1
+#endif
+template <bool B> struct PmfFlag { static constexpr bool value = B; };
 template <int KB, int NW, int RBW, int BMODE, bool MIXED, int GM, bool DB, bool XW = false, bool XR = false>
 __global__ __launch_bounds__(64 * NW, (NW == 8 ? 2 : PMF_NW4_WAVES)) void pmf_fused_kernel(const FusedArgs a) {
   using Cfg = FusedCfg<KB, NW, RBW>;
@@ -80,14 +84,16 @@
     const int i = 4 * (lane >> 4) + u;
     xw_g[u] = i * 32 + 4 * ((xw_j >> 2) ^ (i & 7)) + (xw_j & 3);
     xw_xa[u] = (unsigned)(uintptr_t)(lds_cptr)(Xs + xw_x + u * KpS);
-    if (XW && !TIGHT) asm volatile("" : "+v"(xw_xa[u]));
+    if (XW && !TIGHT && !XR) asm volatile("" : "+v"(xw_xa[u]));
   }
 
   constexpr bool HOIST = KB == 2 && NW == 8 && RBW == 1 && GM != 3 && !TIGHT && (XW || GM != 0 || BMODE == 0);
-  unsigned ho_y[2][YV], ho_s[2][YV], ho_c[2], ho_g[2][RV4];
+  constexpr bool PLAINB = XW && XR && HOIST && !MIXED && !BATCH;
+  constexpr int HOZ = PLAINB ? 1 : 2;
+  unsigned ho_y[HOZ][YV], ho_s[HOZ][YV], ho_c[HOZ], ho_g[HOZ][RV4];
   if (HOIST) {
 #pragma unroll
-    for (int z = 0; z < 2; ++z) {
+    for (int z = 0; z < HOZ; ++z) {
       const int ncol = z == 0 || N % BN == 0 ? BN : (int)(N % BN);
 #pragma unroll
       for (int q = 0; q < YV; ++q) {
@@ -113,7 +119,13 @@
       }
     }
   }
-  auto ho_at = [](const void *base, unsigned off) { return reinterpret_cast<const char *>(base) + off; };
+  constexpr bool Y1BASE = PLAINB && PMF_Y1BASE != 0;
+  unsigned g2_lane = (unsigned)(uintptr_t)(lds_cptr)(Ys + 4 * h * KpS + l31);
+  if (Y1BASE) asm volatile("" : "+v"(g2_lane));
+  auto ho_at = [](const void *base, unsigned &off) {
+    if (PLAINB) asm volatile("" : "+v"(off));
+    return reinterpret_cast<const char *>(base) + off;
+  };
 #ifdef PMF_STAMPS
   unsigned long long st_acc[16] = {0, 0, 0, 0, 0, 0, 0, 0, 0, 0, 0, 0, 0, 0, 0, 0};
   unsigned long long st_prev = __builtin_amdgcn_s_memtime();
@@ -125,6 +137,7 @@
   float *myslab = a.gy_slabs + (int64_t)wg * a.slab_stride;
   const int64_t seg_block = a.n_rp * a.tps;
   double lossacc = 0.0;
+  int n_plain = 0;
   int seg_cur = -1, pidx = 0, t0_first = 0;
   int gx_slot = (GM == 2) ? 0 : a.piece_base[wg];
   for (int64_t widx = w_begin; widx < w_end;) {
@@ -138,6 +151,21 @@
     widx += ntiles;
     if (cs != seg_cur) { seg_cur = cs; pidx = 0; t0_first = ti0; } else { ++pidx; }
     bool slab_first = true;
+    int pl_b = ntiles, pl_e = ntiles;
+    int32_t pl_c0 = 0, pl_c1 = 0;
+    if (PLAINB && a.plain) {
+      const int64_t c_abs = (int64_t)a.ct0 + (int64_t)cs * a.tps + ti0;
+      const bool rag = (c_abs + ntiles) * PMF_BN > N;
+      pl_b = pidx == 0 ? ntiles : (pidx == 1 ? (t0_first - ti0 < 0 ? 0 : (t0_first - ti0 < ntiles ? t0_first - ti0 : ntiles)) : 0);
+      pl_e = rag ? ntiles - 2 : ntiles;
+      if (pl_b < pl_e) {
+        const int32_t *pt = a.ptab + rp * a.ptab_stride;
+        pl_c0 = pt[c_abs + pl_b];
+        pl_c1 = pt[c_abs + (rag ? ntiles - 1 : ntiles)];
+      } else {
+        pl_b = pl_e = ntiles;
+      }
+    }
     const int64_t col_begin = ((int64_t)a.ct0 + (int64_t)cs * a.tps + ti0) * BN;
     int64_t row0[RBW], irow_c[RBW];
     bool row_ok[RBW];
@@ -171,14 +199,14 @@
     float4 xf[XR ? KS / 4 : 1];
     float xg[XR ? 8 * NW : 1];
 
-    auto stage_load_y = [&](int64_t jt, int q, float4 (&yv)[YV], float (&sgv)[YV]) {
+    auto stage_load_y = [&](int64_t jt, int q, float4 (&yv)[YV], float (&sgv)[YV], bool plain = false) {
       const float *yb = a.Y + jt * Kp;
       const float4 *cb = a.colp + jt;
       const int64_t rem = N - jt;
-      if (HOIST) {
-        const bool rag = rem < BN;
-        yv[q] = *reinterpret_cast<const float4 *>(ho_at(yb, rag ? ho_y[1][q] : ho_y[0][q]));
-        sgv[q] = *reinterpret_cast<const float *>(ho_at(cb, rag ? ho_s[1][q] : ho_s[0][q]));
+      if (HOIST && !(PLAINB && !plain && rem < BN)) {
+        const bool rag = HOZ == 2 && rem < BN;
+        yv[q] = *reinterpret_cast<const float4 *>(ho_at(yb, rag ? ho_y[HOZ - 1][q] : ho_y[0][q]));
+        sgv[q] = *reinterpret_cast<const float *>(ho_at(cb, rag ? ho_s[HOZ - 1][q] : ho_s[0][q]));
         return;
       }
       const int ncol = rem > BN ? BN : (int)rem;
@@ -189,11 +217,11 @@
       yv[q] = *reinterpret_cast<const float4 *>(yb + e4 * 4);
       sgv[q] = cb[jl].x;
     };
-    auto stage_load_c = [&](int64_t jt, float4 &cv) {
+    auto stage_load_c = [&](int64_t jt, float4 &cv, bool plain = false) {
       const float4 *cb = a.colp + jt;
       const int64_t rem = N - jt;
-      if (HOIST) {
-        cv = *reinterpret_cast<const float4 *>(ho_at(cb, rem < BN ? ho_c[1] : ho_c[0]));
+      if (HOIST && !(PLAINB && !plain && rem < BN)) {
+        cv = *reinterpret_cast<const float4 *>(ho_at(cb, HOZ == 2 && rem < BN ? ho_c[HOZ - 1] : ho_c[0]));
         return;
       }
       const int ncol = rem > BN ? BN : (int)rem;
@@ -204,22 +232,22 @@
       for (int q = 0; q < YV; ++q) stage_load_y(jt, q, yv, sgv);
       stage_load_c(jt, cv);
     };
-    auto stage_store = [&](int ybuf, int cbuf, int64_t jt, const float4 (&yv)[YV], const float (&sgv)[YV], const float4 &cv) {
+    auto stage_store = [&](int ybuf, int cbuf, int64_t jt, const float4 (&yv)[YV], const float (&sgv)[YV], const float4 &cv, bool plain = false) {
       float *Yn = Ys + ybuf * Cfg::YT;
       const int64_t rem = N - jt;
-      const int ncol = rem > BN ? BN : (int)rem;
+      const int ncol = plain || rem > BN ? BN : (int)rem;
 #pragma unroll
       for (int q = 0; q < YV; ++q) {
         const int e4 = tid + NT * q;
         if (e4 < BN * Kp / 4) {
           const int jl = (e4 * 4) / Kp, kf = (e4 * 4) % Kp;
-          const float sg = jl < ncol ? sgv[q] : 0.f;
+          const float sg = plain || jl < ncol ? sgv[q] : 0.f;
           *reinterpret_cast<float4 *>(Yn + jl * KpS + kf) = make_float4(yv[q].x * sg, yv[q].y * sg, yv[q].z * sg, yv[q].w * sg);
         }
       }
       asm volatile("" ::"v"(cv.x), "v"(cv.y), "v"(cv.z), "v"(cv.w));
       if (tid < BN) {
-        const bool livec = tid < ncol;
+        const bool livec = plain || tid < ncol;
         Csg[cbuf * BN + tid] = livec ? cv.x : 0.f;
         Cmu[cbuf * BN + tid] = livec ? cv.y : 0.f;
         Cw[cbuf * BN + tid] = livec ? cv.z : 0.f;
@@ -256,11 +284,11 @@
       e = ((ff % (BN * 8)) / 8) * Kp + 32 * (ff / (BN * 8)) + 4 * (ff % 8);
       return in;
     };
-    auto slab_prefetch_one = [&](int64_t jt, int q) {
+    auto slab_prefetch_one = [&](int64_t jt, int q, bool plain = false) {
       const float *sb = myslab + jt * Kp;
       const int64_t rem = N - jt;
-      if (HOIST) {
-        gold[q] = pmf_load_stream(reinterpret_cast<const float4 *>(ho_at(sb, rem < BN ? ho_g[1][q] : ho_g[0][q])));
+      if (HOIST && !(PLAINB && !plain && rem < BN)) {
+        gold[q] = pmf_load_stream(reinterpret_cast<const float4 *>(ho_at(sb, HOZ == 2 && rem < BN ? ho_g[HOZ - 1][q] : ho_g[0][q])));
         return;
       }
       const int nel = (rem > BN ? BN : (int)rem) * Kp;
@@ -400,7 +428,16 @@
     f32x16 acc[RBW];
     forward_reduce(acc, 0, 0, false, 0);
 
-    for (int t = 0; t < ntiles; ++t) {
+    int t_plain = ntiles, t_pend = ntiles;
+    if (PLAINB && a.plain) {
+      const bool run = pl_b < pl_e && pl_c0 == pl_c1;
+      t_plain = __builtin_amdgcn_readfirstlane(run ? pl_b : ntiles);
+      t_pend = __builtin_amdgcn_readfirstlane(run ? pl_e : ntiles);
+      n_plain += t_pend - t_plain;
+    }
+    auto tile_loop = [&](auto plain_flag, const int t_begin, const int t_end) __attribute__((always_inline)) {
+    constexpr bool PLAIN = decltype(plain_flag)::value;
+    for (int t = t_begin; t < t_end; ++t) {
       const int par = t & 1;
       const int cur = NYB == 2 ? par : 0, nxt = NYB == 2 ? (par ^ 1) : 0;
       const int64_t j0 = col_begin + (int64_t)t * BN;
@@ -478,24 +515,25 @@
 
       const int64_t jn = have_next ? j0 + BN : j0;
       constexpr int NOTH = YV + 1 + RV4 + (BATCH ? NBT : 0);
-      constexpr int NVM = NOTH + (DCH + 1) * RBW;
+      constexpr int DPR = DCH + (PLAIN ? 0 : 1);
+      constexpr int NVM = NOTH + DPR * RBW;
       bool tile_fast[RBW];
 #pragma unroll
-      for (int rb = 0; rb < RBW; ++rb) tile_fast[rb] = rows_in[rb] && tflag[rb] != 0;
+      for (int rb = 0; rb < RBW; ++rb) tile_fast[rb] = PLAIN || (rows_in[rb] && tflag[rb] != 0);
       auto vmem_op = [&](int i) {
         if (i == 0 && bt_lds) {
 #pragma unroll
           for (int q = 0; q < NBT; ++q) btv[q] = pmf_bt_view(a, jn, bt_e(q));
         }
-        if (i < YV) stage_load_y(jn, i, ynext, sgnext);
-        else if (i == YV) stage_load_c(jn, cnext);
-        else if (i < YV + 1 + RV4) { if (want_gy) slab_prefetch_one(j0, i - YV - 1); }
+        if (i < YV) stage_load_y(jn, i, ynext, sgnext, PLAIN);
+        else if (i == YV) stage_load_c(jn, cnext, PLAIN);
+        else if (i < YV + 1 + RV4) { if (want_gy) slab_prefetch_one(j0, i - YV - 1, PLAIN); }
         else if (i < NOTH) {
           const int q = i - YV - 1 - RV4;
           if (bt_lds) { btn[q] = pmf_bt_entry(a, Pm, jn, bt_e(q), btv[q]); btm[q] = bt_mu(jn, bt_e(q)); }
         }
         else if (i < NVM) {
-          const int rb = (i - NOTH) / (DCH + 1), q = (i - NOTH) % (DCH + 1);
+          const int rb = (i - NOTH) / DPR, q = (i - NOTH) % DPR;
           if (q < DCH) {
             if (FULL || !(dbg & 2)) dcur[rb].load(a.D, (jn >> 5) * a.nRB + rb_u[rb], lane, q);
           } else {
@@ -557,19 +595,23 @@
       PMF_STAMP(1);
       if (want_gx) {
         float bq[3][KB];
+        unsigned g2_y = g2_lane + (unsigned)(cur * Cfg::YT * 4);
+        if (Y1BASE) asm volatile("" : "+v"(g2_y));
+        auto g2_read = [&](int s, int kb) -> float {
+          if (Y1BASE) return *(const volatile __attribute__((address_space(3))) float *)(uintptr_t)(g2_y + 4 * (pmf_rowmap(s, 0) * KpS + 32 * kb));
+          return (Yc + pmf_rowmap(s, h) * KpS + l31)[32 * kb];
+        };
 #pragma unroll
         for (int s0 = 0; s0 < 2; ++s0) {
-          const float *yp = Yc + pmf_rowmap(s0, h) * KpS + l31;
-#pragma unroll
-          for (int kb = 0; kb < KB; ++kb) bq[s0][kb] = yp[32 * kb];
+#pragma unroll
+          for (int kb = 0; kb < KB; ++kb) bq[s0][kb] = g2_read(s0, kb);
         }
         __builtin_amdgcn_sched_barrier(0);
 #pragma unroll
         for (int s = 0; s < 16; ++s) {
           if (s + 2 < 16) {
-            const float *yp = Yc + pmf_rowmap(s + 2, h) * KpS + l31;
-#pragma unroll
-            for (int kb = 0; kb < KB; ++kb) bq[(s + 2) % 3][kb] = yp[32 * kb];
+#pragma unroll
+            for (int kb = 0; kb < KB; ++kb) bq[(s + 2) % 3][kb] = g2_read(s + 2, kb);
           }
           if (s < NVM) vmem_op(s);
 #pragma unroll
@@ -626,7 +668,7 @@
 
       PMF_STAMP(4);
       if (NYB == 1) __syncthreads();
-      stage_store(nxt, par ^ 1, jn, ynext, sgnext, cnext);
+      stage_store(nxt, par ^ 1, jn, ynext, sgnext, cnext, PLAIN);
       PMF_STAMP(5);
       __syncthreads();
       PMF_STAMP(6);
@@ -635,7 +677,7 @@
 #pragma unroll
         for (int q = 0; q < NBT; ++q) bt_store(bt_e(q), btn[q], btm[q]);
       }
-      slab_first = pidx == 0 || (pidx == 1 && ti0 + t < t0_first);
+      slab_first = !PLAIN && (pidx == 0 || (pidx == 1 && ti0 + t < t0_first));
       if (XW) {
         typedef float f32x4 __attribute__((ext_vector_type(4)));
         constexpr int XW_RING = 8, XW_AHEAD = 6;
@@ -677,7 +719,8 @@
         const int nel = (rem > BN ? BN : (int)rem) * Kp;
         float4 v = make_float4((gy0[0] + gy1[0]) * xw_sg, (gy0[1] + gy1[1]) * xw_sg, (gy0[2] + gy1[2]) * xw_sg, (gy0[3] + gy1[3]) * xw_sg);
         if (!slab_first) { v.x += gold[0].x; v.y += gold[0].y; v.z += gold[0].z; v.w += gold[0].w; }
-        if (xw_e < nel) pmf_store_stream(reinterpret_cast<float4 *>(myslab + j0 * Kp + xw_e), v);
+        if (PLAIN) pmf_store_stream(reinterpret_cast<float4 *>(const_cast<char *>(ho_at(myslab + j0 * Kp, ho_g[0][0]))), v);
+        else if (xw_e < nel) pmf_store_stream(reinterpret_cast<float4 *>(myslab + j0 * Kp + xw_e), v);
         PMF_STAMP(4);
         forward_reduce(acc, nxt, par ^ 1, false, 0);
         PMF_STAMP(8);
@@ -691,6 +734,18 @@
         PMF_STAMP(9);
       }
     }
+    };
+    if constexpr (PLAINB) {
+      tile_loop(PmfFlag<false>{}, 0, t_plain);
+      tile_loop(PmfFlag<PLAINB>{}, t_plain, t_pend);
+      if (t_pend < ntiles) {
+#pragma unroll
+        for (int rb = 0; rb < RBW; ++rb) tflag[rb] = 1;
+        tile_loop(PmfFlag<false>{}, t_pend, ntiles);
+      }
+    } else {
+      tile_loop(PmfFlag<false>{}, 0, ntiles);
+    }
     if (XW && !bt_lds) __syncthreads();
 
     PMF_STAMP(10);
@@ -714,6 +769,7 @@
     double s = 0.0;
     for (int q = 0; q < NW; ++q) s += red[q];
     a.loss_partial[wg] = s;
+    if (PLAINB && a.plain_count) a.plain_count[wg] = n_plain;
   }
 #ifdef PMF_STAMPS
   st_acc[14] = __builtin_amdgcn_s_memtime() - st_t0;
diff --git a/pathmatfac.jl_amd/csrc/pmf_pass.hip b/pathmatfac.jl_amd/csrc/pmf_pass.hip
--- a/pathmatfac.jl_amd/csrc/pmf_pass.hip
+++ b/pathmatfac.jl_amd/csrc/pmf_pass.hip
@@ -23,6 +23,47 @@
   k_tile_flags<<<(unsigned)ntiles, 256, 0, c->stream>>>(c->D, ntiles, c->tflags, c->store == PMF_STORE_BF16);
   HIPCHK(hipGetLastError());
   c->tflags_valid = true;
+  c->ptab_bm = 0;
+  return 0;
+}
+
+__global__ __launch_bounds__(256) void k_plain_table(const uint32_t *__restrict__ flags, int64_t nRB, int nblk, int64_t n_ct,
+                                                     int32_t *__restrict__ out) {
+  __shared__ int sc[256];
+  const int64_t rp = blockIdx.x;
+  int32_t *o = out + rp * (n_ct + 1);
+  int carry = 0;
+  if (threadIdx.x == 0) o[0] = 0;
+  for (int64_t c0 = 0; c0 < n_ct; c0 += 256) {
+    const int64_t ct = c0 + threadIdx.x;
+    int bad = 0;
+    if (ct < n_ct)
+      for (int r = 0; r < nblk; ++r) {
+        const int64_t rb = rp * nblk + r;
+        if (rb >= nRB || flags[ct * nRB + rb] == 0) bad = 1;
+      }
+    sc[threadIdx.x] = bad;
+    __syncthreads();
+    for (int d = 1; d < 256; d <<= 1) {
+      const int v = threadIdx.x >= d ? sc[threadIdx.x - d] : 0;
+      __syncthreads();
+      sc[threadIdx.x] += v;
+      __syncthreads();
+    }
+    if (ct < n_ct) o[ct + 1] = carry + sc[threadIdx.x];
+    carry += sc[255];
+    __syncthreads();
+  }
+}
+
+static int ensure_plain_table(pmf_ctx *c, int64_t bm, int64_t n_ct) {
+  const int64_t n_rp = (c->M + bm - 1) / bm;
+  if (c->ptab_bm == bm && c->ptab_n_rp == n_rp && c->ptab_n_ct == n_ct) return 0;
+  if (n_ct + 1 > 0x7fffffff || n_rp > 0x7fffffff) return pmf_fail("too many tiles");
+  PMFCHK(c->ptab.ensure((size_t)n_rp * (size_t)(n_ct + 1), false));
+  k_plain_table<<<(unsigned)n_rp, 256, 0, c->stream>>>(c->tflags, c->nRB, (int)(bm / 32), n_ct, c->ptab);
+  HIPCHK(hipGetLastError());
+  c->ptab_bm = bm; c->ptab_n_rp = n_rp; c->ptab_n_ct = n_ct;
   return 0;
 }
 
@@ -289,6 +330,11 @@
   return nullptr;
 }
 
+static bool pass_has_plain_loop(const pmf_ctx *c, const FusedGeom &g, bool want_gx, bool want_gy) {
+  const FusedFamily &f = *g.fam;
+  return f.kernel == 0 && f.KB == 2 && f.NW == 8 && f.RBW == 1 && want_gx && want_gy && g.bmode == 0 && !c->mixed;
+}
+
 FusedGeom fused_geometry(pmf_ctx *c, bool want_gx, bool want_gy, bool allow_chunks) {
   FusedGeom g;
   auto batch_fits = [&](const FusedFamily *f) {
@@ -411,6 +457,10 @@
     PMFCHK(c->gx_part.ensure(pieces * (size_t)f.BM() * (size_t)c->Kp, false));
   }
   PMFCHK(ensure_tile_flags(c));
+  if (pass_has_plain_loop(c, g, want_gx, want_gy)) {
+    PMFCHK(ensure_plain_table(c, f.BM(), g.n_ct_all));
+    PMFCHK(c->plain_count.ensure((size_t)grid_sum, false));
+  }
   if (f.img != IMG_NONE) {
     size_t xblk = 0, yblk = 0;
     for (const FusedFamily &o : fused_families)
@@ -452,7 +502,11 @@
   out[n++] = {"loss_partial", grid_sum * 8, (int64_t)c->loss_partial.bytes()};
   out[n++] = {"pm", bt ? g.n_rp * c->n_bv * 16 : 0, bt ? (int64_t)g.ps->pm.bytes() : 0};
   out[n++] = {"row_slot", bt ? (int64_t)c->n_bv * c->M : 0, bt ? (int64_t)g.ps->row_slot.bytes() : 0};
-  static_assert(PMF_PASS_EXTENTS == 10, "fused_pass_extents");
+  if (pass_has_plain_loop(c, g, want_gx, want_gy)) {
+    out[n++] = {"ptab", g.n_rp * (g.n_ct_all + 1) * 4, c->ptab_bm == f.BM() ? (int64_t)c->ptab.bytes() : 0};
+    out[n++] = {"plain_count", grid_sum * 4, (int64_t)c->plain_count.bytes()};
+  }
+  static_assert(PMF_PASS_EXTENTS == 12, "fused_pass_extents");
   return n;
 }
 int check_pass_extents(const PassExtent *e, int n) {
@@ -525,6 +579,12 @@
   a.M = c->M; a.N = c->N; a.n_tiles = n_rp * n_ct; a.tps = (int)tiles_per_seg; a.n_ct = (int)n_ct; a.n_cseg = (int)n_cseg;
   a.want_gx = want_gx; a.want_gy = want_gy;
   a.ct0 = (int32_t)g.ct0[s];
+  const bool has_plain = pass_has_plain_loop(c, g, want_gx, want_gy);
+  if (has_plain) {
+    const char *pe = getenv("PMF_PLAIN");
+    a.ptab = c->ptab; a.ptab_stride = (int32_t)(g.n_ct_all + 1); a.plain = !(pe && atoi(pe) == 0);
+    a.plain_count = c->plain_count + loss_off;
+  }
   a.gx_part = c->gx_part; a.piece_base = ws.d_piece_base_abs; a.gx_slot_stride = (int64_t)f.BM() * c->Kp;
   {
     const char *dbg = getenv("PMF_DEBUG_FLAGS");
@@ -564,6 +624,7 @@
   pmf_last_xreg = 0;
   const int rc = f.launch[c->store == PMF_STORE_BF16](&c->dyn_lds, c->stream, a, grid, batch, c->mixed);
   c->last_xreg = pmf_last_xreg;
+  c->last_plain_n = has_plain && pmf_last_xreg ? loss_off + grid : -1;
   if (f.kernel != 0) c->sb_launches += 1;
   PMFCHK(rc);
   HIPCHK(hipEventRecord(ev.second, c->stream));
@@ -597,12 +658,39 @@
   return 0;
 }
 
-extern "C" int pmf_debug_last_path(pmf_ctx *c, int *bmode, int *layer_path, int *slots, int *xreg) {
+extern "C" int pmf_debug_last_path(pmf_ctx *c, int *bmode, int *layer_path, int *slots, int *xreg, int64_t *plain_tiles) {
   if (!c) return pmf_fail("null context");
+  if (plain_tiles) {
+    *plain_tiles = 0;
+    if (c->last_plain_n > 0) {
+      PMFCHK(ctx_bind(c));
+      std::vector<int32_t> h((size_t)c->last_plain_n);
+      HIPCHK(hipMemcpyAsync(h.data(), c->plain_count, h.size() * sizeof(int32_t), hipMemcpyDeviceToHost, c->stream));
+      HIPCHK(hipStreamSynchronize(c->stream));
+      for (int32_t v : h) *plain_tiles += v;
+    }
+  }
   if (xreg) *xreg = c->last_xreg;
   if (bmode) *bmode = c->last_bmode;
   if (layer_path) *layer_path = c->last_layer_path;
   if (slots) *slots = c->nbs;
+  return 0;
+}
+
+extern "C" int pmf_debug_plain_table(pmf_ctx *c, int32_t *out, int64_t cap, int64_t *n_rp, int64_t *n_ct) {
+  PMFCHK(ctx_bind(c));
+  if (!c->D) return pmf_fail("data not set");
+  PMFCHK(ensure_tile_flags(c));
+  const int64_t nct = (c->N + PMF_BN - 1) / PMF_BN;
+  PMFCHK(ensure_plain_table(c, 256, nct));
+  if (n_rp) *n_rp = c->ptab_n_rp;
+  if (n_ct) *n_ct = nct;
+  if (out) {
+    const int64_t n = c->ptab_n_rp * (nct + 1);
+    if (cap < n) return pmf_fail("pmf_debug_plain_table: room for %lld entries, %lld needed", (long long)cap, (long long)n);
+    HIPCHK(hipMemcpyAsync(out, c->ptab, (size_t)n * sizeof(int32_t), hipMemcpyDeviceToHost, c->stream));
+    HIPCHK(hipStreamSynchronize(c->stream));
+  }
   return 0;
 }
 
```
